# BaZzz01010101/ReflaxMan

Hardware: AMD Instinct MI355X
Metric: Mrays/sec at 3840×2160 depth-8; max per-channel |Δ| vs CPU reference (higher is better)
Workload: dtype f32; 1 GPU; C3 synth16: 16 spheres + 4 textured triangles + sun, 3840x2160, depth 8, 1 spp; scene=synth16, width=3840, height=2160, depth=8, spp=1, parallelism=single-gpu

## Files before the change

include/rfx.h:

```cpp
#ifndef RFX_H
#define RFX_H
#include <stddef.h>
#include <stdint.h>

#ifdef __cplusplus
extern "C" {
#endif

#define RFX_ABI_VERSION 4

typedef enum {
  RFX_OK = 0,
  RFX_ERR_ARG = -1,
  RFX_ERR_HIP = -2,
  RFX_ERR_STATE = -3,
  RFX_ERR_IO = -4,
  RFX_ERR_RNG = -5,
  RFX_ERR_NODEV = -6
} rfx_status;

enum { RFX_METAL = 0, RFX_DIELECTRIC = 1 };

typedef struct rfx_scene rfx_scene;
typedef struct rfx_renderer rfx_renderer;

int rfx_abi_version(void);
const char *rfx_last_error(void);
enum { RFX_BUILD_PRIM_LARGE = 1, RFX_BUILD_PRIM_SSAA = 2, RFX_BUILD_PRIM_LANES = 4, RFX_BUILD_ONE_LIGHT = 8 };
int rfx_build_options(void);

rfx_scene *rfx_scene_create(float diff_r, float diff_g, float diff_b, float diff_power);
void rfx_scene_destroy(rfx_scene *scene);
int rfx_scene_add_sphere(rfx_scene *scene, const float center[3], float radius, int material_type,
                         const float rgb[3], float reflectivity, float transparency);
int rfx_scene_add_triangle(rfx_scene *scene, const float v1[3], const float v2[3], const float v3[3],
                           int material_type, const float rgb[3], float reflectivity, float transparency);
int rfx_scene_add_mesh(rfx_scene *scene, const float *vertices, uint32_t n_vertices, const uint32_t *indices,
                       uint32_t n_triangles, int material_type, const float rgb[3], float reflectivity,
                       float transparency);
int rfx_scene_add_plane(rfx_scene *scene, const float pos[3], const float norm[3], int material_type,
                        const float rgb[3], float reflectivity, float transparency);
int rfx_scene_plane_count(const rfx_scene *scene);
int rfx_triangle_set_texture(rfx_scene *scene, int object_index, int texture_index, const float uv[6]);
int rfx_scene_add_light(rfx_scene *scene, const float origin[3], float radius, const float rgb[3], float power);
int rfx_scene_add_texture_argb(rfx_scene *scene, uint32_t width, uint32_t height, const uint32_t *argb);
int rfx_scene_add_texture_file(rfx_scene *scene, const char *path, int *loaded);
int rfx_scene_set_skybox_file(rfx_scene *scene, const char *path);
int rfx_scene_set_skybox_argb(rfx_scene *scene, uint32_t width, uint32_t height, const uint32_t *argb);
int rfx_scene_counts(const rfx_scene *scene, int *spheres, int *triangles, int *lights, int *textures);
int rfx_scene_tri_bvh_dump(const rfx_scene *scene, int32_t counts[5], float *boxes, int32_t *children,
                           int32_t *leaf_ids, int32_t *residual);

void rfx_camera_view(const float eye[3], const float at[3], float view[9]);
float rfx_camera_rz(uint32_t width, float fov);

int rfx_tga_load(const char *path, uint32_t *width, uint32_t *height, uint32_t *argb, size_t capacity);
int rfx_tga_save(const char *path, uint32_t width, uint32_t height, const uint32_t *argb);
int rfx_bmp_save(const char *path, uint32_t width, uint32_t height, const uint32_t *argb);
void rfx_argb_from_rgb(const float *rgb, size_t pixels, uint32_t *argb);

int rfx_renderer_create(rfx_renderer **out, int device);
void rfx_renderer_destroy(rfx_renderer *r);
int rfx_renderer_device(const rfx_renderer *r);
int rfx_renderer_set_stream(rfx_renderer *r, void *hip_stream);
int rfx_renderer_set_scene(rfx_renderer *r, const rfx_scene *scene);
int rfx_renderer_set_tile_order(rfx_renderer *r, int mode);
int rfx_renderer_set_regroup(rfx_renderer *r, int park_after);
int rfx_renderer_set_regroup_sort(rfx_renderer *r, int on);
int rfx_renderer_bounce_form(const rfx_renderer *r);
int rfx_renderer_set_tri_accel(rfx_renderer *r, int mode);
typedef struct {
  int32_t tri_nodes, tri_depth;
  int32_t tri_leaf_size;
  int32_t tri_in_leaves;
  int32_t tri_residual;
  int32_t sph_nodes, sph_depth;
  int32_t narrow_tri_bvh;
} rfx_accel_info;
int rfx_renderer_accel_info(const rfx_renderer *r, rfx_accel_info *out);
int rfx_renderer_set_prim_masks(rfx_renderer *r, int mode);
int rfx_renderer_set_rng(rfx_renderer *r, uint32_t sphere_seed, uint32_t jitter_seed);
int rfx_renderer_get_rng(rfx_renderer *r, uint32_t *sphere_seed, uint32_t *jitter_seed);

typedef struct {
  float eye[3];
  float view[9];
  float fov;
  uint32_t width, height;
  int32_t reflect_num;
  int32_t sample_num;
  int32_t additive;
  int32_t additive_counter;
  uint32_t row_block;
  uint32_t rank, nranks;
  uint64_t pixel_begin;
  uint64_t pixel_end;
  uint64_t span_begin;
  uint64_t span_end;
} rfx_frame;

uint32_t rfx_strip_rows(uint32_t height, uint32_t row_block, uint32_t rank, uint32_t nranks);
uint32_t rfx_strip_row_to_y(uint32_t r, uint32_t row_block, uint32_t rank, uint32_t nranks);

#define RFX_NCOUNTERS 40
int rfx_render_frame(rfx_renderer *r, const rfx_frame *frame, float *d_rgb, uint32_t *d_argb,
                     uint64_t *d_counters, void *stream);
int rfx_renderer_set_launch_traces(rfx_renderer *r, uint64_t max_traces);

int rfx_frame_rng_blocks(rfx_renderer *r, const rfx_frame *frame, uint32_t nslices, uint64_t *blocks_per_slice);
int rfx_frame_rng_count(rfx_renderer *r, const rfx_frame *frame, uint32_t slice, uint32_t nslices,
                        uint32_t *d_blk_counts, void *stream);
int rfx_render_frame_counted(rfx_renderer *r, const rfx_frame *frame, uint32_t nslices, const uint32_t *d_blk_counts,
                             float *d_rgb, uint32_t *d_argb, uint64_t *d_counters, void *stream);
int rfx_render_frame_counted_ev(rfx_renderer *r, const rfx_frame *frame, uint32_t nslices,
                                const uint32_t *d_blk_counts, float *d_rgb, uint32_t *d_argb, uint64_t *d_counters,
                                void *stream, void *emitted_event);

int rfx_frame_rng_emit(rfx_renderer *r, const rfx_frame *frame, uint32_t nslices, const uint32_t *d_blk_counts,
                       void *stream, void *emitted_event);
int rfx_render_frame_emitted(rfx_renderer *r, const rfx_frame *frame, float *d_rgb, uint32_t *d_argb,
                             uint64_t *d_counters, void *stream);
int rfx_frame_rng_discard(rfx_renderer *r);
int rfx_frame_rng_pending(rfx_renderer *r, uint32_t *frame_start);

int rfx_frame_rng_rewind(rfx_renderer *r);

typedef struct rfx_group rfx_group;
int rfx_group_create(rfx_group **out, const int *devices, int n);
void rfx_group_destroy(rfx_group *g);
int rfx_group_size(const rfx_group *g);
rfx_renderer *rfx_group_renderer(rfx_group *g, int member);
int rfx_group_set_scene(rfx_group *g, const rfx_scene *scene);
int rfx_group_set_bands(rfx_group *g, uint32_t height, const uint32_t *bounds);
int rfx_group_get_bands(const rfx_group *g, uint32_t *bounds);
int rfx_group_render_frame(rfx_group *g, const rfx_frame *frame, float *d_rgb, uint32_t *d_argb, void *stream);

int rfx_renderer_set_timing(rfx_renderer *r, int enable);
int rfx_renderer_get_timing(rfx_renderer *r, double *prepass_ms, double *trace_ms, uint64_t *frames);

int rfx_render_frame_host(rfx_renderer *r, const rfx_frame *frame, float *rgb, uint32_t *argb,
                          uint64_t *counters);

int rfx_device_alloc(rfx_renderer *r, size_t bytes, void **dptr);
int rfx_device_free(rfx_renderer *r, void *dptr);
int rfx_memcpy_d2h(rfx_renderer *r, void *dst, const void *src, size_t bytes);
int rfx_memcpy_h2d(rfx_renderer *r, void *dst, const void *src, size_t bytes);
int rfx_memcpy_d2d(rfx_renderer *r, void *dst, const void *src, size_t bytes);
int rfx_synchronize(rfx_renderer *r);

int rfx_rand_dirs(rfx_renderer *r, uint32_t seed, uint64_t n, float *out3, uint32_t *seed_out);

int rfx_kat_objects(rfx_renderer *r, const float *rays, const int32_t *objects, uint64_t n, float *out);
int rfx_kat_texels(rfx_renderer *r, int texture, const float *in, uint64_t n, float *out);
int rfx_kat_powf(rfx_renderer *r, const float *xy, uint64_t n, float *out);
int rfx_kat_argb(rfx_renderer *r, const float *rgb, uint64_t n, uint32_t *out);
int rfx_kat_powf_cube(rfx_renderer *r, uint64_t counts[2]);
int rfx_kat_div(rfx_renderer *r, uint64_t first, uint64_t n, uint64_t counts[3]);
int rfx_kat_kernarg(rfx_renderer *r, int swapped, uint32_t out[3]);

#ifdef __cplusplus
}
#endif
#endif
```

reflaxman_amd/_lib.py:

```python
from __future__ import annotations

import ctypes as C
import os

from . import _build

RFX_OK = 0
RFX_NCOUNTERS = 40
RFX_ABI_VERSION = 4
METAL, DIELECTRIC = 0, 1

_fp = C.POINTER(C.c_float)
_u32p = C.POINTER(C.c_uint32)
_u64p = C.POINTER(C.c_uint64)


class RfxError(RuntimeError):
    pass


class Frame(C.Structure):
    _fields_ = [
        ("eye", C.c_float * 3), ("view", C.c_float * 9), ("fov", C.c_float),
        ("width", C.c_uint32), ("height", C.c_uint32),
        ("reflect_num", C.c_int32), ("sample_num", C.c_int32),
        ("additive", C.c_int32), ("additive_counter", C.c_int32),
        ("row_block", C.c_uint32), ("rank", C.c_uint32), ("nranks", C.c_uint32),
        ("pixel_begin", C.c_uint64), ("pixel_end", C.c_uint64),
        ("span_begin", C.c_uint64), ("span_end", C.c_uint64),
    ]


class AccelInfo(C.Structure):
    _fields_ = [(n, C.c_int32) for n in ("tri_nodes", "tri_depth", "tri_leaf_size", "tri_in_leaves", "tri_residual",
                                         "sph_nodes", "sph_depth", "narrow_tri_bvh")]


_i32p = C.POINTER(C.c_int32)

SIGNATURES = [
    ("rfx_abi_version", C.c_int, []),
    ("rfx_last_error", C.c_char_p, []),
    ("rfx_build_options", C.c_int, []),
    ("rfx_scene_create", C.c_void_p, [C.c_float] * 4),
    ("rfx_scene_destroy", None, [C.c_void_p]),
    ("rfx_scene_add_sphere", C.c_int, [C.c_void_p, _fp, C.c_float, C.c_int, _fp, C.c_float, C.c_float]),
    ("rfx_scene_add_triangle", C.c_int, [C.c_void_p, _fp, _fp, _fp, C.c_int, _fp, C.c_float, C.c_float]),
    ("rfx_scene_add_mesh", C.c_int, [C.c_void_p, _fp, C.c_uint32, _u32p, C.c_uint32, C.c_int, _fp, C.c_float, C.c_float]),
    ("rfx_scene_tri_bvh_dump", C.c_int, [C.c_void_p, _i32p, _fp, _i32p, _i32p, _i32p]),
    ("rfx_scene_add_plane", C.c_int, [C.c_void_p, _fp, _fp, C.c_int, _fp, C.c_float, C.c_float]),
    ("rfx_scene_plane_count", C.c_int, [C.c_void_p]),
    ("rfx_triangle_set_texture", C.c_int, [C.c_void_p, C.c_int, C.c_int, _fp]),
    ("rfx_scene_add_light", C.c_int, [C.c_void_p, _fp, C.c_float, _fp, C.c_float]),
    ("rfx_scene_add_texture_argb", C.c_int, [C.c_void_p, C.c_uint32, C.c_uint32, _u32p]),
    ("rfx_scene_add_texture_file", C.c_int, [C.c_void_p, C.c_char_p, C.POINTER(C.c_int)]),
    ("rfx_scene_set_skybox_file", C.c_int, [C.c_void_p, C.c_char_p]),
    ("rfx_scene_set_skybox_argb", C.c_int, [C.c_void_p, C.c_uint32, C.c_uint32, _u32p]),
    ("rfx_scene_counts", C.c_int, [C.c_void_p] + [C.POINTER(C.c_int)] * 4),
    ("rfx_camera_view", None, [_fp, _fp, _fp]),
    ("rfx_camera_rz", C.c_float, [C.c_uint32, C.c_float]),
    ("rfx_tga_load", C.c_int, [C.c_char_p, _u32p, _u32p, _u32p, C.c_size_t]),
    ("rfx_tga_save", C.c_int, [C.c_char_p, C.c_uint32, C.c_uint32, _u32p]),
    ("rfx_bmp_save", C.c_int, [C.c_char_p, C.c_uint32, C.c_uint32, _u32p]),
    ("rfx_argb_from_rgb", None, [_fp, C.c_size_t, _u32p]),
    ("rfx_renderer_create", C.c_int, [C.POINTER(C.c_void_p), C.c_int]),
    ("rfx_renderer_destroy", None, [C.c_void_p]),
    ("rfx_renderer_device", C.c_int, [C.c_void_p]),
    ("rfx_renderer_set_stream", C.c_int, [C.c_void_p, C.c_void_p]),
    ("rfx_renderer_set_scene", C.c_int, [C.c_void_p, C.c_void_p]),
    ("rfx_renderer_set_rng", C.c_int, [C.c_void_p, C.c_uint32, C.c_uint32]),
    ("rfx_renderer_get_rng", C.c_int, [C.c_void_p, _u32p, _u32p]),
    ("rfx_strip_rows", C.c_uint32, [C.c_uint32] * 4),
    ("rfx_strip_row_to_y", C.c_uint32, [C.c_uint32] * 4),
    ("rfx_render_frame", C.c_int, [C.c_void_p, C.POINTER(Frame), C.c_void_p, C.c_void_p, C.c_void_p, C.c_void_p]),
    ("rfx_render_frame_host", C.c_int, [C.c_void_p, C.POINTER(Frame), _fp, _u32p, _u64p]),
    ("rfx_frame_rng_blocks", C.c_int, [C.c_void_p, C.POINTER(Frame), C.c_uint32, _u64p]),
    ("rfx_frame_rng_count", C.c_int, [C.c_void_p, C.POINTER(Frame), C.c_uint32, C.c_uint32, C.c_void_p, C.c_void_p]),
    ("rfx_render_frame_counted", C.c_int, [C.c_void_p, C.POINTER(Frame), C.c_uint32, C.c_void_p, C.c_void_p,
                                           C.c_void_p, C.c_void_p, C.c_void_p]),
    ("rfx_render_frame_counted_ev", C.c_int, [C.c_void_p, C.POINTER(Frame), C.c_uint32, C.c_void_p, C.c_void_p,
                                              C.c_void_p, C.c_void_p, C.c_void_p, C.c_void_p]),
    ("rfx_frame_rng_emit", C.c_int, [C.c_void_p, C.POINTER(Frame), C.c_uint32, C.c_void_p, C.c_void_p, C.c_void_p]),
    ("rfx_render_frame_emitted", C.c_int, [C.c_void_p, C.POINTER(Frame), C.c_void_p, C.c_void_p, C.c_void_p,
                                           C.c_void_p]),
    ("rfx_frame_rng_discard", C.c_int, [C.c_void_p]),
    ("rfx_frame_rng_pending", C.c_int, [C.c_void_p, _u32p]),
    ("rfx_frame_rng_rewind", C.c_int, [C.c_void_p]),
    ("rfx_group_create", C.c_int, [C.POINTER(C.c_void_p), C.POINTER(C.c_int), C.c_int]),
    ("rfx_group_destroy", None, [C.c_void_p]),
    ("rfx_group_size", C.c_int, [C.c_void_p]),
    ("rfx_group_renderer", C.c_void_p, [C.c_void_p, C.c_int]),
    ("rfx_group_set_scene", C.c_int, [C.c_void_p, C.c_void_p]),
    ("rfx_group_set_bands", C.c_int, [C.c_void_p, C.c_uint32, _u32p]),
    ("rfx_group_get_bands", C.c_int, [C.c_void_p, _u32p]),
    ("rfx_group_render_frame", C.c_int, [C.c_void_p, C.POINTER(Frame), C.c_void_p, C.c_void_p, C.c_void_p]),
    ("rfx_renderer_set_timing", C.c_int, [C.c_void_p, C.c_int]),
    ("rfx_renderer_set_tile_order", C.c_int, [C.c_void_p, C.c_int]),
    ("rfx_renderer_set_prim_masks", C.c_int, [C.c_void_p, C.c_int]),
    ("rfx_renderer_set_regroup", C.c_int, [C.c_void_p, C.c_int]),
    ("rfx_renderer_set_regroup_sort", C.c_int, [C.c_void_p, C.c_int]),
    ("rfx_renderer_set_launch_traces", C.c_int, [C.c_void_p, C.c_uint64]),
    ("rfx_renderer_bounce_form", C.c_int, [C.c_void_p]),
    ("rfx_renderer_set_tri_accel", C.c_int, [C.c_void_p, C.c_int]),
    ("rfx_renderer_accel_info", C.c_int, [C.c_void_p, C.POINTER(AccelInfo)]),
    ("rfx_renderer_get_timing", C.c_int, [C.c_void_p, C.POINTER(C.c_double), C.POINTER(C.c_double), _u64p]),
    ("rfx_device_alloc", C.c_int, [C.c_void_p, C.c_size_t, C.POINTER(C.c_void_p)]),
    ("rfx_device_free", C.c_int, [C.c_void_p, C.c_void_p]),
    ("rfx_memcpy_d2h", C.c_int, [C.c_void_p, C.c_void_p, C.c_void_p, C.c_size_t]),
    ("rfx_memcpy_h2d", C.c_int, [C.c_void_p, C.c_void_p, C.c_void_p, C.c_size_t]),
    ("rfx_memcpy_d2d", C.c_int, [C.c_void_p, C.c_void_p, C.c_void_p, C.c_size_t]),
    ("rfx_synchronize", C.c_int, [C.c_void_p]),
    ("rfx_rand_dirs", C.c_int, [C.c_void_p, C.c_uint32, C.c_uint64, _fp, _u32p]),
    ("rfx_kat_objects", C.c_int, [C.c_void_p, _fp, C.POINTER(C.c_int32), C.c_uint64, _fp]),
    ("rfx_kat_texels", C.c_int, [C.c_void_p, C.c_int, _fp, C.c_uint64, _fp]),
    ("rfx_kat_powf", C.c_int, [C.c_void_p, _fp, C.c_uint64, _fp]),
    ("rfx_kat_argb", C.c_int, [C.c_void_p, _fp, C.c_uint64, _u32p]),
    ("rfx_kat_powf_cube", C.c_int, [C.c_void_p, C.POINTER(C.c_uint64)]),
    ("rfx_kat_div", C.c_int, [C.c_void_p, C.c_uint64, C.c_uint64, C.POINTER(C.c_uint64)]),
    ("rfx_kat_kernarg", C.c_int, [C.c_void_p, C.c_int, C.POINTER(C.c_uint32)]),
]

_lib = None


def lib_path() -> str:
    return _build.LIB


def bind(path: str, partial: bool = False):
    L = C.CDLL(os.path.abspath(path))
    for name, res, args in SIGNATURES:
        if partial and not hasattr(L, name):
            continue
        fn = getattr(L, name)
        fn.restype = res
        fn.argtypes = args
    return L


def load(build_if_missing: bool = True):
    global _lib
    if _lib is not None:
        return _lib
    path = _build.LIB
    if build_if_missing:
        try:
            _build.build()
        except Exception as e:
            if not os.path.exists(path):
                raise RfxError(f"librfx.so missing and cannot be built: {e}") from e
    if not os.path.exists(path):
        raise RfxError(f"librfx.so not found at {path}: the HIP renderer is required (no CPU fallback)")
    L = C.CDLL(path)
    for name, res, args in SIGNATURES:
        fn = getattr(L, name)
        fn.restype = res
        fn.argtypes = args
    if L.rfx_abi_version() != RFX_ABI_VERSION:
        raise RfxError("librfx.so ABI version mismatch")
    _lib = L
    return L


def lib_sha256(path: str = None) -> str:
    import hashlib
    with open(path or _build.LIB, "rb") as f:
        return hashlib.sha256(f.read()).hexdigest()


def device_sha256(path: str = None) -> str:
    import hashlib
    import struct
    with open(path or _build.LIB, "rb") as f:
        b = f.read()
    shoff = struct.unpack_from("<Q", b, 0x28)[0]
    shentsize, shnum, shstrndx = struct.unpack_from("<HHH", b, 0x3A)
    secs = [struct.unpack_from("<IIQQQQIIQQ", b, shoff + i * shentsize) for i in range(shnum)]
    names = secs[shstrndx][4]
    for name_off, _, _, _, off, size, *_ in secs:
        if b[names + name_off:b.index(b"\0", names + name_off)] == b".hip_fatbin":
            return hashlib.sha256(b[off:off + size]).hexdigest()
    return None


def check(rc: int, what: str = "") -> int:
    if rc < 0:
        msg = load().rfx_last_error().decode(errors="replace")
        raise RfxError(f"{what or 'rfx call'} failed ({rc}): {msg}")
    return rc


def fptr(a):
    return a.ctypes.data_as(_fp)


def u32ptr(a):
    return a.ctypes.data_as(_u32p)


def u64ptr(a):
    return a.ctypes.data_as(_u64p)


def farr(v, n=None):
    v = list(v)
    if n is not None and len(v) != n:
        raise ValueError(f"expected {n} floats, got {len(v)}")
    return (C.c_float * len(v))(*v)
```

reflaxman_amd/csrc/rfx_host.cpp:

```cpp
#include <hip/hip_runtime.h>

#include <math.h>
#include <stdarg.h>
#include <stdio.h>
#include <stdlib.h>
#include <string.h>

#include <algorithm>
#include <cmath>
#include <mutex>
#include <string>
#include <vector>

#include "../../include/rfx.h"
#include "rfx_math.h"
#include "rfx_types.h"

#pragma clang fp contract(off)

namespace rfx {
uint64_t rng_blocks_for(uint64_t traces);
void rng_jump_table(uint64_t nblk, uint32_t *out);
hipError_t launch_rng_count(const uint32_t *d_seed, const uint32_t *d_jump, uint32_t *d_blk_cnt, uint64_t blk0,
                            uint64_t nblk_slice, uint16_t *d_masks, hipStream_t st);
hipError_t launch_rng_finish(const uint32_t *d_seed, const uint32_t *d_jump, uint32_t *d_next_seed,
                             const uint32_t *d_blk_cnt, const uint16_t *d_masks, uint64_t nblk, uint64_t traces,
                             uint32_t *d_rd_state, int *d_err, uint64_t ss2, uint64_t W, uint32_t row_block,
                             uint32_t rank, uint32_t nranks, hipStream_t st);
hipError_t launch_rng_finish_band(const uint32_t *d_seed, const uint32_t *d_jump, uint32_t *d_next_seed,
                                  const uint32_t *d_blk_cnt, const uint16_t *d_masks, uint64_t nblk, uint64_t traces,
                                  uint32_t *d_rd_state, int *d_err, uint64_t lo, uint64_t hi, uint64_t *d_off,
                                  uint32_t *d_range, uint32_t *d_tile_sum, hipStream_t st);
hipError_t launch_rng_fused(const uint32_t *d_seed, const uint32_t *d_jump, uint32_t *d_next_seed, uint64_t nblk,
                            uint64_t traces, uint32_t *d_rd_state, int *d_err, unsigned long long *d_status,
                            unsigned long long *d_ticket, unsigned long long base, uint32_t epoch, hipStream_t st);
hipError_t launch_trace(const DevScene &S, const FrameParams &P, bool stats, hipStream_t st);
hipError_t launch_prim_cull(const DevScene &S, const FrameParams &P, uint64_t *masks, hipStream_t st);
hipError_t launch_queue_sort(const uint32_t *count, const uint32_t *key, uint32_t *hist, uint32_t *order, hipStream_t st);
uint32_t trace_tiles(const FrameParams &P);
bool trace_lanes(const FrameParams &P);
bool trace_chunks(const FrameParams &P);
size_t tile_order_scratch();
hipError_t launch_tile_order(const uint32_t *cost, uint32_t n, uint32_t *order, uint32_t *scratch, hipStream_t st);
void launch_bounce(int cfg, dim3 grid, const DevScene &S, const FrameParams &P, hipStream_t st);
hipError_t launch_bounce_lds(int cfg, uint32_t groups, const DevScene &S, const FrameParams &P, hipStream_t st);
hipError_t launch_kat(int what, const DevScene &S, int tex, const void *in, const int32_t *objs, uint32_t n, void *out,
                      hipStream_t st);
hipError_t launch_kat_powf_cube(uint32_t first, uint32_t n, unsigned long long *counts, hipStream_t st);
hipError_t launch_kat_div(uint64_t first, uint32_t n, unsigned long long *counts, hipStream_t st);
hipError_t launch_kat_kernarg(const DevScene &S, const FrameParams &P, int swapped, uint32_t *out, hipStream_t st);
}

using namespace rfx;

static thread_local std::string g_last_error;

static int fail(int code, const char *fmt, ...)
{
  char buf[512];
  va_list ap;
  va_start(ap, fmt);
  vsnprintf(buf, sizeof(buf), fmt, ap);
  va_end(ap);
  g_last_error = buf;
  return code;
}

#define HIP_CHECK(expr)                                                                  \
  do {                                                                                   \
    hipError_t e_ = (expr);                                                              \
    if (e_ != hipSuccess) return fail(RFX_ERR_HIP, "%s: %s", #expr, hipGetErrorString(e_)); \
  } while (0)

extern "C" int rfx_abi_version(void) { return RFX_ABI_VERSION; }
extern "C" const char *rfx_last_error(void) { return g_last_error.c_str(); }

struct HostTexture { uint32_t w = 0, h = 0; bool loaded = false; std::vector<uint32_t> texels; };
struct HostMat { int dielectric; float r, g, b, refl, transp; };
struct HostSphere { v3 center; float radius, sq_radius; HostMat mat; int obj; };
struct HostTri {
  v3 v0, v1, v2, norm;
  double cond = INFINITY;
  m33 ax, tuv;
  float tu0 = 0, tv0 = 0;
  int tex = -1;
  HostMat mat;
  int obj;
};
struct HostLight { v3 origin; float radius; float r, g, b, power; };
struct HostPlane { v3 pos, norm; HostMat mat; int obj; };

struct rfx_scene {
  col diff, env;
  float diff_power;
  float half_tile_w, half_tile_h;
  int skybox = -1;
  std::vector<HostSphere> spheres;
  std::vector<HostTri> tris;
  std::vector<HostPlane> planes;
  std::vector<int> obj_kind, obj_idx;
  std::vector<HostLight> lights;
  std::vector<HostTexture> textures;
};

static void default_half_tiles(rfx_scene *s)
{
  s->half_tile_w = 1.0f / 8.0f - kFltEpsilon;
  s->half_tile_h = 1.0f / 6.0f - kFltEpsilon;
}

extern "C" rfx_scene *rfx_scene_create(float dr, float dg, float db, float dp)
{
  rfx_scene *s = new rfx_scene();
  s->diff = mkc(dr, dg, db);
  s->diff_power = dp;
  s->env = cscale(s->diff, dp);
  default_half_tiles(s);
  return s;
}

extern "C" void rfx_scene_destroy(rfx_scene *s) { delete s; }

static HostMat make_mat(int type, const float rgb[3], float refl, float transp)
{
  HostMat m;
  m.dielectric = type == RFX_DIELECTRIC;
  m.r = rgb[0]; m.g = rgb[1]; m.b = rgb[2];
  m.refl = clampf(refl, 0.0f, 1.0f);
  m.transp = clampf(transp, 0.0f, 1.0f);
  return m;
}

extern "C" int rfx_scene_add_sphere(rfx_scene *s, const float c[3], float radius, int type, const float rgb[3],
                                    float refl, float transp)
{
  if (!s || !c || !rgb || (type != RFX_METAL && type != RFX_DIELECTRIC)) return fail(RFX_ERR_ARG, "add_sphere: bad args");
  if (radius <= kVerySmall) radius = kVerySmall;
  HostSphere sp;
  sp.center = mk(c[0], c[1], c[2]);
  sp.radius = radius;
  sp.sq_radius = radius * radius;
  sp.mat = make_mat(type, rgb, refl, transp);
  sp.obj = (int)s->obj_kind.size();
  s->obj_kind.push_back(0);
  s->obj_idx.push_back((int)s->spheres.size());
  s->spheres.push_back(sp);
  return sp.obj;
}

extern "C" int rfx_scene_add_triangle(rfx_scene *s, const float a[3], const float b[3], const float c[3], int type,
                                      const float rgb[3], float refl, float transp)
{
  if (!s || !a || !b || !c || !rgb || (type != RFX_METAL && type != RFX_DIELECTRIC))
    return fail(RFX_ERR_ARG, "add_triangle: bad args");
  HostTri t;
  const v3 v0 = mk(a[0], a[1], a[2]), v1 = mk(b[0], b[1], b[2]), v2 = mk(c[0], c[1], c[2]);
  t.v0 = v0;
  t.mat = make_mat(type, rgb, refl, transp);
  t.norm = normalized(cross(sub(v1, v0), sub(v2, v0)));
  const m33 basis = from_cols(sub(v2, v0), sub(v1, v0), neg(t.norm));
  t.ax = inverted(basis);
  t.v1 = v1;
  t.v2 = v2;
  {
    const float *a = &basis.m11, *b = &t.ax.m11;
    double na = 0.0, nb = 0.0;
    for (int k = 0; k < 9; ++k) { na += (double)a[k] * a[k]; nb += (double)b[k] * b[k]; }
    const float det = basis.m11 * (basis.m22 * basis.m33 - basis.m32 * basis.m23) +
                      basis.m21 * (basis.m32 * basis.m13 - basis.m12 * basis.m33) +
                      basis.m31 * (basis.m12 * basis.m23 - basis.m13 * basis.m22);
    t.cond = fabsf(det) > kVerySmall ? sqrt(na * nb) : INFINITY;
  }
  memset(&t.tuv, 0, sizeof(t.tuv));
  t.obj = (int)s->obj_kind.size();
  s->obj_kind.push_back(1);
  s->obj_idx.push_back((int)s->tris.size());
  s->tris.push_back(t);
  return t.obj;
}

extern "C" int rfx_scene_add_mesh(rfx_scene *s, const float *vertices, uint32_t n_vertices, const uint32_t *indices,
                                  uint32_t n_triangles, int type, const float rgb[3], float refl, float transp)
{
  if (!s || !rgb || (type != RFX_METAL && type != RFX_DIELECTRIC) || (n_triangles && (!vertices || !indices)))
    return fail(RFX_ERR_ARG, "add_mesh: bad args");
  for (size_t i = 0; i < 3 * (size_t)n_triangles; ++i)
    if (indices[i] >= n_vertices)
      return fail(RFX_ERR_ARG, "add_mesh: index %u of triangle %zu is not below %u vertices", indices[i], i / 3, n_vertices);
// ... 156 lines not shown
  ih.biSize = sizeof(ih); ih.biWidth = (int32_t)w; ih.biHeight = (int32_t)h; ih.biPlanes = 1; ih.biBitCount = 32;
  bool ok = fwrite(&fh, sizeof(fh), 1, f) == 1 && fwrite(&ih, sizeof(ih), 1, f) == 1 &&
            fwrite(argb, (size_t)w * h * 4, 1, f) == 1;
  fclose(f);
  return ok ? RFX_OK : fail(RFX_ERR_IO, "bmp_save: short write");
}

extern "C" int rfx_scene_add_texture_file(rfx_scene *s, const char *path, int *loaded)
{
  if (!s || !path) return fail(RFX_ERR_ARG, "add_texture_file: bad args");
  HostTexture t;
  const bool ok = has_ext(path, ".tga") && tga_read(path, t.w, t.h, t.texels);
  t.loaded = ok;
  if (loaded) *loaded = ok ? 1 : 0;
  s->textures.push_back(std::move(t));
  return (int)s->textures.size() - 1;
}

static void set_skybox_index(rfx_scene *s, int idx)
{
  s->skybox = idx;
  const HostTexture &t = s->textures[idx];
  if (t.loaded)
  {
    s->half_tile_w = 1.0f / 8.0f - 1.0f / (float)t.w - kFltEpsilon;
    s->half_tile_h = 1.0f / 6.0f - 1.0f / (float)t.h - kFltEpsilon;
  }
  else
    default_half_tiles(s);
}

extern "C" int rfx_scene_set_skybox_file(rfx_scene *s, const char *path)
{
  if (!s || !path) return fail(RFX_ERR_ARG, "set_skybox_file: bad args");
  int loaded = 0;
  const int idx = rfx_scene_add_texture_file(s, path, &loaded);
  set_skybox_index(s, idx);
  return loaded;
}

extern "C" int rfx_scene_set_skybox_argb(rfx_scene *s, uint32_t w, uint32_t h, const uint32_t *argb)
{
  if (!s) return fail(RFX_ERR_ARG, "set_skybox_argb: null scene");
  const int idx = rfx_scene_add_texture_argb(s, w, h, argb);
  set_skybox_index(s, idx);
  return s->textures[idx].loaded ? 1 : 0;
}

extern "C" int rfx_scene_plane_count(const rfx_scene *s)
{
  if (!s) return fail(RFX_ERR_ARG, "plane_count: null scene");
  return (int)s->planes.size();
}

extern "C" int rfx_scene_counts(const rfx_scene *s, int *ns, int *nt, int *nl, int *nx)
{
  if (!s) return fail(RFX_ERR_ARG, "counts: null scene");
  if (ns) *ns = (int)s->spheres.size();
  if (nt) *nt = (int)s->tris.size();
  if (nl) *nl = (int)s->lights.size();
  if (nx) *nx = (int)s->textures.size();
  return RFX_OK;
}

extern "C" void rfx_camera_view(const float e[3], const float a[3], float view[9])
{
  const v3 eye = mk(e[0], e[1], e[2]), at = mk(a[0], a[1], a[2]);
  const v3 up = mk(0.0f, 1.0f, 0.0f);
  const v3 oz = normalized(sub(at, eye));
  const v3 ox = normalized(cross(up, oz));
  const v3 oy = normalized(cross(oz, ox));
  const m33 m = from_cols(ox, oy, oz);
  memcpy(view, &m, sizeof(m));
}

extern "C" float rfx_camera_rz(uint32_t width, float fov)
{
  return (float)width / 2.0f / tanf(fov / 2.0f);
}

extern "C" void rfx_argb_from_rgb(const float *rgb, size_t n, uint32_t *out)
{
  for (size_t i = 0; i < n; ++i) out[i] = argb(mkc(rgb[i * 3], rgb[i * 3 + 1], rgb[i * 3 + 2]));
}

extern "C" uint32_t rfx_strip_rows(uint32_t H, uint32_t rb, uint32_t rank, uint32_t nranks)
{
  if (nranks <= 1) return H;
  if (!rb || rank >= nranks) return 0;
  const uint32_t full = H / rb, rem = H % rb;
  uint32_t rows = (full / nranks) * rb;
  const uint32_t extra = full % nranks;
  if (rank < extra) rows += rb;
  if (rem && full % nranks == rank) rows += rem;
  return rows;
}

extern "C" uint32_t rfx_strip_row_to_y(uint32_t r, uint32_t rb, uint32_t rank, uint32_t nranks)
{
  if (nranks <= 1) return r;
  return (r / rb * nranks + rank) * rb + r % rb;
}

#ifndef RFX_TILE_ORDER_DEFAULT
#define RFX_TILE_ORDER_DEFAULT 1
#endif
#ifndef RFX_TILE_ORDER_MIN_TILES
#define RFX_TILE_ORDER_MIN_TILES 49152
#endif
constexpr size_t kPrimWords = 5;
constexpr size_t kPrimLargeWords = 12;
#ifndef RFX_PRIM_SSAA
#define RFX_PRIM_SSAA 0
#endif
#ifndef RFX_PRIM_LANES
#define RFX_PRIM_LANES 1
#endif
#ifndef RFX_PRIM_CHUNKS
#define RFX_PRIM_CHUNKS 1
#endif
#ifndef RFX_PRIM_LARGE
#define RFX_PRIM_LARGE 0
#endif
#ifndef RFX_ONE_LIGHT
#define RFX_ONE_LIGHT 1
#endif
#ifndef RFX_BOUNCE_GROUPS_PER_CU
#define RFX_BOUNCE_GROUPS_PER_CU 14
#endif

#ifndef RFX_QUEUE_SORT
#define RFX_QUEUE_SORT 0
#endif
#ifndef RFX_TRI_BVH_AUTO_MIN
#define RFX_TRI_BVH_AUTO_MIN 128
#endif
#ifndef RFX_TRI_BVH_NARROW_MIN
#define RFX_TRI_BVH_NARROW_MIN (1 << 30)
#endif
#ifndef RFX_PARK_AFTER
#define RFX_PARK_AFTER 2
#endif
#ifndef RFX_TILE_SORT_MAIN
#define RFX_TILE_SORT_MAIN 1
#endif
#ifndef RFX_TILE_SORT_EVERY
#define RFX_TILE_SORT_EVERY 16
#endif
#ifndef RFX_LAUNCH_TRACES
#define RFX_LAUNCH_TRACES (1ull << 30)
#endif
#ifndef RFX_SPLIT_STREAMS
#define RFX_SPLIT_STREAMS 2
#endif
constexpr uint64_t kMaxLaunchTraces = 1ull << 31;
#ifndef RFX_SCAN_EMIT_BLOCKS
#define RFX_SCAN_EMIT_BLOCKS 16384
#endif
struct rfx_renderer {
  int device = 0;
  int cus = 256;
  hipStream_t own_stream = nullptr;
  hipStream_t stream = nullptr;
  DevScene dev{};
  std::vector<void *> scene_allocs;
  bool has_scene = false;
  uint32_t *d_seed = nullptr;
  uint32_t seed_idx = 0;
  int *d_err = nullptr;
  uint32_t jitter_seed = 0;
  uint32_t *d_rd = nullptr; uint64_t rd_cap = 0;
  uint32_t *d_rd_alt = nullptr; uint64_t rd_alt_cap = 0;
  int emit_pending = -1;
  int trace_buf = 0;
  bool split_alt_busy = false;
  uint64_t emit_key[10] = {};
  bool rewind_ok = false, rewind_flip = false, rewind_saved = false;
  uint32_t rewind_jitter = 0;
  hipStream_t rewind_stream = nullptr;
  uint64_t launch_traces = RFX_LAUNCH_TRACES;
  uint64_t state_seq = 0;
  hipStream_t split_stream = nullptr;
  hipEvent_t split_ev[3] = {nullptr, nullptr, nullptr};
  uint32_t *d_blk_cnt = nullptr; uint64_t blk_cap = 0;
  uint64_t *d_blk_off = nullptr;
  uint32_t *d_rng_range = nullptr;
  uint32_t *d_tile_sum = nullptr;
  unsigned long long *d_rng_status = nullptr, *d_rng_ticket = nullptr;
  unsigned long long rng_tickets = 0;
  uint32_t rng_epoch = 0;
  uint16_t *d_rng_masks = nullptr;
  uint32_t *d_jump = nullptr;
  float *d_img = nullptr; uint32_t *d_argb = nullptr; uint64_t *d_cnt = nullptr; size_t img_cap = 0;
  int tile_mode = RFX_TILE_ORDER_DEFAULT;
  uint32_t *d_tile_cost = nullptr, *d_tile_order = nullptr, *d_tile_scratch = nullptr;
  uint32_t tile_cap = 0, tile_n = 0;
  uint64_t tile_key = 0;
  hipStream_t tile_stream = nullptr;
  hipEvent_t tile_fork = nullptr, tile_join = nullptr;
  bool tile_pending = false;
  hipStream_t tile_waited = nullptr;
  uint64_t tile_count = 0;
  int park_after = -1;
  uint64_t *d_prim_mask = nullptr;
  size_t prim_cap = 0;
  uint64_t *d_split_mask[2] = {nullptr, nullptr};
  size_t split_mask_cap[2] = {0, 0};
  std::vector<uint8_t> prim_key;
  std::vector<uint8_t> prim_seen;
  uint64_t scene_gen = 0;
  int prim_mode = 1;
  int tri_accel = -1;
  rfx_accel_info accel{};
  int bounce_form = 0;
  QRay *d_queue = nullptr;
  uint64_t queue_cap = 0;
  uint32_t *d_qctr = nullptr;
  uint32_t *d_qkey = nullptr, *d_qorder = nullptr;
  int queue_sort = RFX_QUEUE_SORT;
  bool timing = false, timing_this = false;
  uint32_t timing_every = 1;
  uint64_t timing_seq = 0;
  std::vector<hipEvent_t> events;
  size_t events_used = 0;
};

static uint32_t *seed_cur(rfx_renderer *r) { return r->d_seed + r->seed_idx; }
static uint32_t *seed_next(rfx_renderer *r) { return r->d_seed + (r->seed_idx ^ 1u); }

static int timing_event(rfx_renderer *r, hipStream_t st)
{
  if (!r->timing_this) return RFX_OK;
  if (r->events_used == r->events.size())
  {
    hipEvent_t e;
    HIP_CHECK(hipEventCreate(&e));
    r->events.push_back(e);
  }
  HIP_CHECK(hipEventRecord(r->events[r->events_used++], st));
  return RFX_OK;
}

static int timing_start(rfx_renderer *r, hipStream_t st)
{
  r->timing_this = r->timing && r->timing_seq++ % r->timing_every == 0;
  return timing_event(r, st);
}

extern "C" int rfx_renderer_set_timing(rfx_renderer *r, int enable)
{
  if (!r || enable < 0) return fail(RFX_ERR_ARG, "set_timing: null renderer or negative period");
  r->timing = enable != 0;
  r->timing_every = enable > 1 ? (uint32_t)enable : 1u;
  r->timing_seq = 0;
  r->timing_this = false;
  r->events_used = 0;
  return RFX_OK;
}

extern "C" int rfx_renderer_get_timing(rfx_renderer *r, double *prepass_ms, double *trace_ms, uint64_t *frames)
{
  if (!r) return fail(RFX_ERR_ARG, "get_timing: null renderer");
  double pre = 0.0, tr = 0.0;
  const size_t n = r->events_used / 3;
  if (n) HIP_CHECK(hipEventSynchronize(r->events[3 * n - 1]));
  for (size_t i = 0; i < n; ++i)
  {
    float a = 0.0f, b = 0.0f;
    HIP_CHECK(hipEventElapsedTime(&a, r->events[3 * i], r->events[3 * i + 1]));
    HIP_CHECK(hipEventElapsedTime(&b, r->events[3 * i + 1], r->events[3 * i + 2]));
    pre += a;
    tr += b;
  }
  r->events_used = 0;
  if (prepass_ms) *prepass_ms = pre;
  if (trace_ms) *trace_ms = tr;
  if (frames) *frames = n;
  return RFX_OK;
}

static int set_dev(rfx_renderer *r)
{
  HIP_CHECK(hipSetDevice(r->device));
  return RFX_OK;
}

extern "C" int rfx_renderer_create(rfx_renderer **out, int device)
{
  if (!out) return fail(RFX_ERR_ARG, "renderer_create: null out");
  *out = nullptr;
  int n = 0;
  if (hipGetDeviceCount(&n) != hipSuccess || n <= 0) return fail(RFX_ERR_NODEV, "no HIP device");
  if (device < 0 || device >= n) return fail(RFX_ERR_ARG, "device %d out of range (%d devices)", device, n);
  rfx_renderer *r = new rfx_renderer();
  r->device = device;
  int rc;
  if ((rc = set_dev(r)) != RFX_OK) { delete r; return rc; }
  if (hipStreamCreateWithFlags(&r->own_stream, hipStreamNonBlocking) != hipSuccess ||
      hipMalloc(&r->d_seed, 3 * sizeof(uint32_t)) != hipSuccess || hipMalloc(&r->d_err, sizeof(int)) != hipSuccess)
  {
    delete r;
    return fail(RFX_ERR_HIP, "renderer_create: HIP allocation failed");
  }
  r->stream = r->own_stream;
  if (hipDeviceGetAttribute(&r->cus, hipDeviceAttributeMultiprocessorCount, device) != hipSuccess || r->cus <= 0)
    r->cus = 256;
  const uint32_t seeds[2] = {1350490027u, 1350490027u};
  if (hipMemcpy(r->d_seed, seeds, sizeof(seeds), hipMemcpyHostToDevice) != hipSuccess ||
      hipMemset(r->d_err, 0, sizeof(int)) != hipSuccess)
  {
    delete r;
    return fail(RFX_ERR_HIP, "renderer_create: HIP init copy failed");
  }
  *out = r;
  return RFX_OK;
}

static void free_scene(rfx_renderer *r)
{
  for (void *p : r->scene_allocs) (void)hipFree(p);
  r->scene_allocs.clear();
  r->has_scene = false;
}

extern "C" void rfx_renderer_destroy(rfx_renderer *r)
{
  if (!r) return;
  (void)hipSetDevice(r->device);
  (void)hipStreamSynchronize(r->stream);
  free_scene(r);
  (void)hipFree(r->d_seed); (void)hipFree(r->d_err); (void)hipFree(r->d_rd); (void)hipFree(r->d_rd_alt);
  (void)hipFree(r->d_blk_cnt); (void)hipFree(r->d_jump); (void)hipFree(r->d_rng_masks); (void)hipFree(r->d_blk_off);
  (void)hipFree(r->d_tile_sum);
  (void)hipFree(r->d_rng_range);
  (void)hipFree(r->d_rng_status); (void)hipFree(r->d_rng_ticket);
  (void)hipFree(r->d_img); (void)hipFree(r->d_argb); (void)hipFree(r->d_cnt);
  (void)hipFree(r->d_queue); (void)hipFree(r->d_qctr); (void)hipFree(r->d_prim_mask);
  (void)hipFree(r->d_split_mask[0]); (void)hipFree(r->d_split_mask[1]);
  (void)hipFree(r->d_qkey); (void)hipFree(r->d_qorder);
  for (hipEvent_t e : r->events) (void)hipEventDestroy(e);
  if (r->tile_stream) (void)hipStreamSynchronize(r->tile_stream);
  (void)hipFree(r->d_tile_cost); (void)hipFree(r->d_tile_order); (void)hipFree(r->d_tile_scratch);
  if (r->tile_fork) (void)hipEventDestroy(r->tile_fork);
  if (r->tile_join) (void)hipEventDestroy(r->tile_join);
  if (r->tile_stream) (void)hipStreamDestroy(r->tile_stream);
  if (r->split_stream)
  {
    (void)hipStreamSynchronize(r->split_stream);
    (void)hipStreamDestroy(r->split_stream);
  }
  for (hipEvent_t e : r->split_ev)
    if (e) (void)hipEventDestroy(e);
  if (r->own_stream) (void)hipStreamDestroy(r->own_stream);
  delete r;
}

extern "C" int rfx_build_options(void)
{
  return (RFX_PRIM_LARGE ? RFX_BUILD_PRIM_LARGE : 0) | (RFX_PRIM_SSAA ? RFX_BUILD_PRIM_SSAA : 0) |
         (RFX_PRIM_LANES ? RFX_BUILD_PRIM_LANES : 0) | (RFX_ONE_LIGHT ? RFX_BUILD_ONE_LIGHT : 0) |
         (RFX_BVH_LEAF_PAIRS << 8);
}

extern "C" int rfx_renderer_set_launch_traces(rfx_renderer *r, uint64_t max_traces)
{
  if (!r) return fail(RFX_ERR_ARG, "renderer_set_launch_traces: null renderer");
  r->launch_traces = max_traces ? std::min(max_traces, kMaxLaunchTraces) : (uint64_t)RFX_LAUNCH_TRACES;
  return RFX_OK;
}

extern "C" int rfx_renderer_device(const rfx_renderer *r) { return r ? r->device : -1; }

extern "C" int rfx_renderer_set_tile_order(rfx_renderer *r, int mode)
{
  if (!r || mode < 0 || mode > 3) return fail(RFX_ERR_ARG, "renderer_set_tile_order: mode 0, 1, 2 or 3");
  r->tile_mode = mode;
  return RFX_OK;
}

extern "C" int rfx_renderer_set_prim_masks(rfx_renderer *r, int mode)
{
  if (!r || mode < 0 || mode > 2) return fail(RFX_ERR_ARG, "renderer_set_prim_masks: mode 0, 1 or 2");
  r->prim_mode = mode;
  r->prim_key.clear();
  r->prim_seen.clear();
  return RFX_OK;
}

extern "C" int rfx_renderer_bounce_form(const rfx_renderer *r)
{
  if (!r) return fail(RFX_ERR_ARG, "renderer_bounce_form: null renderer");
  return r->bounce_form;
}

extern "C" int rfx_renderer_set_regroup(rfx_renderer *r, int park_after)
{
  if (!r || park_after < -1) return fail(RFX_ERR_ARG, "renderer_set_regroup: -1 (default), 0 (off) or segments >= 1");
  r->park_after = park_after;
  return RFX_OK;
}

extern "C" int rfx_renderer_set_regroup_sort(rfx_renderer *r, int on)
{
  if (!r || on < 0 || on > 1) return fail(RFX_ERR_ARG, "renderer_set_regroup_sort: 0 or 1");
  r->queue_sort = on;
  return RFX_OK;
}

extern "C" int rfx_renderer_set_stream(rfx_renderer *r, void *s)
{
  if (!r) return fail(RFX_ERR_ARG, "set_stream: null renderer");
  r->stream = s ? (hipStream_t)s : r->own_stream;
  return RFX_OK;
}

template <class T>
static int upload(rfx_renderer *r, const std::vector<T> &v, const T **dst)
{
  if (v.empty()) { *dst = nullptr; return RFX_OK; }
  void *p = nullptr;
  HIP_CHECK(hipMalloc(&p, v.size() * sizeof(T)));
  r->scene_allocs.push_back(p);
  HIP_CHECK(hipMemcpy(p, v.data(), v.size() * sizeof(T), hipMemcpyHostToDevice));
  *dst = (const T *)p;
  return RFX_OK;
}

static void spatial_order(std::vector<uint32_t> &idx, size_t a, size_t b, const std::vector<HostSphere> &sp)
{
  if (b - a <= 2) return;
  double lo[3] = {INFINITY, INFINITY, INFINITY}, hi[3] = {-INFINITY, -INFINITY, -INFINITY};
  for (size_t i = a; i < b; ++i)
  {
    const double c[3] = {sp[idx[i]].center.x, sp[idx[i]].center.y, sp[idx[i]].center.z};
    for (int k = 0; k < 3; ++k) { lo[k] = fmin(lo[k], c[k]); hi[k] = fmax(hi[k], c[k]); }
  }
  int axis = 0;
  for (int k = 1; k < 3; ++k)
    if (hi[k] - lo[k] > hi[axis] - lo[axis]) axis = k;
  const size_t mid = a + 2 * ((b - a + 2) / 4);
  auto key = [&](uint32_t i) { return axis == 0 ? sp[i].center.x : axis == 1 ? sp[i].center.y : sp[i].center.z; };
  std::nth_element(idx.begin() + a, idx.begin() + mid, idx.begin() + b,
                   [&](uint32_t x, uint32_t y) { return key(x) < key(y) || (key(x) == key(y) && x < y); });
  spatial_order(idx, a, mid, sp);
  spatial_order(idx, mid, b, sp);
}

#ifndef RFX_BVH_STACK
#define RFX_BVH_STACK 16
#endif
namespace {
struct PairBox { double lo[3], hi[3], c[3]; };

int build_pair_bvh(std::vector<BvhNode> &nodes, std::vector<uint32_t> &pairs, size_t a, size_t b,
                   const std::vector<PairBox> &box, const double *ref, int level, int &depth, bool widen = true)
{
  if (b - a == 1) return ~(int)pairs[a];
  depth = std::max(depth, level + 1);
  const int id = (int)nodes.size();
  nodes.push_back(BvhNode{});
  double lo[3] = {INFINITY, INFINITY, INFINITY}, hi[3] = {-INFINITY, -INFINITY, -INFINITY};
  for (size_t i = a; i < b; ++i)
    for (int k = 0; k < 3; ++k) { lo[k] = fmin(lo[k], box[pairs[i]].c[k]); hi[k] = fmax(hi[k], box[pairs[i]].c[k]); }
  int axis = 0;
  for (int k = 1; k < 3; ++k)
    if (hi[k] - lo[k] > hi[axis] - lo[axis]) axis = k;
  size_t mid = a + (b - a) / 2;
  const size_t cnt = b - a;
  int need = 0;
  while (((size_t)1 << need) < cnt) ++need;
  if (level + need + 2 <= RFX_BVH_STACK && cnt > 2)
  {
    double best = INFINITY;
    int best_axis = axis;
    size_t best_mid = mid;
    std::vector<uint32_t> tmp(pairs.begin() + a, pairs.begin() + b);
    std::vector<double> right(cnt + 1);
    auto area = [](const double *l, const double *h) {
      const double dx = h[0] - l[0], dy = h[1] - l[1], dz = h[2] - l[2];
      return dx * dy + dy * dz + dz * dx;
    };
    for (int ax = 0; ax < 3; ++ax)
    {
      std::sort(tmp.begin(), tmp.end(), [&](uint32_t x, uint32_t y) {
        return box[x].c[ax] < box[y].c[ax] || (box[x].c[ax] == box[y].c[ax] && x < y);
      });
      double l[3] = {INFINITY, INFINITY, INFINITY}, h[3] = {-INFINITY, -INFINITY, -INFINITY};
      for (size_t i = cnt; i-- > 0;)
      {
        for (int k = 0; k < 3; ++k) { l[k] = fmin(l[k], box[tmp[i]].lo[k]); h[k] = fmax(h[k], box[tmp[i]].hi[k]); }
        right[i] = area(l, h) * (double)(cnt - i);
      }
      for (int k = 0; k < 3; ++k) { l[k] = INFINITY; h[k] = -INFINITY; }
      const size_t cap = (size_t)1 << std::min(30, RFX_BVH_STACK - level - 2);
      for (size_t i = 1; i < cnt; ++i)
      {
        for (int k = 0; k < 3; ++k) { l[k] = fmin(l[k], box[tmp[i - 1]].lo[k]); h[k] = fmax(h[k], box[tmp[i - 1]].hi[k]); }
        if (i > cap || cnt - i > cap) continue;
        const double cost = area(l, h) * (double)i + right[i];
        if (cost < best) { best = cost; best_axis = ax; best_mid = a + i; }
      }
    }
    axis = best_axis;
    mid = best_mid;
  }
  std::nth_element(pairs.begin() + a, pairs.begin() + mid, pairs.begin() + b, [&](uint32_t x, uint32_t y) {
    return box[x].c[axis] < box[y].c[axis] || (box[x].c[axis] == box[y].c[axis] && x < y);
  });
  const int kids[2] = {build_pair_bvh(nodes, pairs, a, mid, box, ref, level + 1, depth, widen),
                       build_pair_bvh(nodes, pairs, mid, b, box, ref, level + 1, depth, widen)};
  const size_t range[2][2] = {{a, mid}, {mid, b}};
  BvhNode &n = nodes[id];
  for (int c = 0; c < 2; ++c)
  {
    double l[3] = {INFINITY, INFINITY, INFINITY}, h[3] = {-INFINITY, -INFINITY, -INFINITY};
    for (size_t i = range[c][0]; i < range[c][1]; ++i)
      for (int k = 0; k < 3; ++k) { l[k] = fmin(l[k], box[pairs[i]].lo[k]); h[k] = fmax(h[k], box[pairs[i]].hi[k]); }
#if RFX_BVH_PREWIDE
    if (widen)
    {
      double cd = 0.0, hd = 0.0;
      for (int k = 0; k < 3; ++k)
      {
        const double dc = ref[k] - 0.5 * (l[k] + h[k]), dh = 0.5 * (h[k] - l[k]);
        cd += dc * dc;
        hd += dh * dh;
      }
      const double w = 2e-3 * (double)nextafterf((float)((sqrt(cd) + sqrt(hd)) * 1.0001), INFINITY) * (1.0 + 1e-6);
      for (int k = 0; k < 3; ++k) { l[k] -= w; h[k] += w; }
    }
#endif
    n.lx[c] = nextafterf((float)l[0], -INFINITY); n.ly[c] = nextafterf((float)l[1], -INFINITY);
    n.lz[c] = nextafterf((float)l[2], -INFINITY);
    n.hx[c] = nextafterf((float)h[0], INFINITY); n.hy[c] = nextafterf((float)h[1], INFINITY);
    n.hz[c] = nextafterf((float)h[2], INFINITY);
    n.child[c] = kids[c];
    double mt = 0.0;
    {
      double cd = 0.0, hd = 0.0;
      for (int k = 0; k < 3; ++k)
// ... 311 lines not shown
    {
      PairBox &b = box[j];
      for (int k = 0; k < 3; ++k) { b.lo[k] = INFINITY; b.hi[k] = -INFINITY; }
      for (size_t q = kLeafSph * j; q < std::min(nsph, kLeafSph * j + kLeafSph); ++q)
      {
        const double c[3] = {bd[q].x, bd[q].y, bd[q].z}, rr = bd[q].r;
        for (int k = 0; k < 3; ++k) { b.lo[k] = fmin(b.lo[k], c[k] - rr); b.hi[k] = fmax(b.hi[k], c[k] + rr); }
      }
      for (int k = 0; k < 3; ++k) b.c[k] = 0.5 * (b.lo[k] + b.hi[k]);
    }
    std::vector<uint32_t> pairs(npairs);
    for (size_t j = 0; j < npairs; ++j) pairs[j] = (uint32_t)j;
    for (int k = 0; k < 3; ++k)
    {
      double lo = INFINITY, hi = -INFINITY;
      for (const PairBox &pb : box) { lo = fmin(lo, pb.lo[k]); hi = fmax(hi, pb.hi[k]); }
      bvh_ref[k] = (double)(float)(0.5 * (lo + hi));
    }
    build_pair_bvh(bvh, pairs, 0, npairs, box, bvh_ref, 0, bvh_depth);
    if (bvh_depth > RFX_BVH_STACK) { bvh.clear(); bvh_depth = 0; }
    if (bvh.size() > 32767 || npairs > 32768) { bvh.clear(); bvh_depth = 0; }
  }
  TriTree tt;
  std::vector<TriGeo> tleaf;
  const bool want_tri = RFX_TRI_BVH && !small &&
                        (r->tri_accel >= 1 || (r->tri_accel < 0 && s->tris.size() >= (size_t)RFX_TRI_BVH_AUTO_MIN));
  if (want_tri)
  {
    if (nsph <= 32) tri_ref_point(s->tris, bvh_ref);
    if (build_tri_tree(s->tris, bvh_ref, true, tt))
    {
      tleaf.assign(tt.order.size(), TriGeo{});
      for (size_t q = 0; q < tt.order.size(); ++q)
      {
        const int32_t i = tt.order[q];
        if (i < 0) continue;
        tleaf[q] = tg[i];
        const int32_t obj = s->tris[i].obj;
        memcpy(&tleaf[q].pad[0], &i, 4);
        memcpy(&tleaf[q].pad[1], &obj, 4);
      }
    }
  }
  std::vector<PlaneGeo> pg;
  std::vector<MatRec> pm;
  for (const HostPlane &p : s->planes)
  {
    pg.push_back({p.pos.x, p.pos.y, p.pos.z, p.norm.x, p.norm.y, p.norm.z, p.obj, p.mat.dielectric});
    pm.push_back({p.mat.r, p.mat.g, p.mat.b, p.mat.refl});
  }
  std::vector<int32_t> loc(s->obj_kind.size());
  {
    std::vector<int32_t> sph_dev(nsph);
    for (size_t di = 0; di < nsph; ++di) sph_dev[order[di]] = (int32_t)di;
    for (size_t o = 0; o < loc.size(); ++o)
    {
      const int kind = s->obj_kind[o], idx = s->obj_idx[o];
      loc[o] = kind << 28 | (kind == 0 ? sph_dev[idx] : idx);
    }
  }
  std::vector<LightRec> lr;
  for (const HostLight &l : s->lights) lr.push_back({l.origin.x, l.origin.y, l.origin.z, l.radius, l.r, l.g, l.b, l.power});
  std::vector<TexRec> tr;
  std::vector<uint32_t> pool;
  for (const HostTexture &t : s->textures)
  {
    const bool empty = t.texels.empty();
    tr.push_back({(uint32_t)pool.size(), empty ? 0u : t.w, empty ? 0u : t.h, 0});
    pool.insert(pool.end(), t.texels.begin(), t.texels.end());
  }
  DevScene d{};
  if ((rc = upload(r, sg, &d.sph_geo)) || (rc = upload(r, sp, &d.sph_pair)) || (rc = upload(r, sm, &d.sph_mat)) ||
      (rc = upload(r, si, &d.sph_info)) ||
      (rc = upload(r, tg, &d.tri_geo)) || (rc = upload(r, ts, &d.tri_shade)) || (rc = upload(r, tm, &d.tri_mat)) ||
      (rc = upload(r, lr, &d.lights)) || (rc = upload(r, tr, &d.texs)) || (rc = upload(r, pool, &d.texels)) ||
      (rc = upload(r, bd, &d.bound)) || (rc = upload(r, cs, &d.cull_small)) || (rc = upload(r, ct, &d.cull_tri)) || (rc = upload(r, cb, &d.chunk_bound)) ||
      (rc = upload(r, pg, &d.pln_geo)) || (rc = upload(r, pm, &d.pln_mat)) || (rc = upload(r, loc, &d.obj_loc)) ||
      (rc = upload(r, bvh, &d.bvh)) || (rc = upload(r, tt.nodes, &d.tri_bvh)) || (rc = upload(r, tleaf, &d.tri_leaf)) ||
      (rc = upload(r, tt.resid, &d.tri_resid)))
    return rc;
  d.n_tri_resid = (int32_t)tt.resid.size();
  d.n_tri_bvh = (int32_t)tt.nodes.size();
  d.tri_bvh_depth = tt.depth;
  r->accel = rfx_accel_info{};
  r->accel.tri_nodes = d.n_tri_bvh;
  r->accel.tri_depth = tt.depth;
  r->accel.tri_leaf_size = RFX_TRI_BVH_LEAF;
  r->accel.tri_in_leaves = tt.nodes.empty() ? 0 : (int32_t)(s->tris.size() - tt.resid.size());
  r->accel.tri_residual = d.n_tri_resid;
  r->accel.sph_nodes = (int32_t)bvh.size();
  r->accel.sph_depth = bvh_depth;
  d.tri_bvh_narrow = !tt.nodes.empty() && (r->tri_accel == 2 || s->tris.size() >= (size_t)RFX_TRI_BVH_NARROW_MIN);
  r->accel.narrow_tri_bvh = d.tri_bvh_narrow;
  {
    float mt_max = 0.0f;
    for (const BvhNode &n : bvh) mt_max = fmaxf(mt_max, fmaxf(n.mt[0], n.mt[1]));
    const float mstep = mt_max > 0.0f ? mt_max / 65000.0f : 1.0f;
    std::vector<uint32_t> aux(2 * bvh.size());
    for (size_t i = 0; i < bvh.size(); ++i)
    {
      const BvhNode &n = bvh[i];
      uint32_t q[2];
      for (int c = 0; c < 2; ++c) q[c] = (uint32_t)std::min(65535.0, ceil((double)n.mt[c] / mstep) + 1.0);
      aux[2 * i] = ((uint32_t)(uint16_t)(int16_t)n.child[0]) | ((uint32_t)(uint16_t)(int16_t)n.child[1] << 16);
      aux[2 * i + 1] = q[0] | q[1] << 16;
    }
    if ((rc = upload(r, aux, &d.bvh_aux))) return rc;
    d.bvh_mstep = mstep;
    d.n_bvh = (int32_t)bvh.size();
  }
  d.n_sph = (int32_t)sg.size();
  d.n_tri = (int32_t)tg.size();
  d.n_light = (int32_t)lr.size();
  d.n_chunk = (int32_t)cb.size();
  d.n_pln = (int32_t)pg.size();
  d.n_tex = (int32_t)tr.size();
  d.bvh_depth = bvh_depth;
  d.bvh_rx = (float)bvh_ref[0]; d.bvh_ry = (float)bvh_ref[1]; d.bvh_rz = (float)bvh_ref[2];
  if (!bvh.empty())
  {
    const BvhNode &root = bvh[0];
    const float lo[3] = {fminf(root.lx[0], root.lx[1]), fminf(root.ly[0], root.ly[1]), fminf(root.lz[0], root.lz[1])};
    const float hi[3] = {fmaxf(root.hx[0], root.hx[1]), fmaxf(root.hy[0], root.hy[1]), fmaxf(root.hz[0], root.hz[1])};
    float s[3];
    for (int k = 0; k < 3; ++k) s[k] = hi[k] > lo[k] ? 8.0f / (hi[k] - lo[k]) : 0.0f;
    d.key_lx = lo[0]; d.key_ly = lo[1]; d.key_lz = lo[2];
    d.key_sx = s[0]; d.key_sy = s[1]; d.key_sz = s[2];
  }
  d.n_obj = (int32_t)loc.size();
  d.cull_valid = cull_valid;
  d.skybox_tex = s->skybox;
  const col amb = cscale(s->diff, s->diff_power);
  d.amb_r = amb.r; d.amb_g = amb.g; d.amb_b = amb.b;
  d.env_r = s->env.r; d.env_g = s->env.g; d.env_b = s->env.b;
  d.half_tile_w = s->half_tile_w;
  d.half_tile_h = s->half_tile_h;
  r->dev = d;
  r->has_scene = true;
  ++r->scene_gen;
  r->prim_key.clear();
  r->prim_seen.clear();
  return RFX_OK;
}

extern "C" int rfx_renderer_set_rng(rfx_renderer *r, uint32_t sphere_seed, uint32_t jitter_seed)
{
  if (!r) return fail(RFX_ERR_ARG, "set_rng: null renderer");
  int rc;
  if ((rc = set_dev(r)) != RFX_OK) return rc;
  HIP_CHECK(hipMemcpyAsync(seed_cur(r), &sphere_seed, sizeof(uint32_t), hipMemcpyHostToDevice, r->stream));
  HIP_CHECK(hipStreamSynchronize(r->stream));
  r->jitter_seed = jitter_seed;
  r->rewind_ok = false;
  ++r->state_seq;
  return RFX_OK;
}

extern "C" int rfx_renderer_get_rng(rfx_renderer *r, uint32_t *sphere_seed, uint32_t *jitter_seed)
{
  if (!r) return fail(RFX_ERR_ARG, "get_rng: null renderer");
  int rc;
  if ((rc = set_dev(r)) != RFX_OK) return rc;
  uint32_t s = 0;
  int err = 0;
  HIP_CHECK(hipMemcpyAsync(&s, seed_cur(r), sizeof(uint32_t), hipMemcpyDeviceToHost, r->stream));
  HIP_CHECK(hipMemcpyAsync(&err, r->d_err, sizeof(int), hipMemcpyDeviceToHost, r->stream));
  HIP_CHECK(hipStreamSynchronize(r->stream));
  if (err & 1) return fail(RFX_ERR_RNG, "RNG pre-pass ran short of accepted triples");
  if (sphere_seed) *sphere_seed = s;
  if (jitter_seed) *jitter_seed = r->jitter_seed;
  return RFX_OK;
}

static uint64_t rng_layout(uint64_t traces, uint32_t nslices, uint64_t *per_slice)
{
  if (!nslices) nslices = 1;
  const uint64_t bps = (rng_blocks_for(traces) + nslices - 1) / nslices;
  if (per_slice) *per_slice = bps;
  return bps * nslices;
}

static int ensure_rd_alt(rfx_renderer *r, uint64_t traces)
{
  if (r->rd_alt_cap < traces)
  {
    (void)hipFree(r->d_rd_alt);
    r->d_rd_alt = nullptr;
    r->rd_alt_cap = 0;
    HIP_CHECK(hipMalloc(&r->d_rd_alt, traces * sizeof(uint32_t)));
    r->rd_alt_cap = traces;
  }
  return RFX_OK;
}

static int ensure_rng_workspace(rfx_renderer *r, uint64_t traces, uint64_t nblk)
{
  if (traces > r->rd_cap)
  {
    (void)hipFree(r->d_rd);
    r->d_rd = nullptr;
    r->rd_cap = 0;
    HIP_CHECK(hipMalloc(&r->d_rd, traces * sizeof(uint32_t)));
    r->rd_cap = traces;
  }
  if (nblk > r->blk_cap)
  {
    (void)hipFree(r->d_blk_cnt); (void)hipFree(r->d_jump); (void)hipFree(r->d_rng_masks); (void)hipFree(r->d_blk_off);
    (void)hipFree(r->d_rng_status);
    r->d_blk_cnt = nullptr; r->d_jump = nullptr; r->d_rng_masks = nullptr; r->d_blk_off = nullptr; r->blk_cap = 0;
    r->d_rng_status = nullptr;
    HIP_CHECK(hipMalloc(&r->d_blk_cnt, nblk * sizeof(uint32_t)));
    HIP_CHECK(hipMalloc(&r->d_rng_status, nblk * sizeof(unsigned long long)));
    HIP_CHECK(hipMemset(r->d_rng_status, 0, nblk * sizeof(unsigned long long)));
    r->rng_epoch = 0;
    if (!r->d_rng_ticket)
    {
      HIP_CHECK(hipMalloc(&r->d_rng_ticket, sizeof(unsigned long long)));
      HIP_CHECK(hipMemset(r->d_rng_ticket, 0, sizeof(unsigned long long)));
    }
    HIP_CHECK(hipMalloc(&r->d_blk_off, nblk * sizeof(uint64_t)));
    (void)hipFree(r->d_tile_sum);
    r->d_tile_sum = nullptr;
    HIP_CHECK(hipMalloc(&r->d_tile_sum, (nblk / 4096 + 1) * sizeof(uint32_t)));
    if (!r->d_rng_range) HIP_CHECK(hipMalloc(&r->d_rng_range, 4 * sizeof(uint32_t)));
    HIP_CHECK(hipMalloc(&r->d_rng_masks, nblk * 256 * sizeof(uint16_t)));
    std::vector<uint32_t> jump(2 * (256 + nblk));
    rng_jump_table(nblk, jump.data());
    HIP_CHECK(hipMalloc(&r->d_jump, jump.size() * sizeof(uint32_t)));
    HIP_CHECK(hipMemcpy(r->d_jump, jump.data(), jump.size() * sizeof(uint32_t), hipMemcpyHostToDevice));
    r->blk_cap = nblk;
  }
  return RFX_OK;
}

static int enqueue_rng(rfx_renderer *r, uint64_t traces, hipStream_t st)
{
  int rc;
  const uint64_t nblk = rng_layout(traces, 1, nullptr);
  if ((rc = ensure_rng_workspace(r, traces, nblk)) != RFX_OK) return rc;
  HIP_CHECK(launch_rng_count(seed_cur(r), r->d_jump, r->d_blk_cnt, 0, nblk, r->d_rng_masks, st));
  HIP_CHECK(launch_rng_finish(seed_cur(r), r->d_jump, seed_next(r), r->d_blk_cnt, r->d_rng_masks, nblk, traces,
                              r->d_rd, r->d_err, 1, 1, 1, 0, 1, st));
  r->seed_idx ^= 1u;
  ++r->state_seq;
  r->rewind_ok = false;
  return RFX_OK;
}

struct FramePlan {
  FrameParams P;
  uint64_t traces = 0;
  hipStream_t st = nullptr;
  bool band = false;
  uint64_t band_lo = 0, band_hi = UINT64_MAX;
  bool split = false;
  int split_side = 0;
  uint64_t rd_traces() const { return band ? band_hi - band_lo : traces; }
};

static int plan_frame(rfx_renderer *r, const rfx_frame *f, void *stream, FramePlan &plan);

extern "C" int rfx_frame_rng_blocks(rfx_renderer *r, const rfx_frame *f, uint32_t nslices, uint64_t *per_slice)
{
  FramePlan pl;
  int rc;
  if ((rc = plan_frame(r, f, nullptr, pl)) != RFX_OK) return rc;
  if (!nslices || !per_slice) return fail(RFX_ERR_ARG, "frame_rng_blocks: nslices > 0 and an output required");
  rng_layout(pl.traces, nslices, per_slice);
  return RFX_OK;
}

extern "C" int rfx_frame_rng_count(rfx_renderer *r, const rfx_frame *f, uint32_t slice, uint32_t nslices,
                                   uint32_t *d_blk_counts, void *stream)
{
  FramePlan pl;
  int rc;
  if ((rc = plan_frame(r, f, stream, pl)) != RFX_OK) return rc;
  if (!d_blk_counts || !nslices || slice >= nslices) return fail(RFX_ERR_ARG, "frame_rng_count: bad slice");
  uint64_t bps = 0;
  const uint64_t nblk = rng_layout(pl.traces, nslices, &bps);
  if ((rc = ensure_rng_workspace(r, pl.rd_traces(), nblk)) != RFX_OK) return rc;
  HIP_CHECK(launch_rng_count(seed_cur(r), r->d_jump, d_blk_counts, (uint64_t)slice * bps, bps, nullptr, pl.st));
  return RFX_OK;
}

static int tile_schedule(rfx_renderer *r, FrameParams &P, hipStream_t st, uint64_t &key, bool &record)
{
  const uint32_t n = trace_tiles(P);
  key = ((uint64_t)P.W << 40) ^ ((uint64_t)P.grid_rows << 16) ^ ((uint64_t)(uint32_t)P.ss << 4) ^
        (uint64_t)(P.additive * 2 + P.accumulate);
  if (!r->tile_stream)
  {
    HIP_CHECK(hipStreamCreateWithFlags(&r->tile_stream, hipStreamNonBlocking));
    HIP_CHECK(hipEventCreateWithFlags(&r->tile_fork, hipEventDisableTiming));
    HIP_CHECK(hipEventCreateWithFlags(&r->tile_join, hipEventDisableTiming));
    HIP_CHECK(hipMalloc(&r->d_tile_scratch, tile_order_scratch()));
  }
  if (n > r->tile_cap)
  {
    HIP_CHECK(hipStreamSynchronize(r->tile_stream));
    if (r->tile_pending) HIP_CHECK(hipEventSynchronize(r->tile_join));
    HIP_CHECK(hipStreamSynchronize(st));
    (void)hipFree(r->d_tile_cost); (void)hipFree(r->d_tile_order);
    r->d_tile_cost = r->d_tile_order = nullptr;
    r->tile_cap = 0;
    r->tile_n = 0;
    r->tile_pending = false;
    HIP_CHECK(hipMalloc(&r->d_tile_cost, (size_t)n * sizeof(uint32_t)));
    HIP_CHECK(hipMalloc(&r->d_tile_order, (size_t)n * sizeof(uint32_t)));
    r->tile_cap = n;
  }
  if (r->tile_pending && r->tile_waited != st)
  {
    HIP_CHECK(hipStreamWaitEvent(st, r->tile_join, 0));
    r->tile_waited = st;
  }
  const bool same = r->tile_pending && r->tile_n == n && r->tile_key == key;
  P.tile_order = (same && r->tile_mode != 2) ? r->d_tile_order : nullptr;
  record = !same || r->tile_count % RFX_TILE_SORT_EVERY == 0;
  P.tile_cost = record ? r->d_tile_cost : nullptr;
  ++r->tile_count;
  return RFX_OK;
}

static int emit_frame(rfx_renderer *r, FramePlan &pl, const uint32_t *d_counts, const uint16_t *d_masks, uint64_t nblk,
                      uint32_t *rd, hipEvent_t emitted)
{
  const FrameParams &P = pl.P;
  const hipStream_t st = pl.st;
  const uint64_t ss2 = P.ss > 0 ? (uint64_t)(P.ss * P.ss) : 1;
  if (pl.band)
    HIP_CHECK(launch_rng_finish_band(seed_cur(r), r->d_jump, seed_next(r), d_counts, nullptr, nblk, pl.traces,
                                     rd - pl.band_lo, r->d_err, pl.band_lo, pl.band_hi, r->d_blk_off, r->d_rng_range,
                                     r->d_tile_sum, st));
  else if (P.nranks <= 1 && nblk > RFX_SCAN_EMIT_BLOCKS)
    HIP_CHECK(launch_rng_finish_band(seed_cur(r), r->d_jump, seed_next(r), d_counts, d_masks, nblk, pl.traces, rd,
                                     r->d_err, 0, pl.traces, r->d_blk_off, r->d_rng_range, r->d_tile_sum, st));
  else
    HIP_CHECK(launch_rng_finish(seed_cur(r), r->d_jump, seed_next(r), d_counts, d_masks, nblk, pl.traces, rd,
                                r->d_err, ss2, P.W, P.row_block, P.rank, P.nranks, st));
  r->seed_idx ^= 1u;
  ++r->state_seq;
  if (emitted) HIP_CHECK(hipEventRecord(emitted, st));
  return RFX_OK;
}

#ifndef RFX_RNG_FUSED
#define RFX_RNG_FUSED 1
#endif
#ifndef RFX_RNG_FUSED_MAX_BLOCKS
#define RFX_RNG_FUSED_MAX_BLOCKS 256
#endif
static bool fused_prepass(const FramePlan &pl, uint64_t nblk)
{
  return RFX_RNG_FUSED && !pl.band && pl.P.nranks <= 1 && nblk <= (uint64_t)RFX_RNG_FUSED_MAX_BLOCKS;
}

static int prepass_fused(rfx_renderer *r, FramePlan &pl, uint64_t nblk, uint32_t *rd, hipEvent_t emitted)
{
  if (r->rng_epoch == (1u << 28) - 1)
  {
    HIP_CHECK(hipMemsetAsync(r->d_rng_status, 0, r->blk_cap * sizeof(unsigned long long), pl.st));
    r->rng_epoch = 0;
  }
  ++r->rng_epoch;
  HIP_CHECK(launch_rng_fused(seed_cur(r), r->d_jump, seed_next(r), nblk, pl.traces, rd, r->d_err, r->d_rng_status,
                             r->d_rng_ticket, r->rng_tickets, r->rng_epoch, pl.st));
  r->rng_tickets += nblk;
  r->seed_idx ^= 1u;
  ++r->state_seq;
  if (emitted) HIP_CHECK(hipEventRecord(emitted, pl.st));
  return RFX_OK;
}

static int trace_frame(rfx_renderer *r, FramePlan &pl, const uint32_t *rd, float *d_rgb, uint32_t *d_argb,
                       uint64_t *d_counters);

static int finish_frame(rfx_renderer *r, FramePlan &pl, const uint32_t *d_counts, const uint16_t *d_masks,
                        uint64_t nblk, float *d_rgb, uint32_t *d_argb, uint64_t *d_counters,
                        hipEvent_t emitted = nullptr)
{
  int rc;
  if (r->emit_pending >= 0)
    return fail(RFX_ERR_STATE, "render_frame: an emitted frame awaits rfx_render_frame_emitted (or rfx_frame_rng_discard)");
  if ((rc = emit_frame(r, pl, d_counts, d_masks, nblk, r->d_rd, emitted)) != RFX_OK) return rc;
  r->trace_buf = 0;
  if ((rc = timing_event(r, pl.st)) != RFX_OK) return rc;
  return trace_frame(r, pl, r->d_rd, d_rgb, d_argb, d_counters);
}

static int trace_frame(rfx_renderer *r, FramePlan &pl, const uint32_t *rd, float *d_rgb, uint32_t *d_argb,
                       uint64_t *d_counters)
{
  int rc;
  FrameParams &P = pl.P;
  const hipStream_t st = pl.st;
  P.img = d_rgb;
  P.argb = d_argb;
  const bool small = r->dev.n_sph <= 32 && r->dev.n_tri <= 32;
  const bool plain = P.ss == 1 && !P.additive && !P.accumulate;
  const int park_after = r->park_after < 0 ? (small ? 0 : RFX_PARK_AFTER) : r->park_after;
  const bool park = park_after > 0 && plain && !d_counters && P.depth > park_after && P.grid_rows && !pl.split;
  const bool sort_queue = park && r->queue_sort;
  if (park)
  {
    if (pl.traces > r->queue_cap)
    {
      (void)hipFree(r->d_queue); (void)hipFree(r->d_qkey); (void)hipFree(r->d_qorder);
      r->d_queue = nullptr;
      r->d_qkey = r->d_qorder = nullptr;
      r->queue_cap = 0;
      HIP_CHECK(hipMalloc(&r->d_queue, pl.traces * sizeof(QRay)));
      HIP_CHECK(hipMalloc(&r->d_qkey, pl.traces * sizeof(uint32_t)));
      HIP_CHECK(hipMalloc(&r->d_qorder, pl.traces * sizeof(uint32_t)));
      r->queue_cap = pl.traces;
    }
    const size_t qwords = 2 + kQueueBuckets;
    if (!r->d_qctr) HIP_CHECK(hipMalloc(&r->d_qctr, qwords * sizeof(uint32_t)));
    HIP_CHECK(hipMemsetAsync(r->d_qctr, 0, (sort_queue ? qwords : 2) * sizeof(uint32_t), st));
    P.queue = r->d_queue;
    P.queue_count = r->d_qctr;
    P.queue_next = r->d_qctr + 1;
    P.park_after = park_after;
    if (sort_queue)
    {
      P.queue_key = r->d_qkey;
      P.queue_order = r->d_qorder;
    }
  }
  P.rd_state = pl.band ? rd - pl.band_lo : rd;
  P.counters = (unsigned long long *)d_counters;
  const bool sched = P.grid_rows && r->tile_mode && !d_counters && P.ss >= 0 && !pl.split &&
                     (r->tile_mode != 1 || trace_tiles(P) >= RFX_TILE_ORDER_MIN_TILES);
  uint64_t key = 0;
  bool record = false;
  if (sched && (rc = tile_schedule(r, P, st, key, record)) != RFX_OK) return rc;
  const bool chunks = RFX_PRIM_CHUNKS && RFX_PRIM_LANES && small && trace_chunks(P);
  if (chunks && pl.split && !d_counters && P.grid_rows && r->prim_mode)
  {
    const int sd = pl.split_side;
    const size_t nwords = (size_t)trace_tiles(P) * kPrimWords;
    if (nwords > r->split_mask_cap[sd])
    {
      (void)hipFree(r->d_split_mask[sd]);
      r->d_split_mask[sd] = nullptr;
      r->split_mask_cap[sd] = 0;
      HIP_CHECK(hipMalloc(&r->d_split_mask[sd], nwords * sizeof(uint64_t)));
      r->split_mask_cap[sd] = nwords;
    }
    HIP_CHECK(launch_prim_cull(r->dev, P, r->d_split_mask[sd], st));
    P.prim_mask = r->d_split_mask[sd];
    P.prim_shadow = 0;
  }
  else if (((small && (plain || (RFX_PRIM_LANES && (trace_lanes(P) || chunks)) || (RFX_PRIM_SSAA && P.ss >= 1)) &&
             !park) ||
            (RFX_PRIM_LARGE && !small && plain)) &&
           !d_counters && P.grid_rows && r->prim_mode && !pl.split)
  {
    struct Key { float cam[15]; uint32_t W, H, grid_rows, row0, row_block, rank, nranks; int32_t depth, ss, additive;
                 uint64_t p_begin, p_end, gen; } k;
    memset(&k, 0, sizeof(k));
    const float cam[15] = {P.eye_x, P.eye_y, P.eye_z, P.v11, P.v12, P.v13, P.v21, P.v22, P.v23,
                           P.v31, P.v32, P.v33, P.rz, P.wh, P.hh};
    memcpy(k.cam, cam, sizeof(cam));
    k.W = P.W; k.H = P.H; k.grid_rows = P.grid_rows; k.row0 = P.row0; k.row_block = P.row_block; k.rank = P.rank;
    k.nranks = P.nranks; k.depth = P.depth > 0 ? 1 : 0; k.p_begin = P.p_begin; k.p_end = P.p_end; k.gen = r->scene_gen;
    k.ss = P.ss; k.additive = P.additive ? 1 : 0;
    const size_t nwords = trace_tiles(P) * (small ? kPrimWords : kPrimLargeWords);
    std::vector<uint8_t> kb((const uint8_t *)&k, (const uint8_t *)&k + sizeof(k));
    if (nwords > r->prim_cap)
    {
      (void)hipFree(r->d_prim_mask);
      r->d_prim_mask = nullptr;
      r->prim_cap = 0;
      HIP_CHECK(hipMalloc(&r->d_prim_mask, nwords * sizeof(uint64_t)));
      r->prim_cap = nwords;
      r->prim_key.clear();
      r->prim_seen.clear();
    }
    if (r->prim_mode == 2 || kb != r->prim_key)
    {
      const bool repeat = kb == r->prim_seen;
      r->prim_seen = kb;
      r->prim_key.clear();
      if (repeat || r->prim_mode == 2 || chunks)
      {
        HIP_CHECK(launch_prim_cull(r->dev, P, r->d_prim_mask, st));
        r->prim_key = kb;
      }
    }
    if (!r->prim_key.empty())
    {
      P.prim_mask = r->d_prim_mask;
      P.prim_shadow = P.additive || chunks ? 0 : 1;
    }
  }
  if (P.grid_rows) HIP_CHECK(launch_trace(r->dev, P, d_counters != nullptr, st));
  r->bounce_form = 0;
  if (park)
  {
    const uint64_t waves = (pl.traces + 63) / 64;
    const uint32_t groups = (uint32_t)std::min<uint64_t>((waves + 1) / 2, (uint64_t)r->cus * RFX_BOUNCE_GROUPS_PER_CU);
    const int cfg = 1 | (r->dev.n_light > 32 ? 2 : 0) | (small ? 4 : 0) | (r->dev.n_pln ? 8 : 0) |
                    (RFX_ONE_LIGHT && r->dev.n_light == 1 ? 32 : 0) |
                    (RFX_TRI_BVH && r->dev.tri_bvh ? 64 : 0);
    if (sort_queue) HIP_CHECK(launch_queue_sort(r->d_qctr, r->d_qkey, r->d_qctr + 2, r->d_qorder, st));
    const uint32_t lgroups = (uint32_t)std::min<uint64_t>((waves + kLdsBvhWaves - 1) / kLdsBvhWaves, (uint64_t)r->cus);
    r->bounce_form = 2;
    if (small || !lds_bvh_fits(r->dev.n_bvh) || launch_bounce_lds(cfg, lgroups, r->dev, P, st) != hipSuccess)
    {
      (void)hipGetLastError();
      launch_bounce(cfg, dim3(groups), r->dev, P, st);
      r->bounce_form = 1;
    }
    HIP_CHECK(hipGetLastError());
  }
  if (record)
  {
#if RFX_TILE_SORT_MAIN
    HIP_CHECK(launch_tile_order(r->d_tile_cost, trace_tiles(P), r->d_tile_order, r->d_tile_scratch, st));
    HIP_CHECK(hipEventRecord(r->tile_join, st));
    r->tile_waited = st;
#else
    HIP_CHECK(hipEventRecord(r->tile_fork, st));
    HIP_CHECK(hipStreamWaitEvent(r->tile_stream, r->tile_fork, 0));
    HIP_CHECK(launch_tile_order(r->d_tile_cost, trace_tiles(P), r->d_tile_order, r->d_tile_scratch, r->tile_stream));
    HIP_CHECK(hipEventRecord(r->tile_join, r->tile_stream));
    r->tile_waited = nullptr;
#endif
    r->tile_pending = true;
    r->tile_n = trace_tiles(P);
    r->tile_key = key;
  }
  if ((rc = timing_event(r, st)) != RFX_OK) return rc;
  if (P.additive)
    r->jitter_seed = lcg_jump(r->jitter_seed, 2ull * (P.p_end - P.p_begin));
  return RFX_OK;
}

extern "C" int rfx_render_frame_counted(rfx_renderer *r, const rfx_frame *f, uint32_t nslices,
                                        const uint32_t *d_blk_counts, float *d_rgb, uint32_t *d_argb,
                                        uint64_t *d_counters, void *stream)
{
  return rfx_render_frame_counted_ev(r, f, nslices, d_blk_counts, d_rgb, d_argb, d_counters, stream, nullptr);
}

extern "C" int rfx_render_frame_counted_ev(rfx_renderer *r, const rfx_frame *f, uint32_t nslices,
                                           const uint32_t *d_blk_counts, float *d_rgb, uint32_t *d_argb,
                                           uint64_t *d_counters, void *stream, void *emitted_event)
{
  FramePlan pl;
  int rc;
  if ((rc = plan_frame(r, f, stream, pl)) != RFX_OK) return rc;
  if (!d_rgb || !d_blk_counts || !nslices) return fail(RFX_ERR_ARG, "render_frame_counted: bad args");
  if (pl.traces == 0) return RFX_OK;
  const uint64_t nblk = rng_layout(pl.traces, nslices, nullptr);
  if ((rc = ensure_rng_workspace(r, pl.rd_traces(), nblk)) != RFX_OK) return rc;
  if ((rc = timing_start(r, pl.st)) != RFX_OK) return rc;
  return finish_frame(r, pl, d_blk_counts, nullptr, nblk, d_rgb, d_argb, d_counters, (hipEvent_t)emitted_event);
}

static void plan_key(const FramePlan &pl, uint64_t key[10])
{
  const FrameParams &P = pl.P;
  key[0] = pl.traces;
  key[1] = pl.band_lo;
  key[2] = pl.band_hi;
  key[3] = ((uint64_t)P.W << 32) | P.H;
  key[4] = ((uint64_t)(uint32_t)P.ss << 32) | P.row_block;
  key[5] = ((uint64_t)P.rank << 32) | P.nranks;
  key[6] = ((uint64_t)P.row0 << 32) | P.grid_rows;
  key[7] = P.p_begin;
  key[8] = P.p_end;
  key[9] = P.trace_base;
}

extern "C" int rfx_frame_rng_emit(rfx_renderer *r, const rfx_frame *f, uint32_t nslices, const uint32_t *d_blk_counts,
                                  void *stream, void *emitted_event)
{
  FramePlan pl;
  int rc;
  if ((rc = plan_frame(r, f, stream, pl)) != RFX_OK) return rc;
  if (!d_blk_counts || !nslices) return fail(RFX_ERR_ARG, "frame_rng_emit: bad args");
  if (r->emit_pending >= 0) return fail(RFX_ERR_STATE, "frame_rng_emit: the last emitted frame has not been traced");
  if (pl.traces == 0) return RFX_OK;
  const uint64_t nblk = rng_layout(pl.traces, nslices, nullptr);
  if ((rc = ensure_rng_workspace(r, pl.rd_traces(), nblk)) != RFX_OK) return rc;
  if ((rc = ensure_rd_alt(r, pl.rd_traces())) != RFX_OK) return rc;
  const int buf = r->trace_buf == 0 ? 1 : 0;
  if (buf == 1 && r->split_alt_busy) HIP_CHECK(hipStreamWaitEvent(pl.st, r->split_ev[2], 0));
  r->split_alt_busy = false;
  if ((rc = emit_frame(r, pl, d_blk_counts, nullptr, nblk, buf ? r->d_rd_alt : r->d_rd,
                       (hipEvent_t)emitted_event)) != RFX_OK)
    return rc;
  r->emit_pending = buf;
  plan_key(pl, r->emit_key);
  return RFX_OK;
}

extern "C" int rfx_render_frame_emitted(rfx_renderer *r, const rfx_frame *f, float *d_rgb, uint32_t *d_argb,
                                        uint64_t *d_counters, void *stream)
{
  FramePlan pl;
  int rc;
  if ((rc = plan_frame(r, f, stream, pl)) != RFX_OK) return rc;
  if (!d_rgb) return fail(RFX_ERR_ARG, "render_frame_emitted: null framebuffer");
  if (pl.traces == 0) return RFX_OK;
  if (r->emit_pending < 0) return fail(RFX_ERR_STATE, "render_frame_emitted: no emitted frame (rfx_frame_rng_emit)");
  uint64_t key[10];
  plan_key(pl, key);
  if (memcmp(key, r->emit_key, sizeof(key)) != 0)
    return fail(RFX_ERR_STATE, "render_frame_emitted: the frame differs from the emitted one (band, geometry or traces); "
                               "rfx_frame_rng_discard it first");
  const int buf = r->emit_pending;
  r->emit_pending = -1;
  r->trace_buf = buf;
  if ((rc = timing_start(r, pl.st)) != RFX_OK) return rc;
  if ((rc = timing_event(r, pl.st)) != RFX_OK) return rc;
  return trace_frame(r, pl, buf ? r->d_rd_alt : r->d_rd, d_rgb, d_argb, d_counters);
}

extern "C" int rfx_frame_rng_discard(rfx_renderer *r)
{
  if (!r) return fail(RFX_ERR_ARG, "frame_rng_discard: null renderer");
  r->rewind_ok = false;
  if (r->emit_pending >= 0)
  {
    r->seed_idx ^= 1u;
    ++r->state_seq;
    r->emit_pending = -1;
  }
  return RFX_OK;
}

extern "C" int rfx_frame_rng_pending(rfx_renderer *r, uint32_t *frame_start)
{
  if (!r || !frame_start) return fail(RFX_ERR_ARG, "frame_rng_pending: bad args");
  int rc;
  if ((rc = set_dev(r)) != RFX_OK) return rc;
  const uint32_t *w = r->emit_pending >= 0 ? r->d_seed + (r->seed_idx ^ 1u) : seed_cur(r);
  HIP_CHECK(hipMemcpyAsync(frame_start, w, sizeof(uint32_t), hipMemcpyDeviceToHost, r->stream));
  HIP_CHECK(hipStreamSynchronize(r->stream));
  return r->emit_pending >= 0 ? 1 : 0;
}

static int render_split(rfx_renderer *r, const rfx_frame *f, uint64_t p0, uint64_t p1, float *d_rgb, uint32_t *d_argb,
                        uint64_t *d_counters, void *stream);

extern "C" int rfx_render_frame(rfx_renderer *r, const rfx_frame *f, float *d_rgb, uint32_t *d_argb,
                                uint64_t *d_counters, void *stream)
{
  FramePlan pl;
  int rc;
  if (!d_rgb) return fail(RFX_ERR_ARG, "render_frame: null framebuffer");
  if (r && f && f->sample_num > 0 && f->sample_num <= 256 && f->nranks <= 1 && f->width && f->height)
  {
    const uint64_t npx = (uint64_t)f->width * f->height;
    const uint64_t p0 = f->pixel_begin, p1 = (f->pixel_begin == 0 && f->pixel_end == 0) ? npx : f->pixel_end;
    if (p0 < p1 && p1 <= npx && (p1 - p0) * (uint64_t)(f->sample_num * f->sample_num) > r->launch_traces)
      return render_split(r, f, p0, p1, d_rgb, d_argb, d_counters, stream);
  }
  if ((rc = plan_frame(r, f, stream, pl)) != RFX_OK) return rc;
  const uint32_t jitter0 = r->jitter_seed;
  r->rewind_saved = false;
  if (pl.traces == 0)
  {
    r->rewind_ok = true;
    r->rewind_flip = false;
    r->rewind_jitter = jitter0;
    return RFX_OK;
  }
  const uint64_t nblk = rng_layout(pl.traces, 1, nullptr);
  if ((rc = ensure_rng_workspace(r, pl.traces, nblk)) != RFX_OK) return rc;
  if ((rc = timing_start(r, pl.st)) != RFX_OK) return rc;
  if (r->emit_pending >= 0)
    return fail(RFX_ERR_STATE, "render_frame: an emitted frame awaits rfx_render_frame_emitted (or rfx_frame_rng_discard)");
  if (fused_prepass(pl, nblk))
  {
    if ((rc = prepass_fused(r, pl, nblk, r->d_rd, nullptr)) != RFX_OK) return rc;
    r->trace_buf = 0;
    if ((rc = timing_event(r, pl.st)) != RFX_OK) return rc;
    if ((rc = trace_frame(r, pl, r->d_rd, d_rgb, d_argb, d_counters)) != RFX_OK) return rc;
  }
  else
  {
    HIP_CHECK(launch_rng_count(seed_cur(r), r->d_jump, r->d_blk_cnt, 0, nblk, r->d_rng_masks, pl.st));
    if ((rc = finish_frame(r, pl, r->d_blk_cnt, r->d_rng_masks, nblk, d_rgb, d_argb, d_counters)) != RFX_OK) return rc;
  }
  r->rewind_ok = true;
  r->rewind_flip = true;
  r->rewind_jitter = jitter0;
  return RFX_OK;
}

static int save_rewind_state(rfx_renderer *r, hipStream_t st)
{
  HIP_CHECK(hipMemcpyAsync(r->d_seed + 2, seed_cur(r), sizeof(uint32_t), hipMemcpyDeviceToDevice, st));
  return RFX_OK;
}

static int render_split(rfx_renderer *r, const rfx_frame *f, uint64_t p0, uint64_t p1, float *d_rgb, uint32_t *d_argb,
                        uint64_t *d_counters, void *stream)
{
  int rc;
  if ((rc = set_dev(r)) != RFX_OK) return rc;
  if (r->emit_pending >= 0)
    return fail(RFX_ERR_STATE, "render_frame: an emitted frame awaits rfx_render_frame_emitted (or rfx_frame_rng_discard)");
  const uint64_t W = f->width, spp = (uint64_t)(f->sample_num * f->sample_num);
  uint64_t per = std::max<uint64_t>(1, r->launch_traces / spp);
  const bool rows = per >= W;
  if (rows) per = per / W * W;
  const uint64_t cap = per * spp;
  const hipStream_t st[2] = {stream ? (hipStream_t)stream : r->stream, nullptr};
  if (!r->split_stream) HIP_CHECK(hipStreamCreateWithFlags(&r->split_stream, hipStreamNonBlocking));
  for (hipEvent_t &e : r->split_ev)
    if (!e) HIP_CHECK(hipEventCreateWithFlags(&e, hipEventDisableTiming));
  hipStream_t s2[2] = {st[0], r->split_stream};
  if ((rc = ensure_rng_workspace(r, cap, rng_layout(cap, 1, nullptr))) != RFX_OK) return rc;
  if ((rc = ensure_rd_alt(r, cap)) != RFX_OK) return rc;
  const uint32_t jitter0 = r->jitter_seed;
  if ((rc = save_rewind_state(r, s2[0])) != RFX_OK) return rc;
  HIP_CHECK(hipEventRecord(r->split_ev[2], s2[0]));
  HIP_CHECK(hipStreamWaitEvent(s2[1], r->split_ev[2], 0));
  uint64_t k = 0;
  for (uint64_t a = p0; a < p1; ++k)
  {
    const uint64_t b = std::min(p1, rows ? (a / W) * W + per : a + per);
    rfx_frame fk = *f;
    fk.pixel_begin = a;
    fk.pixel_end = b;
    const int side = RFX_SPLIT_STREAMS > 1 ? (int)(k & 1) : 0;
    FramePlan pl;
    if ((rc = plan_frame(r, &fk, s2[side], pl)) != RFX_OK) return rc;
    pl.split = true;
    pl.split_side = side;
    const uint64_t nblk = rng_layout(pl.traces, 1, nullptr);
    if (k > 0) HIP_CHECK(hipStreamWaitEvent(s2[side], r->split_ev[side ^ 1], 0));
    if ((rc = timing_start(r, pl.st)) != RFX_OK) return rc;
    uint32_t *rd = side ? r->d_rd_alt : r->d_rd;
    if (fused_prepass(pl, nblk))
    {
      if ((rc = prepass_fused(r, pl, nblk, rd, r->split_ev[side])) != RFX_OK) return rc;
    }
    else
    {
      HIP_CHECK(launch_rng_count(seed_cur(r), r->d_jump, r->d_blk_cnt, 0, nblk, r->d_rng_masks, pl.st));
      if ((rc = emit_frame(r, pl, r->d_blk_cnt, r->d_rng_masks, nblk, rd, r->split_ev[side])) != RFX_OK) return rc;
    }
    if ((rc = timing_event(r, pl.st)) != RFX_OK) return rc;
    if ((rc = trace_frame(r, pl, rd, d_rgb, d_argb, d_counters)) != RFX_OK) return rc;
    a = b;
  }
  if (k > 1)
  {
    HIP_CHECK(hipEventRecord(r->split_ev[2], s2[1]));
    HIP_CHECK(hipStreamWaitEvent(s2[0], r->split_ev[2], 0));
  }
  r->trace_buf = 0;
  r->split_alt_busy = k > 1;
  r->rewind_ok = true;
  r->rewind_flip = false;
  r->rewind_saved = true;
  r->rewind_stream = s2[0];
  r->rewind_jitter = jitter0;
  return RFX_OK;
}

extern "C" int rfx_frame_rng_rewind(rfx_renderer *r)
{
  if (!r) return fail(RFX_ERR_ARG, "frame_rng_rewind: null renderer");
  if (!r->rewind_ok) return fail(RFX_ERR_STATE, "frame_rng_rewind: the last call was not rfx_render_frame");
  if (r->rewind_flip) r->seed_idx ^= 1u;
  ++r->state_seq;
  if (r->rewind_saved)
  {
    int rc;
    if ((rc = set_dev(r)) != RFX_OK) return rc;
    HIP_CHECK(hipMemcpyAsync(seed_cur(r), r->d_seed + 2, sizeof(uint32_t), hipMemcpyDeviceToDevice, r->rewind_stream));
    ++r->state_seq;
  }
  r->jitter_seed = r->rewind_jitter;
  r->rewind_ok = false;
  r->rewind_saved = false;
  return RFX_OK;
}

static int plan_frame(rfx_renderer *r, const rfx_frame *f, void *stream, FramePlan &plan)
{
  if (!r || !f) return fail(RFX_ERR_ARG, "render_frame: bad args");
  if (!r->has_scene) return fail(RFX_ERR_STATE, "render_frame: no scene uploaded");
  r->rewind_ok = false;
  if (!f->width || !f->height || f->reflect_num <= 0 || f->sample_num == 0)
    return fail(RFX_ERR_ARG, "render_frame: W=%u H=%u reflect_num=%d sample_num=%d", f->width, f->height,
                f->reflect_num, f->sample_num);
  const uint32_t nranks = f->nranks ? f->nranks : 1;
  const bool band = nranks > 1 && !f->row_block;
  if (nranks > 1 && (f->sample_num < 0 || f->rank >= nranks))
    return fail(RFX_ERR_ARG, "render_frame: a partition needs sample_num > 0, rank < nranks");
  if (f->sample_num > 256 || f->sample_num < -4096) return fail(RFX_ERR_ARG, "render_frame: sample_num out of range");
  int rc;
  if ((rc = set_dev(r)) != RFX_OK) return rc;
  hipStream_t st = stream ? (hipStream_t)stream : r->stream;

  const uint32_t W = f->width, H = f->height;
  const uint64_t npx = (uint64_t)W * H;
  uint64_t p0 = f->pixel_begin, p1 = f->pixel_end;
  if (band)
  {
    const uint64_t s0 = f->span_begin, s1 = (f->span_begin == 0 && f->span_end == 0) ? npx : f->span_end;
    if (p0 >= p1 || p1 > npx || p0 % W || p1 % W)
      return fail(RFX_ERR_ARG, "render_frame: a band is whole rows [pixel_begin, pixel_end) / W of the frame");
    if (s0 >= s1 || s1 > npx || s0 % W || s1 % W || p0 < s0 || p1 > s1)
      return fail(RFX_ERR_ARG, "render_frame: a band's span is whole rows [span_begin, span_end) / W around the band");
    plan.band = true;
    plan.band_lo = (p0 - s0) * (uint64_t)(f->sample_num * f->sample_num);
    plan.band_hi = (p1 - s0) * (uint64_t)(f->sample_num * f->sample_num);
    p0 = s0;
    p1 = s1;
  }
  if (p0 == 0 && p1 == 0) p1 = npx;
  if (p0 >= p1 || p1 > npx) return fail(RFX_ERR_ARG, "render_frame: pixel span [%llu, %llu) outside frame",
                                        (unsigned long long)p0, (unsigned long long)p1);
  if (nranks > 1 && !band && (p0 != 0 || p1 != npx)) return fail(RFX_ERR_ARG, "render_frame: strips need the whole frame");
  const uint32_t y0 = (uint32_t)(p0 / W), y1 = (uint32_t)((p1 - 1) / W);
  uint64_t traces, trace_base = 0;
  uint32_t grid_rows, row0;
  if (f->sample_num < 0)
  {
    const uint64_t n = (uint64_t)(-f->sample_num);
    const uint64_t bw = (W + n - 1) / n;
    auto corners_before = [&](uint64_t p) -> uint64_t {
      const uint64_t y = p / W, x = p % W;
      return (y + n - 1) / n * bw + (y % n == 0 ? (x + n - 1) / n : 0);
    };
    trace_base = corners_before(p0);
    traces = corners_before(p1) - trace_base;
    row0 = (uint32_t)(y0 / n);
    grid_rows = (uint32_t)(y1 / n - y0 / n + 1);
  }
  else
  {
    traces = (p1 - p0) * (uint64_t)(f->sample_num * f->sample_num);
    row0 = nranks > 1 ? 0 : y0;
    grid_rows = nranks > 1 ? rfx_strip_rows(H, f->row_block, f->rank, nranks) : y1 - y0 + 1;
    if (band)
    {
      row0 = (uint32_t)(f->pixel_begin / W);
      grid_rows = (uint32_t)((f->pixel_end - f->pixel_begin) / W);
    }
  }
  if (traces > kMaxLaunchTraces)
    return fail(RFX_ERR_ARG, "render_frame: %llu traces in one launch exceed 2^31 (partitions: a smaller span)",
                (unsigned long long)traces);
  plan.traces = traces;
  plan.st = st;
  FrameParams &P = plan.P;
  P = FrameParams{};
  P.eye_x = f->eye[0]; P.eye_y = f->eye[1]; P.eye_z = f->eye[2];
  P.v11 = f->view[0]; P.v12 = f->view[1]; P.v13 = f->view[2];
  P.v21 = f->view[3]; P.v22 = f->view[4]; P.v23 = f->view[5];
  P.v31 = f->view[6]; P.v32 = f->view[7]; P.v33 = f->view[8];
  P.rz = rfx_camera_rz(W, f->fov);
  P.wh = W / 2.0f;
  P.hh = H / 2.0f;
  P.W = W; P.H = H;
  P.depth = f->reflect_num;
  P.ss = f->sample_num;
  P.accumulate = f->sample_num > 0 && f->additive_counter > 1;
  P.additive = f->sample_num > 0 && f->additive;
  P.jitter_seed = r->jitter_seed;
  P.row_block = f->row_block ? f->row_block : 1;
  P.rank = nranks > 1 && !band ? f->rank : 0;
  P.nranks = band ? 1 : nranks;
  P.grid_rows = grid_rows;
  P.row0 = row0;
  P.p_begin = p0;
  P.p_end = p1;
  P.trace_base = trace_base;
  return RFX_OK;
}

extern "C" int rfx_device_alloc(rfx_renderer *r, size_t bytes, void **p)
{
  if (!r || !p) return fail(RFX_ERR_ARG, "device_alloc: bad args");
  int rc;
  if ((rc = set_dev(r)) != RFX_OK) return rc;
  HIP_CHECK(hipMalloc(p, bytes ? bytes : 1));
  return RFX_OK;
}

extern "C" int rfx_device_free(rfx_renderer *r, void *p)
{
  if (!r) return fail(RFX_ERR_ARG, "device_free: null renderer");
  int rc;
  if ((rc = set_dev(r)) != RFX_OK) return rc;
  HIP_CHECK(hipFree(p));
  return RFX_OK;
}

extern "C" int rfx_memcpy_d2h(rfx_renderer *r, void *dst, const void *src, size_t n)
{
  if (!r) return fail(RFX_ERR_ARG, "memcpy: null renderer");
  HIP_CHECK(hipMemcpyAsync(dst, src, n, hipMemcpyDeviceToHost, r->stream));
  HIP_CHECK(hipStreamSynchronize(r->stream));
  return RFX_OK;
}

extern "C" int rfx_memcpy_d2d(rfx_renderer *r, void *dst, const void *src, size_t n)
{
  if (!r || (n && (!dst || !src))) return fail(RFX_ERR_ARG, "memcpy_d2d: bad args");
  int rc;
  if ((rc = set_dev(r)) != RFX_OK) return rc;
  if (n) HIP_CHECK(hipMemcpyAsync(dst, src, n, hipMemcpyDeviceToDevice, r->stream));
  return RFX_OK;
}

extern "C" int rfx_memcpy_h2d(rfx_renderer *r, void *dst, const void *src, size_t n)
{
  if (!r) return fail(RFX_ERR_ARG, "memcpy: null renderer");
  HIP_CHECK(hipMemcpyAsync(dst, src, n, hipMemcpyHostToDevice, r->stream));
  HIP_CHECK(hipStreamSynchronize(r->stream));
  return RFX_OK;
}

extern "C" int rfx_synchronize(rfx_renderer *r)
{
  if (!r) return fail(RFX_ERR_ARG, "synchronize: null renderer");
  HIP_CHECK(hipStreamSynchronize(r->stream));
  int err = 0;
  HIP_CHECK(hipMemcpy(&err, r->d_err, sizeof(int), hipMemcpyDeviceToHost));
  if (err & 1) return fail(RFX_ERR_RNG, "RNG pre-pass ran short of accepted triples");
  return RFX_OK;
}

extern "C" int rfx_render_frame_host(rfx_renderer *r, const rfx_frame *f, float *rgb, uint32_t *argb_out,
                                     uint64_t *counters)
{
  if (!r || !f || !rgb) return fail(RFX_ERR_ARG, "render_frame_host: bad args");
  if (f->nranks > 1) return fail(RFX_ERR_ARG, "render_frame_host: whole frames only");
  int rc;
  if ((rc = set_dev(r)) != RFX_OK) return rc;
  const size_t px = (size_t)f->width * f->height;
  if (px > r->img_cap)
  {
    (void)hipFree(r->d_img); (void)hipFree(r->d_argb);
    r->d_img = nullptr; r->d_argb = nullptr; r->img_cap = 0;
    HIP_CHECK(hipMalloc(&r->d_img, px * 3 * sizeof(float)));
    HIP_CHECK(hipMalloc(&r->d_argb, px * sizeof(uint32_t)));
    r->img_cap = px;
  }
  if (!r->d_cnt) HIP_CHECK(hipMalloc(&r->d_cnt, RFX_NCOUNTERS * sizeof(uint64_t)));
  HIP_CHECK(hipMemcpyAsync(r->d_img, rgb, px * 3 * sizeof(float), hipMemcpyHostToDevice, r->stream));
  if (counters) HIP_CHECK(hipMemsetAsync(r->d_cnt, 0, RFX_NCOUNTERS * sizeof(uint64_t), r->stream));
  if ((rc = rfx_render_frame(r, f, r->d_img, argb_out ? r->d_argb : nullptr, counters ? r->d_cnt : nullptr, nullptr)))
    return rc;
  HIP_CHECK(hipMemcpyAsync(rgb, r->d_img, px * 3 * sizeof(float), hipMemcpyDeviceToHost, r->stream));
  if (argb_out) HIP_CHECK(hipMemcpyAsync(argb_out, r->d_argb, px * sizeof(uint32_t), hipMemcpyDeviceToHost, r->stream));
  if (counters)
  {
    uint64_t c[RFX_NCOUNTERS];
    HIP_CHECK(hipMemcpyAsync(c, r->d_cnt, sizeof(c), hipMemcpyDeviceToHost, r->stream));
    HIP_CHECK(hipStreamSynchronize(r->stream));
    for (int k = 0; k < RFX_NCOUNTERS; ++k) counters[k] += c[k];
  }
  return rfx_synchronize(r);
}

extern "C" int rfx_rand_dirs(rfx_renderer *r, uint32_t seed, uint64_t n, float *out3, uint32_t *seed_out)
{
  if (!r || !out3 || !n) return fail(RFX_ERR_ARG, "rand_dirs: bad args");
  int rc;
  if ((rc = set_dev(r)) != RFX_OK) return rc;
  uint32_t saved = 0;
  HIP_CHECK(hipMemcpyAsync(&saved, seed_cur(r), sizeof(uint32_t), hipMemcpyDeviceToHost, r->stream));
  HIP_CHECK(hipStreamSynchronize(r->stream));
  HIP_CHECK(hipMemcpyAsync(seed_cur(r), &seed, sizeof(uint32_t), hipMemcpyHostToDevice, r->stream));
  if ((rc = enqueue_rng(r, n, r->stream)) != RFX_OK) return rc;
  std::vector<uint32_t> states(n);
  HIP_CHECK(hipMemcpyAsync(states.data(), r->d_rd, n * sizeof(uint32_t), hipMemcpyDeviceToHost, r->stream));
  uint32_t after = 0;
  HIP_CHECK(hipMemcpyAsync(&after, seed_cur(r), sizeof(uint32_t), hipMemcpyDeviceToHost, r->stream));
  HIP_CHECK(hipMemcpyAsync(seed_cur(r), &saved, sizeof(uint32_t), hipMemcpyHostToDevice, r->stream));
  if ((rc = rfx_synchronize(r)) != RFX_OK) return rc;
  for (uint64_t i = 0; i < n; ++i)
  {
    const uint32_t s1 = lcg_step(states[i]), s2 = lcg_step(s1), s3 = lcg_step(s2);
    out3[i * 3] = rand_component(lcg_out(s1));
    out3[i * 3 + 1] = rand_component(lcg_out(s2));
    out3[i * 3 + 2] = rand_component(lcg_out(s3));
  }
  if (seed_out) *seed_out = after;
  return RFX_OK;
}

template <class T>
static int kat_buffer(size_t n, const T *src, T **dev)
{
  *dev = nullptr;
  HIP_CHECK(hipMalloc((void **)dev, n ? n * sizeof(T) : sizeof(T)));
  if (src && n) HIP_CHECK(hipMemcpy(*dev, src, n * sizeof(T), hipMemcpyHostToDevice));
  return RFX_OK;
}

static int kat_run(rfx_renderer *r, int what, int tex, const void *in, size_t in_elems, const int32_t *objs,
                   uint64_t n, void *out, size_t out_elems)
{
  int rc;
  if ((rc = set_dev(r)) != RFX_OK) return rc;
  if (n >= (1ull << 31)) return fail(RFX_ERR_ARG, "kat: n too large");
  float *d_in = nullptr, *d_out = nullptr;
  int32_t *d_obj = nullptr;
  rc = kat_buffer(in_elems, (const float *)in, &d_in);
  if (rc == RFX_OK && objs) rc = kat_buffer((size_t)n, objs, &d_obj);
  if (rc == RFX_OK) rc = kat_buffer(out_elems, (const float *)nullptr, &d_out);
  if (rc == RFX_OK)
  {
    hipError_t e = launch_kat(what, r->dev, tex, d_in, d_obj, (uint32_t)n, d_out, r->stream);
    if (e == hipSuccess) e = hipStreamSynchronize(r->stream);
    if (e == hipSuccess) e = hipMemcpy(out, d_out, out_elems * 4, hipMemcpyDeviceToHost);
    if (e != hipSuccess) rc = fail(RFX_ERR_HIP, "kat: %s", hipGetErrorString(e));
  }
  (void)hipFree(d_in); (void)hipFree(d_obj); (void)hipFree(d_out);
  return rc;
}

extern "C" int rfx_kat_objects(rfx_renderer *r, const float *rays, const int32_t *objects, uint64_t n, float *out)
{
  if (!r || (n && (!rays || !objects || !out))) return fail(RFX_ERR_ARG, "kat_objects: bad args");
  if (!r->has_scene) return fail(RFX_ERR_STATE, "kat_objects: no scene uploaded");
  for (uint64_t i = 0; i < n; ++i)
    if (objects[i] < 0 || objects[i] >= r->dev.n_obj) return fail(RFX_ERR_ARG, "kat_objects: object %d", objects[i]);
  return kat_run(r, 0, 0, rays, (size_t)n * 6, objects, n, out, (size_t)n * 15);
}

extern "C" int rfx_kat_texels(rfx_renderer *r, int texture, const float *in, uint64_t n, float *out)
{
  if (!r || (n && (!in || !out))) return fail(RFX_ERR_ARG, "kat_texels: bad args");
  if (!r->has_scene) return fail(RFX_ERR_STATE, "kat_texels: no scene uploaded");
  if (texture >= r->dev.n_tex) return fail(RFX_ERR_ARG, "kat_texels: texture %d", texture);
  return kat_run(r, 1, texture, in, (size_t)n * (texture >= 0 ? 2 : 3), nullptr, n, out, (size_t)n * 3);
}

extern "C" int rfx_kat_powf(rfx_renderer *r, const float *xy, uint64_t n, float *out)
{
  if (!r || (n && (!xy || !out))) return fail(RFX_ERR_ARG, "kat_powf: bad args");
  return kat_run(r, 2, 0, xy, (size_t)n * 2, nullptr, n, out, (size_t)n);
}

extern "C" int rfx_kat_powf_cube(rfx_renderer *r, uint64_t counts[2])
{
  if (!r || !counts) return fail(RFX_ERR_ARG, "kat_powf_cube: bad args");
  unsigned long long *d = nullptr;
  hipError_t e = hipMalloc(&d, 2 * sizeof(unsigned long long));
  if (e == hipSuccess) e = hipMemsetAsync(d, 0, 2 * sizeof(unsigned long long), r->stream);
  for (uint64_t first = 0; e == hipSuccess && first <= 0x3f800000ull; first += 1ull << 28)
    e = launch_kat_powf_cube((uint32_t)first, (uint32_t)std::min<uint64_t>(1ull << 28, 0x3f800001ull - first), d, r->stream);
  unsigned long long h[2] = {0, 0};
  if (e == hipSuccess) e = hipStreamSynchronize(r->stream);
  if (e == hipSuccess) e = hipMemcpy(h, d, sizeof(h), hipMemcpyDeviceToHost);
  (void)hipFree(d);
  if (e != hipSuccess) return fail(RFX_ERR_HIP, "kat_powf_cube: %s", hipGetErrorString(e));
  counts[0] = h[0];
  counts[1] = h[1];
  return RFX_OK;
}

extern "C" int rfx_kat_div(rfx_renderer *r, uint64_t first, uint64_t n, uint64_t counts[3])
{
  if (!r || !counts) return fail(RFX_ERR_ARG, "kat_div: bad args");
  int rc;
  if ((rc = set_dev(r)) != RFX_OK) return rc;
  unsigned long long *d = nullptr;
  hipError_t e = hipMalloc(&d, 3 * sizeof(unsigned long long));
  if (e == hipSuccess) e = hipMemsetAsync(d, 0, 3 * sizeof(unsigned long long), r->stream);
  for (uint64_t k = 0; e == hipSuccess && k < n; k += 1ull << 28)
    e = launch_kat_div(first + k, (uint32_t)std::min<uint64_t>(1ull << 28, n - k), d, r->stream);
  unsigned long long h[3] = {0, 0, 0};
  if (e == hipSuccess) e = hipStreamSynchronize(r->stream);
  if (e == hipSuccess) e = hipMemcpy(h, d, sizeof(h), hipMemcpyDeviceToHost);
  (void)hipFree(d);
  if (e != hipSuccess) return fail(RFX_ERR_HIP, "kat_div: %s", hipGetErrorString(e));
  for (int i = 0; i < 3; ++i) counts[i] = h[i];
  return RFX_OK;
}

extern "C" int rfx_kat_argb(rfx_renderer *r, const float *rgb, uint64_t n, uint32_t *out)
{
  if (!r || (n && (!rgb || !out))) return fail(RFX_ERR_ARG, "kat_argb: bad args");
  return kat_run(r, 3, 0, rgb, (size_t)n * 3, nullptr, n, out, (size_t)n);
}

extern "C" int rfx_kat_kernarg(rfx_renderer *r, int swapped, uint32_t out[3])
{
  if (!r || !out) return fail(RFX_ERR_ARG, "kat_kernarg: bad args");
  if (!r->has_scene) return fail(RFX_ERR_STATE, "kat_kernarg: no scene uploaded");
  int rc;
  if ((rc = set_dev(r)) != RFX_OK) return rc;
  FrameParams P;
  uint32_t *w = (uint32_t *)&P;
  for (size_t i = 0; i < sizeof(P) / 4; ++i) w[i] = 0x9E3779B9u * (uint32_t)(i + 1);
  uint32_t *d = nullptr;
  hipError_t e = hipMalloc(&d, 3 * sizeof(uint32_t));
  if (e == hipSuccess) e = hipMemsetAsync(d, 0xFF, 3 * sizeof(uint32_t), r->stream);
  if (e == hipSuccess) e = launch_kat_kernarg(r->dev, P, swapped, d, r->stream);
  if (e == hipSuccess) e = hipStreamSynchronize(r->stream);
  if (e == hipSuccess) e = hipMemcpy(out, d, 3 * sizeof(uint32_t), hipMemcpyDeviceToHost);
  (void)hipFree(d);
  if (e != hipSuccess) return fail(RFX_ERR_HIP, "kat_kernarg: %s", hipGetErrorString(e));
  return RFX_OK;
}

int rfx_detail_fail(int code, const char *msg) { return fail(code, "%s", msg); }
uint32_t *rfx_detail_seed_word(rfx_renderer *r) { return seed_cur(r); }
uint32_t rfx_detail_jitter(const rfx_renderer *r) { return r->jitter_seed; }
void rfx_detail_set_jitter(rfx_renderer *r, uint32_t jitter) { r->jitter_seed = jitter; }
hipStream_t rfx_detail_stream(const rfx_renderer *r) { return r->stream; }
void rfx_detail_set_rewindable(rfx_renderer *r, uint32_t jitter0)
{
  r->rewind_ok = true;
  r->rewind_flip = true;
  r->rewind_saved = false;
  r->rewind_jitter = jitter0;
}
int rfx_detail_save_start(rfx_renderer *r, hipStream_t st)
{
  int rc;
  if ((rc = set_dev(r)) != RFX_OK) return rc;
  return save_rewind_state(r, st);
}
void rfx_detail_set_rewindable_saved(rfx_renderer *r, uint32_t jitter0, hipStream_t st)
{
  r->rewind_ok = true;
  r->rewind_flip = false;
  r->rewind_saved = true;
  r->rewind_stream = st;
  r->rewind_jitter = jitter0;
}
uint64_t rfx_detail_launch_traces(const rfx_renderer *r) { return r->launch_traces; }
uint64_t rfx_detail_state_seq(const rfx_renderer *r) { return r->state_seq; }
```

reflaxman_amd/csrc/rfx_kernels.hip:

```cpp
#include "rfx_trace.h"

#pragma clang fp contract(off)

namespace rfx {

constexpr int kLptThreads = 1024, kLptBuckets = 256, kLptGroups = 64;

__device__ __forceinline__ uint32_t lpt_key(const uint32_t *cost, uint32_t i)
{
  const uint32_t c = max(cost[i], 1u);
  const uint32_t e = 31u - (uint32_t)__clz(c);
  const uint32_t m = e >= 3u ? (c >> (e - 3u)) & 7u : (c << (3u - e)) & 7u;
  return (uint32_t)(kLptBuckets - 1) - min(e * 8u + m, (uint32_t)(kLptBuckets - 1));
}

__global__ __launch_bounds__(kLptThreads) void lpt_hist(const uint32_t *cost, uint32_t n, uint32_t chunk, uint32_t *hist)
{
  __shared__ uint32_t h[kLptBuckets];
  for (uint32_t b = threadIdx.x; b < kLptBuckets; b += kLptThreads) h[b] = 0;
  __syncthreads();
  const uint32_t i0 = blockIdx.x * chunk, i1 = min(n, i0 + chunk);
  for (uint32_t i = i0 + threadIdx.x; i < i1; i += kLptThreads) atomicAdd(&h[lpt_key(cost, i)], 1u);
  __syncthreads();
  for (uint32_t b = threadIdx.x; b < kLptBuckets; b += kLptThreads) hist[blockIdx.x * kLptBuckets + b] = h[b];
}

__global__ __launch_bounds__(kLptBuckets) void lpt_scan(uint32_t *hist)
{
  __shared__ uint32_t wtot[kLptBuckets / 64];
  const uint32_t b = threadIdx.x, lane = b & 63u;
  uint32_t v[kLptGroups];
#pragma unroll
  for (int g = 0; g < kLptGroups; ++g) v[g] = hist[g * kLptBuckets + b];
  uint32_t run = 0;
#pragma unroll
  for (int g = 0; g < kLptGroups; ++g) { const uint32_t c = v[g]; v[g] = run; run += c; }
  uint32_t inc = run;
#pragma unroll
  for (int o = 1; o < 64; o <<= 1)
  {
    const uint32_t t = __shfl_up(inc, o, 64);
    if (lane >= (uint32_t)o) inc += t;
  }
  if (lane == 63u) wtot[b >> 6] = inc;
  __syncthreads();
  uint32_t base = inc - run;
  for (uint32_t w = 0; w < (b >> 6); ++w) base += wtot[w];
#pragma unroll
  for (int g = 0; g < kLptGroups; ++g) hist[g * kLptBuckets + b] = v[g] + base;
}

__global__ __launch_bounds__(kLptThreads) void lpt_scatter(const uint32_t *cost, uint32_t n, uint32_t chunk,
                                                            const uint32_t *hist, uint32_t *order)
{
  __shared__ uint32_t off[kLptBuckets];
  for (uint32_t b = threadIdx.x; b < kLptBuckets; b += kLptThreads) off[b] = hist[blockIdx.x * kLptBuckets + b];
  __syncthreads();
  const uint32_t i0 = blockIdx.x * chunk, i1 = min(n, i0 + chunk);
  for (uint32_t i = i0 + threadIdx.x; i < i1; i += kLptThreads) order[atomicAdd(&off[lpt_key(cost, i)], 1u)] = i;
}

uint32_t trace_tiles(const FrameParams &P);

size_t tile_order_scratch() { return (size_t)kLptGroups * kLptBuckets * sizeof(uint32_t); }

hipError_t launch_tile_order(const uint32_t *cost, uint32_t n, uint32_t *order, uint32_t *scratch, hipStream_t st)
{
  const uint32_t chunk = (n + kLptGroups - 1) / kLptGroups;
  hipLaunchKernelGGL(lpt_hist, dim3(kLptGroups), dim3(kLptThreads), 0, st, cost, n, chunk, scratch);
  hipLaunchKernelGGL(lpt_scan, dim3(1), dim3(kLptBuckets), 0, st, scratch);
  hipLaunchKernelGGL(lpt_scatter, dim3(kLptGroups), dim3(kLptThreads), 0, st, cost, n, chunk, scratch, order);
  return hipGetLastError();
}

constexpr int kQsThreads = 1024, kQsGroups = 256;

__global__ __launch_bounds__(kQsThreads) void qs_hist(const uint32_t *count, const uint32_t *key, uint32_t *hist)
{
  __shared__ uint32_t h[kQueueBuckets];
  for (uint32_t b = threadIdx.x; b < kQueueBuckets; b += kQsThreads) h[b] = 0;
  __syncthreads();
  const uint32_t n = *count, chunk = (n + kQsGroups - 1) / kQsGroups;
  const uint32_t i0 = blockIdx.x * chunk, i1 = min(n, i0 + chunk);
  for (uint32_t i = i0 + threadIdx.x; i < i1; i += kQsThreads) atomicAdd(&h[key[i]], 1u);
  __syncthreads();
  for (uint32_t b = threadIdx.x; b < kQueueBuckets; b += kQsThreads)
    if (h[b]) atomicAdd(&hist[b], h[b]);
}

__global__ __launch_bounds__(kQsThreads) void qs_scan(uint32_t *hist)
{
  static_assert(kQueueBuckets == 4 * kQsThreads, "qs_scan: 4 buckets per thread");
  __shared__ uint32_t s[kQsThreads];
  const uint32_t t = threadIdx.x;
  const uint4 v = reinterpret_cast<const uint4 *>(hist)[t];
  const uint32_t sum = v.x + v.y + v.z + v.w;
  s[t] = sum;
  __syncthreads();
  for (uint32_t off = 1; off < kQsThreads; off <<= 1)
  {
    const uint32_t x = t >= off ? s[t - off] : 0u;
    __syncthreads();
    s[t] += x;
    __syncthreads();
  }
  const uint32_t e = s[t] - sum;
  reinterpret_cast<uint4 *>(hist)[t] = make_uint4(e, e + v.x, e + v.x + v.y, e + v.x + v.y + v.z);
}

__global__ __launch_bounds__(kQsThreads) void qs_scatter(const uint32_t *count, const uint32_t *key, uint32_t *cursor,
                                                         uint32_t *order)
{
  __shared__ uint32_t h[kQueueBuckets];
  for (uint32_t b = threadIdx.x; b < kQueueBuckets; b += kQsThreads) h[b] = 0;
  __syncthreads();
  const uint32_t n = *count, chunk = (n + kQsGroups - 1) / kQsGroups;
  const uint32_t i0 = blockIdx.x * chunk, i1 = min(n, i0 + chunk);
  for (uint32_t i = i0 + threadIdx.x; i < i1; i += kQsThreads) atomicAdd(&h[key[i]], 1u);
  __syncthreads();
  for (uint32_t b = threadIdx.x; b < kQueueBuckets; b += kQsThreads)
    if (h[b]) h[b] = atomicAdd(&cursor[b], h[b]);
  __syncthreads();
  for (uint32_t i = i0 + threadIdx.x; i < i1; i += kQsThreads) order[atomicAdd(&h[key[i]], 1u)] = i;
}

hipError_t launch_queue_sort(const uint32_t *count, const uint32_t *key, uint32_t *hist, uint32_t *order, hipStream_t st)
{
  hipLaunchKernelGGL(qs_hist, dim3(kQsGroups), dim3(kQsThreads), 0, st, count, key, hist);
  hipLaunchKernelGGL(qs_scan, dim3(1), dim3(kQsThreads), 0, st, hist);
  hipLaunchKernelGGL(qs_scatter, dim3(kQsGroups), dim3(kQsThreads), 0, st, count, key, hist, order);
  return hipGetLastError();
}

constexpr int kTriplesPerThread = 16;
constexpr int kRngBlock = 256;
constexpr uint64_t kTriplesPerBlock = (uint64_t)kTriplesPerThread * kRngBlock;

__device__ __forceinline__ uint32_t thread_state(uint32_t s, const uint32_t *jump, uint64_t b, uint32_t tid)
{
  const uint32_t *bj = jump + 2 * (kRngBlock + b), *tj = jump + 2 * tid;
  return tj[0] * (bj[0] * s + bj[1]) + tj[1];
}

constexpr int kHalfRun = kTriplesPerThread / 2;
struct LcgJump { uint32_t a, c; };
constexpr LcgJump lcg_jump_const(int draws)
{
  uint32_t a = 1u, c = 0u;
  for (int i = 0; i < draws; ++i) { a = 214013u * a; c = 214013u * c + 2531011u; }
  return LcgJump{a, c};
}
constexpr LcgJump kHalfJump = lcg_jump_const(3 * kHalfRun);
struct TripleJumps { LcgJump m[kTriplesPerThread]; };
constexpr TripleJumps triple_jumps()
{
  TripleJumps t{};
  for (int j = 0; j < kTriplesPerThread; ++j) t.m[j] = lcg_jump_const(3 * j);
  return t;
}
constexpr TripleJumps kTripleJump = triple_jumps();

__device__ __forceinline__ bool float_accept(uint32_t s1, uint32_t s2, uint32_t s3)
{
  const float x = rand_component_dev(lcg_out(s1)), y = rand_component_dev(lcg_out(s2)),
              z = rand_component_dev(lcg_out(s3));
  return !(x * x + y * y + z * z > 1.f);
}

#ifndef RFX_RNG_INT_ACCEPT
#define RFX_RNG_INT_ACCEPT 1
#endif
constexpr uint32_t kSphereN = 32767u * 32767u;
constexpr uint32_t kSphereShell = 1024u;

__device__ __forceinline__ uint32_t mad_u24(uint32_t a, uint32_t b, uint32_t c)
{
  uint32_t d;
  asm("v_mad_u32_u24 %0, %1, %2, %3" : "=v"(d) : "v"(a), "v"(b), "v"(c));
  return d;
}

__device__ __forceinline__ uint32_t sphere_n(uint32_t k1, uint32_t k2, uint32_t k3)
{
  const uint32_t q = mad_u24(k3, k3, mad_u24(k2, k2, mad_u24(k1, k1, 0u))), t = k1 + k2 + k3;
  return 4u * q - 131068u * t + 3u * kSphereN;
}

__device__ __forceinline__ void triple(uint32_t &s, int j, uint32_t &acc, uint32_t &und)
{
  const uint32_t s1 = lcg_step(s), s2 = lcg_step(s1), s3 = lcg_step(s2);
  s = s3;
#if RFX_RNG_INT_ACCEPT
  const uint32_t n = sphere_n(lcg_out(s1), lcg_out(s2), lcg_out(s3));
  acc |= (n < kSphereN ? 1u : 0u) << j;
  und |= (n - (kSphereN - kSphereShell) <= 2u * kSphereShell ? 1u : 0u) << j;
#else
  acc |= (float_accept(s1, s2, s3) ? 1u : 0u) << j;
#endif
}

template <bool kStates>
__device__ __forceinline__ uint32_t thread_flags(uint32_t s0, uint32_t *st)
{
  uint32_t s = s0, s2 = kHalfJump.a * s0 + kHalfJump.c, acc = 0, und = 0;
#pragma unroll
  for (int j = 0; j < kHalfRun; ++j)
  {
    if (kStates)
    {
      st[j] = s;
      st[j + kHalfRun] = s2;
    }
    triple(s, j, acc, und);
    triple(s2, j + kHalfRun, acc, und);
  }
  if (__builtin_expect(und != 0u, 0))
  {
    acc = 0u;
    s = s0;
#pragma nounroll
    for (int j = 0; j < kTriplesPerThread; ++j)
    {
      const uint32_t s1 = lcg_step(s), s2b = lcg_step(s1), s3 = lcg_step(s2b);
      s = s3;
      acc |= (float_accept(s1, s2b, s3) ? 1u : 0u) << j;
    }
  }
  return acc;
}

__global__ __launch_bounds__(kRngBlock) void rng_count(const uint32_t *seed, const uint32_t *jump, uint32_t *blk_cnt,
                                                       uint64_t blk0, uint16_t *masks)
{
  const uint64_t b = blk0 + blockIdx.x;
  const uint32_t acc = thread_flags<false>(thread_state(*seed, jump, b, threadIdx.x), nullptr);
  uint32_t c = (uint32_t)__popc(acc);
  if (masks) masks[b * kRngBlock + threadIdx.x] = (uint16_t)acc;
#pragma unroll
  for (int off = 32; off > 0; off >>= 1) c += __shfl_xor(c, off, 64);
  __shared__ uint32_t wsum[kRngBlock / 64];
  if ((threadIdx.x & 63) == 0) wsum[threadIdx.x >> 6] = c;
  __syncthreads();
  if (threadIdx.x == 0)
  {
    uint32_t tot = 0;
    for (int w = 0; w < kRngBlock / 64; ++w) tot += wsum[w];
    blk_cnt[b] = tot;
  }
}

struct EmitFilter {
  uint64_t ss2;
  uint64_t W;
  uint32_t row_block, rank, nranks;
  uint64_t lo, hi;
};

__device__ __forceinline__ bool owned(uint64_t idx, const EmitFilter &f)
{
  if (f.nranks <= 1) return idx >= f.lo && idx < f.hi;
  return ((idx / f.ss2 / f.W / f.row_block) % f.nranks) == f.rank;
}

constexpr int kScanThreads = 1024;

struct EmitIn {
  uint32_t cnt, s0, mask;
};
__device__ __forceinline__ EmitIn emit_in(uint32_t b, const uint32_t *seed, const uint32_t *jump, const uint32_t *blk_cnt,
                                          const uint16_t *masks)
{
  EmitIn e;
  e.cnt = blk_cnt[b];
  e.s0 = thread_state(*seed, jump, b, threadIdx.x);
  e.mask = masks ? (uint32_t)masks[(uint64_t)b * kRngBlock + threadIdx.x] : 0u;
  return e;
}

__device__ __forceinline__ void emit_block(uint64_t off, const EmitIn &in, bool have_masks, uint64_t need,
                                           uint32_t *rd_state, uint32_t *next_seed, const EmitFilter &flt,
                                           uint32_t *sst, uint32_t *wsum)
{
  if (off >= need) return;
  const uint32_t cnt = (uint32_t)min((uint64_t)in.cnt, need - off);
  const uint64_t last = off + cnt - 1;
  if (flt.nranks <= 1 && last != need - 1 && (last < flt.lo || off >= flt.hi)) return;
  if (flt.nranks > 1 && last != need - 1)
  {
    const uint64_t s_lo = off / flt.ss2 / flt.W / flt.row_block, s_hi = last / flt.ss2 / flt.W / flt.row_block;
    bool any = false;
    for (uint64_t st = s_lo; st <= s_hi && !any; ++st) any = (st % flt.nranks) == flt.rank;
    if (!any) return;
  }
  uint32_t st[kTriplesPerThread];
  uint32_t acc;
  if (have_masks)
  {
    acc = in.mask;
#pragma unroll
    for (int j = 0; j < kTriplesPerThread; ++j) st[j] = kTripleJump.m[j].a * in.s0 + kTripleJump.m[j].c;
  }
  else
    acc = thread_flags<true>(in.s0, st);
  const uint32_t c = (uint32_t)__popc(acc);
  const uint32_t lane = threadIdx.x & 63;
  uint32_t inc = c;
#pragma unroll
  for (int o = 1; o < 64; o <<= 1)
  {
    const uint32_t v = __shfl_up(inc, o, 64);
    if (lane >= (uint32_t)o) inc += v;
  }
  if (lane == 63) wsum[threadIdx.x >> 6] = inc;
  __syncthreads();
  uint32_t wbase = 0;
  for (uint32_t w = 0; w < (threadIdx.x >> 6); ++w) wbase += wsum[w];
  uint32_t li = wbase + (inc - c);
  const uint32_t fin = last == need - 1 ? cnt - 1 : ~0u;
#pragma unroll
  for (int j = 0; j < kTriplesPerThread; ++j)
    if ((acc >> j) & 1u)
    {
      if (li == fin) *next_seed = lcg_step(lcg_step(lcg_step(st[j])));
      if (li < cnt) sst[li] = st[j];
      ++li;
    }
  __syncthreads();
  for (uint32_t i = threadIdx.x; i < cnt; i += kRngBlock)
  {
    const uint64_t idx = off + i;
    if (owned(idx, flt)) rd_state[idx] = sst[i];
  }
}

__global__ __launch_bounds__(kRngBlock) void rng_emit(const uint32_t *seed, const uint32_t *jump, const uint32_t *blk_cnt,
                                                      const uint16_t *masks, uint64_t need, uint32_t *rd_state,
                                                      uint32_t *next_seed, int *err, EmitFilter flt)
{
  __shared__ uint32_t sst[kTriplesPerBlock];
  __shared__ uint32_t wsum[kRngBlock / 64];
  __shared__ uint32_t wpart[kRngBlock / 64];
  const EmitIn in = emit_in(blockIdx.x, seed, jump, blk_cnt, masks);
  uint32_t part = 0;
  if (((uintptr_t)blk_cnt & 15u) == 0)
  {
    const uint4 *v4 = reinterpret_cast<const uint4 *>(blk_cnt);
    const uint32_t nvec = blockIdx.x >> 2;
    for (uint32_t k0 = 0; k0 < nvec; k0 += 4 * kRngBlock)
    {
      uint4 a[4];
#pragma unroll
      for (int u = 0; u < 4; ++u)
      {
        const uint32_t k = k0 + (uint32_t)u * kRngBlock + threadIdx.x;
        a[u] = k < nvec ? v4[k] : make_uint4(0u, 0u, 0u, 0u);
      }
#pragma unroll
      for (int u = 0; u < 4; ++u) part += a[u].x + a[u].y + a[u].z + a[u].w;
    }
    if (threadIdx.x < (blockIdx.x & 3u)) part += blk_cnt[(nvec << 2) + threadIdx.x];
  }
  else
    for (uint32_t k = threadIdx.x; k < blockIdx.x; k += kRngBlock) part += blk_cnt[k];
#pragma unroll
  for (int o = 32; o > 0; o >>= 1) part += __shfl_xor(part, o, 64);
  if ((threadIdx.x & 63) == 0) wpart[threadIdx.x >> 6] = part;
  __syncthreads();
  uint64_t off = 0;
#pragma unroll
  for (int w = 0; w < kRngBlock / 64; ++w) off += wpart[w];
  if (blockIdx.x == gridDim.x - 1 && threadIdx.x == 0 && off + in.cnt < need) *err = 1;
  emit_block(off, in, masks != nullptr, need, rd_state, next_seed, flt, sst, wsum);
}

constexpr uint32_t kScanTile = 16 * kScanThreads;
__global__ __launch_bounds__(kScanThreads) void rng_band_range(const uint32_t *blk_cnt, uint64_t nblk, uint64_t need,
                                                               uint64_t lo, uint64_t hi, uint64_t *off, uint32_t *range,
                                                               int *err)
{
  __shared__ uint32_t t[kScanTile];
  __shared__ uint32_t wsum[kScanThreads / 64];
  const uint32_t tid = threadIdx.x, lane = tid & 63u, wv = tid >> 6;
  if (tid == 0) { range[0] = 0; range[1] = 0; range[2] = 0; }
  uint64_t carry = 0;
  for (uint64_t base = 0; base < nblk; base += kScanTile)
  {
    const uint32_t n = (uint32_t)min((uint64_t)kScanTile, nblk - base);
#pragma unroll
    for (uint32_t k = 0; k < 16; ++k)
    {
      const uint32_t i = k * kScanThreads + tid;
      t[i] = i < n ? blk_cnt[base + i] : 0u;
    }
    __syncthreads();
    uint32_t c[16], sum = 0;
#pragma unroll
    for (uint32_t k = 0; k < 16; ++k) { c[k] = t[16 * tid + k]; sum += c[k]; }
    uint32_t inc = sum;
#pragma unroll
    for (int o = 1; o < 64; o <<= 1)
    {
      const uint32_t v = __shfl_up(inc, o, 64);
      if (lane >= (uint32_t)o) inc += v;
    }
    if (lane == 63) wsum[wv] = inc;
    __syncthreads();
    uint32_t wb = 0, tot = 0;
    for (uint32_t w = 0; w < kScanThreads / 64; ++w)
    {
      wb += w < wv ? wsum[w] : 0u;
      tot += wsum[w];
    }
    uint64_t run = carry + wb + (inc - sum);
#pragma unroll
    for (uint32_t k = 0; k < 16; ++k)
    {
      const uint64_t b = base + 16 * tid + k, e = run + c[k];
      if (c[k] && run <= lo && lo < e) range[0] = (uint32_t)b;
      if (c[k] && run <= hi - 1 && hi - 1 < e) range[1] = (uint32_t)b;
      if (c[k] && run <= need - 1 && need - 1 < e) range[2] = (uint32_t)b;
      t[16 * tid + k] = (uint32_t)run;
      run = e;
    }
    __syncthreads();
#pragma unroll
    for (uint32_t k = 0; k < 16; ++k)
    {
      const uint32_t i = k * kScanThreads + tid;
      if (i < n) off[base + i] = t[i];
    }
    carry += tot;
    __syncthreads();
  }
  if (tid == 0 && carry < need) *err = 1;
}

constexpr uint32_t kScanTileCounts = 4096, kTileSumThreads = 256;
__global__ __launch_bounds__(kTileSumThreads) void rng_tile_sums(const uint32_t *blk_cnt, uint64_t nblk,
                                                                 uint32_t *tile_sum, uint32_t *range)
{
  __shared__ uint32_t wsum[kTileSumThreads / 64];
  const uint64_t base = (uint64_t)blockIdx.x * kScanTileCounts;
  const uint32_t n = (uint32_t)min((uint64_t)kScanTileCounts, nblk - base);
  uint32_t sum = 0;
  if (n == kScanTileCounts && ((uintptr_t)(blk_cnt + base) & 15u) == 0)
  {
    const uint4 *v = reinterpret_cast<const uint4 *>(blk_cnt + base);
#pragma unroll
    for (uint32_t k = 0; k < kScanTileCounts / 4 / kTileSumThreads; ++k)
    {
      const uint4 a = v[k * kTileSumThreads + threadIdx.x];
      sum += a.x + a.y + a.z + a.w;
    }
  }
  else
    for (uint32_t i = threadIdx.x; i < n; i += kTileSumThreads) sum += blk_cnt[base + i];
#pragma unroll
  for (int o = 32; o > 0; o >>= 1) sum += __shfl_xor(sum, o, 64);
  if ((threadIdx.x & 63u) == 0) wsum[threadIdx.x >> 6] = sum;
  __syncthreads();
  if (threadIdx.x == 0)
  {
    uint32_t t = 0;
    for (uint32_t w = 0; w < kTileSumThreads / 64; ++w) t += wsum[w];
    tile_sum[blockIdx.x] = t;
    if (blockIdx.x == 0) { range[0] = 0; range[1] = 0; range[2] = 0; }
  }
}

__global__ __launch_bounds__(kScanThreads) void rng_tile_scan(const uint32_t *blk_cnt, uint64_t nblk, uint64_t need,
                                                              uint64_t lo, uint64_t hi, const uint32_t *tile_sum,
                                                              uint64_t *off, uint32_t *range, int *err)
{
  __shared__ uint32_t wsum[kScanThreads / 64];
  __shared__ uint64_t s_pre;
  const uint32_t tid = threadIdx.x, lane = tid & 63u, wv = tid >> 6;
  unsigned long long pre = 0;
// ... 59 lines not shown
  const uint32_t first = range[0], last = range[1], fin = range[2];
  const uint32_t n = last - first + 1 + (fin > last || fin < first ? 1u : 0u);
  for (uint32_t j = blockIdx.x; j < n; j += gridDim.x)
  {
    const uint32_t b = j <= last - first ? first + j : fin;
    if (b >= nblk) break;
    emit_block(off[b], emit_in(b, seed, jump, blk_cnt, masks), masks != nullptr, need, rd_state, next_seed, flt, sst,
               wsum);
    __syncthreads();
  }
}

#ifndef RFX_RNG_TICKET
#define RFX_RNG_TICKET 1
#endif
#ifndef RFX_LOOKBACK_SLEEP
#define RFX_LOOKBACK_SLEEP 1
#endif
constexpr uint64_t kStatAgg = 1ull << 34, kStatPre = 2ull << 34, kStatVal = (1ull << 34) - 1;
#ifndef RFX_LOOKBACK_SPINS
#define RFX_LOOKBACK_SPINS (1u << 22)
#endif
constexpr uint32_t kLookbackSpins = RFX_LOOKBACK_SPINS;

__device__ __forceinline__ unsigned long long status_load(const unsigned long long *p)
{
  return __hip_atomic_load(p, __ATOMIC_RELAXED, __HIP_MEMORY_SCOPE_AGENT);
}

__device__ __forceinline__ void status_store(unsigned long long *p, unsigned long long v)
{
  __hip_atomic_store(p, v, __ATOMIC_RELAXED, __HIP_MEMORY_SCOPE_AGENT);
}

__global__ __launch_bounds__(kRngBlock) void rng_fused(const uint32_t *seed, const uint32_t *jump, uint32_t nblk,
                                                       uint64_t need, uint32_t *rd_state, uint32_t *next_seed, int *err,
                                                       unsigned long long *status, unsigned long long *ticket,
                                                       unsigned long long base, uint32_t epoch)
{
  __shared__ uint32_t sst[kTriplesPerBlock];
  __shared__ uint32_t wsum[kRngBlock / 64];
  __shared__ uint64_t s_off;
  uint32_t b = blockIdx.x;
#if RFX_RNG_TICKET
  __shared__ uint32_t s_b;
  if (threadIdx.x == 0) s_b = (uint32_t)(atomicAdd(ticket, 1ull) - base);
  __syncthreads();
  b = s_b;
#endif
  uint32_t st[kTriplesPerThread];
  const uint32_t acc = thread_flags<true>(thread_state(*seed, jump, b, threadIdx.x), st);
  const uint32_t c = (uint32_t)__popc(acc);
  const uint32_t lane = threadIdx.x & 63;
  uint32_t inc = c;
#pragma unroll
  for (int o = 1; o < 64; o <<= 1)
  {
    const uint32_t v = __shfl_up(inc, o, 64);
    if (lane >= (uint32_t)o) inc += v;
  }
  if (lane == 63) wsum[threadIdx.x >> 6] = inc;
  __shared__ uint32_t s_gaveup;
  if (threadIdx.x == 0) s_gaveup = 0;
  __syncthreads();
  uint32_t wbase = 0, tot = 0;
  for (uint32_t w = 0; w < kRngBlock / 64; ++w)
  {
    if (w < (threadIdx.x >> 6)) wbase += wsum[w];
    tot += wsum[w];
  }
  const unsigned long long tag = (unsigned long long)epoch << 36;
  if (threadIdx.x < 64)
  {
    uint64_t excl = 0;
    if (b == 0)
    {
      if (lane == 0) status_store(&status[0], tag | kStatPre | tot);
    }
    else
    {
      if (lane == 0) status_store(&status[b], tag | kStatAgg | tot);
      int64_t j = (int64_t)b - 1 - (int64_t)lane;
      uint32_t spins = 0;
      bool gaveup = false;
      for (;;)
      {
        const unsigned long long w = j >= 0 ? status_load(&status[j]) : (tag | kStatPre);
        const bool ready = (w >> 36) == (unsigned long long)epoch && (w & (3ull << 34)) != 0;
        const uint64_t pre = __ballot(ready && (w & (3ull << 34)) == kStatPre);
        const uint32_t first = pre ? (uint32_t)__builtin_ctzll(pre) : 64u;
        const uint64_t upto = first >= 63 ? ~0ull : (2ull << first) - 1ull;
        if (__ballot(!ready) & upto)
        {
          if (++spins > kLookbackSpins)
          {
            gaveup = true;
            break;
          }
          __builtin_amdgcn_s_sleep(RFX_LOOKBACK_SLEEP);
          continue;
        }
        uint64_t v = lane <= first ? (uint64_t)(w & kStatVal) : 0ull;
#pragma unroll
        for (int o = 32; o > 0; o >>= 1) v += __shfl_xor(v, o, 64);
        excl += v;
        if (first < 64) break;
        j -= 64;
      }
      if (gaveup)
      {
        if (lane == 0) s_gaveup = 1;
      }
      else if (lane == 0)
        status_store(&status[b], tag | kStatPre | ((excl + tot) & kStatVal));
    }
    if (lane == 0) s_off = excl;
  }
  __syncthreads();
  if (s_gaveup)
  {
    uint32_t part = 0;
    for (uint32_t pb = 0; pb < b; ++pb)
    {
      part += (uint32_t)__popc(thread_flags<false>(thread_state(*seed, jump, pb, threadIdx.x), nullptr));
    }
#pragma unroll
    for (int o = 32; o > 0; o >>= 1) part += __shfl_xor(part, o, 64);
    if (threadIdx.x == 0) s_off = 0;
    __syncthreads();
    if (lane == 0) atomicAdd((unsigned long long *)&s_off, (unsigned long long)part);
    __syncthreads();
    if (threadIdx.x == 0)
    {
      status_store(&status[b], tag | kStatPre | ((s_off + tot) & kStatVal));
      atomicOr(err, 4);
    }
  }
  const uint64_t off = s_off;
  if (b == nblk - 1 && threadIdx.x == 0 && off + tot < need) *err = 1;
  if (off >= need) return;
  const uint32_t cnt = (uint32_t)min((uint64_t)tot, need - off);
  uint32_t li = wbase + (inc - c);
  const uint32_t fin = off + cnt == need ? cnt - 1 : ~0u;
#pragma unroll
  for (int j = 0; j < kTriplesPerThread; ++j)
    if ((acc >> j) & 1u)
    {
      if (li == fin) *next_seed = lcg_step(lcg_step(lcg_step(st[j])));
      if (li < cnt) sst[li] = st[j];
      ++li;
    }
  __syncthreads();
  for (uint32_t i = threadIdx.x; i < cnt; i += kRngBlock) rd_state[off + i] = sst[i];
}

constexpr uint32_t kKatThreads = 256;

__device__ __forceinline__ void stage_lut(float *lut)
{
  for (uint32_t i = threadIdx.x; i < 256; i += blockDim.x) lut[i] = (float)i / 255.0f;
}

__global__ __launch_bounds__(kKatThreads) void kat_objects(DevScene S, const float *rays, const int32_t *objs, uint32_t n,
                                                          float *out)
{
  __shared__ float lut[256];
  stage_lut(lut);
  __syncthreads();
  const uint32_t i = blockIdx.x * kKatThreads + threadIdx.x;
  if (i >= n) return;
  Cnt cnt;
  const float *q = rays + 6 * (size_t)i;
  const v3 o = mk(q[0], q[1], q[2]), ray = mk(q[3], q[4], q[5]);
  const int32_t loc = S.obj_loc[objs[i]];
  const int kind = loc >> 28, idx = loc & 0x0FFFFFFF;
  const RayConst k = ray_const(ray);
  bool hit = false, any = false, pre_bad = false;
  float t = 0.0f, sq = 0.0f, t2, sq2, u = 0.0f, v = 0.0f, u2, v2;
  v3 norm = mk(0.0f, 0.0f, 0.0f), drop = o;
  col c = mkc(0.0f, 0.0f, 0.0f);
  if (kind == 0)
  {
    const SphereGeo g = S.sph_geo[idx];
    SpherePair p;
    p.cx[0] = g.cx; p.cy[0] = g.cy; p.cz[0] = g.cz; p.r2[0] = g.sq_radius;
    p.cx[1] = 0.0f; p.cy[1] = 0.0f; p.cz[1] = 0.0f; p.r2[1] = -INFINITY;
    f2 b, d;
    pair_bd(p, o, k, b, d);
    hit = pair_may_hit(b, d) && sphere_tail<false, false>(b.x, d.x, ray, k, t, sq, cnt);
    any = pair_may_hit(b, d) && sphere_tail<false, true>(b.x, d.x, ray, k, t2, sq2, cnt);
    if (hit)
    {
      drop = add(o, mul(ray, t));
      norm = sub(drop, mk(g.cx, g.cy, g.cz));
      const MatRec m = S.sph_mat[idx];
      c = mkc(m.r, m.g, m.b);
    }
  }
  else if (kind == 1)
  {
    hit = tri_hit<false, false>(S.tri_geo[idx], o, ray, t, u, v, sq, cnt, k);
    any = tri_hit<false, true>(S.tri_geo[idx], o, ray, t2, u2, v2, sq2, cnt, k);
    if (tri_hit<false, true, true>(S.tri_geo[idx], o, ray, t2, u2, v2, sq2, cnt, k) != any) pre_bad = true;
    if (hit)
    {
      drop = add(o, mul(ray, t));
      const TriShade sh = S.tri_shade[idx];
      norm = mk(sh.nx, sh.ny, sh.nz);
      const MatRec m = S.tri_mat[idx];
      c = sh.tex >= 0 ? tri_texel<false>(S, sh, u, v, lut, cnt) : mkc(m.r, m.g, m.b);
    }
  }
  else
  {
    const PlaneGeo g = S.pln_geo[idx];
    hit = plane_hit<false, false>(g, o, ray, t, sq, cnt, k);
    any = plane_hit<false, true>(g, o, ray, t2, sq2, cnt, k);
    if (hit)
    {
      drop = add(o, mul(ray, t));
      norm = mk(g.nx, g.ny, g.nz);
      const MatRec m = S.pln_mat[idx];
      c = mkc(m.r, m.g, m.b);
    }
  }
  float *w = out + 15 * (size_t)i;
  for (int j = 0; j < 15; ++j) w[j] = 0.0f;
  w[0] = hit ? 1.0f : 0.0f;
  if (hit)
  {
    const v3 rf = reflect(mul(ray, t), norm);
    w[1] = drop.x; w[2] = drop.y; w[3] = drop.z;
    w[4] = norm.x; w[5] = norm.y; w[6] = norm.z;
    w[7] = rf.x; w[8] = rf.y; w[9] = rf.z;
    w[10] = sqrt_rn(sq);
    w[11] = c.r; w[12] = c.g; w[13] = c.b;
  }
  w[14] = pre_bad ? __builtin_nanf("") : any ? 1.0f : 0.0f;
}

__global__ __launch_bounds__(kKatThreads) void kat_texels(DevScene S, int tex, const float *in, uint32_t n, float *out)
{
  __shared__ float lut[256];
  stage_lut(lut);
  __syncthreads();
  const uint32_t i = blockIdx.x * kKatThreads + threadIdx.x;
  if (i >= n) return;
  Cnt cnt;
  const col c = tex >= 0 ? texel_uv<false>(S, tex, in[2 * (size_t)i], in[2 * (size_t)i + 1], lut, cnt)
                         : skybox_texel<false>(S, mk(in[3 * (size_t)i], in[3 * (size_t)i + 1], in[3 * (size_t)i + 2]), lut, cnt);
  out[3 * (size_t)i] = c.r; out[3 * (size_t)i + 1] = c.g; out[3 * (size_t)i + 2] = c.b;
}

__global__ __launch_bounds__(kKatThreads) void kat_powf(const float *xy, uint32_t n, float *out)
{
  stage_powf_tables();
  __syncthreads();
  const uint32_t i = blockIdx.x * kKatThreads + threadIdx.x;
  if (i < n)
  {
    const float x = xy[2 * (size_t)i], y = xy[2 * (size_t)i + 1];
    out[i] = y == 3.0f ? powf3_dev(x) : powf_dev(x, y);
  }
}

__global__ __launch_bounds__(kKatThreads) void kat_powf_cube(uint32_t first, uint32_t n, unsigned long long *counts)
{
  stage_powf_tables();
  __syncthreads();
  const uint32_t i = blockIdx.x * kKatThreads + threadIdx.x;
  bool bad = false, slow = false;
  if (i < n)
  {
    const float x = __uint_as_float(first + i);
    float p;
    slow = !powf_cube_fast(x, p);
    bad = __float_as_uint(powf3_dev(x)) != __float_as_uint(powf_dev(x, 3.0f));
  }
  const uint64_t mb = __ballot(bad), ms = __ballot(slow);
  if ((threadIdx.x & 63u) == 0 && (mb | ms))
  {
    atomicAdd(&counts[0], (unsigned long long)__popcll(mb));
    atomicAdd(&counts[1], (unsigned long long)__popcll(ms));
  }
}

__device__ __forceinline__ uint32_t kat_mix(uint64_t x)
{
  x ^= x >> 33; x *= 0xff51afd7ed558ccdull; x ^= x >> 33; x *= 0xc4ceb9fe1a85ec53ull; x ^= x >> 33;
  return (uint32_t)x;
}
__device__ __forceinline__ float kat_float(uint32_t sign, int32_t e, uint32_t mant)
{
  return __uint_as_float((sign & 1u) << 31 | (uint32_t)(e + 127) << 23 | (mant & 0x7FFFFFu));
}
__device__ __forceinline__ bool kat_same(float x, float y)
{
  return __float_as_uint(x) == __float_as_uint(y) || (x != x && y != y);
}
__global__ __launch_bounds__(kKatThreads) void kat_div(uint64_t first, uint32_t n, unsigned long long *counts)
{
  const uint32_t i = blockIdx.x * kKatThreads + threadIdx.x;
  uint32_t bad = 0, fast = 0, seen = 0;
  if (i < n)
  {
    const uint64_t k = first + i;
// ... 29 lines not shown
      default: b = kat_float(h1 >> 31, (int32_t)(h0 % 253u) - 126, 0u); a = kat_float(h2 >> 31, (int32_t)(h1 % 253u) - 126, h2 >> 1); break;
    }
    const float q = div_rn(a, b);
    bool ok;
    (void)div_fast(a, div_prep(b), ok);
    const float a2 = __uint_as_float(__float_as_uint(a) ^ (h2 & 0x807F0000u)), a3 = b * -0.5f;
    const v3 v = mk(a, a2, a3), nv = normalized(v);
    const float l = len(v);
    const bool sv = l > kVerySmall;
    const float rx = sv ? v.x / l : v.x, ry = sv ? v.y / l : v.y, rz = sv ? v.z / l : v.z;
    const float den = fabsf(b) + kVerySmall, p = fabsf(a) <= den ? a : copysignf(den, a) * 0.75f;
    bool okp;
    float pd = div_fast_unit(p, den, rcp_refined(den), okp);
    const bool unit_ok = den <= 0x1p64f;
    if (!okp) pd = p / den;
    bad = (kat_same(q, a / b) ? 0u : 1u) + (kat_same(nv.x, rx) ? 0u : 1u) + (kat_same(nv.y, ry) ? 0u : 1u) +
          (kat_same(nv.z, rz) ? 0u : 1u) + (!unit_ok || kat_same(pd, p / den) ? 0u : 1u);
    fast = ok ? 1u : 0u;
    seen = 5;
  }
#pragma unroll
  for (int o = 32; o > 0; o >>= 1)
  {
    bad += __shfl_xor(bad, o, 64);
    fast += __shfl_xor(fast, o, 64);
    seen += __shfl_xor(seen, o, 64);
  }
  if ((threadIdx.x & 63u) == 0 && seen)
  {
    if (bad) atomicAdd(&counts[0], (unsigned long long)bad);
    atomicAdd(&counts[1], (unsigned long long)fast);
    atomicAdd(&counts[2], (unsigned long long)seen);
  }
}

template <bool SWAPPED>
__device__ __forceinline__ void kernarg_compare(const DevScene &S, const FrameParams &P, uint32_t *out)
{
  const uint32_t *ps = (const uint32_t *)&P, *qs = (const uint32_t *)&kernarg_params();
  uint32_t bad_p = 0, bad_s = 0;
  for (size_t i = 0; i < sizeof(FrameParams) / 4; ++i) bad_p += ps[i] != qs[i] ? 1u : 0u;
#ifdef RFX_LAUNDER_SCENE
  const uint32_t *a = (const uint32_t *)&S, *b = (const uint32_t *)&launder_scene<true>(S);
  for (size_t i = 0; i < sizeof(DevScene) / 4; ++i) bad_s += a[i] != b[i] ? 1u : 0u;
  out[2] = 1;
#else
  out[2] = 0;
#endif
  out[0] = bad_s;
  out[1] = bad_p;
}
__global__ void kat_kernarg(DevScene S, FrameParams P, uint32_t *out)
{
  if (threadIdx.x == 0 && blockIdx.x == 0) kernarg_compare<false>(S, P, out);
}
__global__ void kat_kernarg_swapped(FrameParams P, DevScene S, uint32_t *out)
{
  if (threadIdx.x == 0 && blockIdx.x == 0) kernarg_compare<true>(S, P, out);
}

__global__ __launch_bounds__(kKatThreads) void kat_argb(const float *rgb, uint32_t n, uint32_t *out)
{
  const uint32_t i = blockIdx.x * kKatThreads + threadIdx.x;
  if (i < n) out[i] = argb(mkc(rgb[3 * (size_t)i], rgb[3 * (size_t)i + 1], rgb[3 * (size_t)i + 2]));
}

}



namespace rfx {

uint64_t rng_blocks_for(uint64_t traces)
{
  const uint64_t triples = 2 * traces + 65536;
  return (triples + kTriplesPerBlock - 1) / kTriplesPerBlock;
}

void rng_jump_table(uint64_t nblk, uint32_t *out)
{
  uint32_t a1 = 1u, c1 = 0u;
  for (int i = 0; i < 3 * kTriplesPerThread; ++i) { c1 = 214013u * c1 + 2531011u; a1 = 214013u * a1; }
  uint32_t A = 1u, C = 0u;
  for (int t = 0; t < kRngBlock; ++t)
  {
    out[2 * t] = A; out[2 * t + 1] = C;
    C = a1 * C + c1; A = a1 * A;
  }
  const uint32_t ab = A, cb = C;
  A = 1u; C = 0u;
  for (uint64_t b = 0; b < nblk; ++b)
  {
    out[2 * (kRngBlock + b)] = A; out[2 * (kRngBlock + b) + 1] = C;
    C = ab * C + cb; A = ab * A;
  }
}

hipError_t launch_rng_count(const uint32_t *d_seed, const uint32_t *d_jump, uint32_t *d_blk_cnt, uint64_t blk0,
                            uint64_t nblk_slice, uint16_t *d_masks, hipStream_t st)
{
  if (nblk_slice)
    hipLaunchKernelGGL(rng_count, dim3((uint32_t)nblk_slice), dim3(kRngBlock), 0, st, d_seed, d_jump, d_blk_cnt, blk0,
                       d_masks);
  return hipGetLastError();
}

hipError_t launch_rng_finish(const uint32_t *d_seed, const uint32_t *d_jump, uint32_t *d_next_seed,
                             const uint32_t *d_blk_cnt, const uint16_t *d_masks, uint64_t nblk, uint64_t traces,
                             uint32_t *d_rd_state, int *d_err, uint64_t ss2, uint64_t W, uint32_t row_block,
                             uint32_t rank, uint32_t nranks, hipStream_t st)
{
  const EmitFilter flt{ss2 ? ss2 : 1, W ? W : 1, row_block ? row_block : 1, rank, nranks ? nranks : 1, 0, UINT64_MAX};
  hipLaunchKernelGGL(rng_emit, dim3((uint32_t)nblk), dim3(kRngBlock), 0, st, d_seed, d_jump, d_blk_cnt, d_masks,
                     traces, d_rd_state, d_next_seed, d_err, flt);
  return hipGetLastError();
}

#ifndef RFX_SCAN_TILES
#define RFX_SCAN_TILES 2
#endif
hipError_t launch_rng_finish_band(const uint32_t *d_seed, const uint32_t *d_jump, uint32_t *d_next_seed,
                                  const uint32_t *d_blk_cnt, const uint16_t *d_masks, uint64_t nblk, uint64_t traces,
                                  uint32_t *d_rd_state, int *d_err, uint64_t lo, uint64_t hi, uint64_t *d_off,
                                  uint32_t *d_range, uint32_t *d_tile_sum, hipStream_t st)
{
  const EmitFilter flt{1, 1, 1, 0, 1, lo, hi};
  const uint64_t ntiles = (nblk + kScanTileCounts - 1) / kScanTileCounts;
  if (RFX_SCAN_TILES && ntiles >= RFX_SCAN_TILES && d_tile_sum)
  {
    hipLaunchKernelGGL(rng_tile_sums, dim3((uint32_t)ntiles), dim3(kTileSumThreads), 0, st, d_blk_cnt, nblk, d_tile_sum,
                       d_range);
    hipLaunchKernelGGL(rng_tile_scan, dim3((uint32_t)ntiles), dim3(kScanThreads), 0, st, d_blk_cnt, nblk, traces, lo, hi,
                       (const uint32_t *)d_tile_sum, d_off, d_range, d_err);
  }
  else
    hipLaunchKernelGGL(rng_band_range, dim3(1), dim3(kScanThreads), 0, st, d_blk_cnt, nblk, traces, lo, hi, d_off,
                       d_range, d_err);
  const uint64_t est = (hi - lo) / 2048 + 4;
  hipLaunchKernelGGL(rng_emit_band, dim3((uint32_t)std::min<uint64_t>(est, nblk)), dim3(kRngBlock), 0, st, d_seed, d_jump,
                     d_blk_cnt, d_masks, (const uint64_t *)d_off, (const uint32_t *)d_range, nblk, traces, d_rd_state,
                     d_next_seed, flt);
  return hipGetLastError();
}

hipError_t launch_rng_fused(const uint32_t *d_seed, const uint32_t *d_jump, uint32_t *d_next_seed, uint64_t nblk,
                            uint64_t traces, uint32_t *d_rd_state, int *d_err, unsigned long long *d_status,
                            unsigned long long *d_ticket, unsigned long long base, uint32_t epoch, hipStream_t st)
{
  hipLaunchKernelGGL(rng_fused, dim3((uint32_t)nblk), dim3(kRngBlock), 0, st, d_seed, d_jump, (uint32_t)nblk, traces,
                     d_rd_state, d_next_seed, d_err, d_status, d_ticket, base, epoch);
  return hipGetLastError();
}

static void launch_mode_cfg(bool stats, int mode, int cfg, dim3 grid, const DevScene &S, const FrameParams &P,
                            hipStream_t st)
{
  if (mode == kModeBlock) (stats ? launch_trace_block_stats : launch_trace_block_fast)(cfg, grid, S, P, st);
  else if (mode == kModePlain)
  {
    if (stats) launch_trace_plain_stats(cfg, grid, S, P, st);
    else if (P.park_after > 0) launch_trace_plain_park(cfg, grid, S, P, st);
    else launch_trace_plain_fast(cfg, grid, S, P, st);
  }
  else if (mode == kModeSsaaLanes) (stats ? launch_trace_lanes_stats : launch_trace_lanes_fast)(cfg, grid, S, P, st);
  else if (mode == kModeSsaaChunks) (stats ? launch_trace_chunks_stats : launch_trace_chunks_fast)(cfg, grid, S, P, st);
  else (stats ? launch_trace_ssaa_stats : launch_trace_ssaa_fast)(cfg, grid, S, P, st);
}

static dim3 kat_grid(uint32_t n) { return dim3((n + kKatThreads - 1) / kKatThreads); }

hipError_t launch_kat_kernarg(const DevScene &S, const FrameParams &P, int swapped, uint32_t *out, hipStream_t st)
{
  if (swapped) hipLaunchKernelGGL(kat_kernarg_swapped, dim3(1), dim3(64), 0, st, P, S, out);
  else hipLaunchKernelGGL(kat_kernarg, dim3(1), dim3(64), 0, st, S, P, out);
  return hipGetLastError();
}

hipError_t launch_kat(int what, const DevScene &S, int tex, const void *in, const int32_t *objs, uint32_t n, void *out,
                      hipStream_t st)
{
  if (!n) return hipSuccess;
  switch (what)
  {
    case 0: hipLaunchKernelGGL(kat_objects, kat_grid(n), dim3(kKatThreads), 0, st, S, (const float *)in, objs, n, (float *)out); break;
    case 1: hipLaunchKernelGGL(kat_texels, kat_grid(n), dim3(kKatThreads), 0, st, S, tex, (const float *)in, n, (float *)out); break;
    case 2: hipLaunchKernelGGL(kat_powf, kat_grid(n), dim3(kKatThreads), 0, st, (const float *)in, n, (float *)out); break;
    default: hipLaunchKernelGGL(kat_argb, kat_grid(n), dim3(kKatThreads), 0, st, (const float *)in, n, (uint32_t *)out); break;
  }
  return hipGetLastError();
}

hipError_t launch_kat_div(uint64_t first, uint32_t n, unsigned long long *counts, hipStream_t st)
{
  if (!n) return hipSuccess;
  hipLaunchKernelGGL(kat_div, kat_grid(n), dim3(kKatThreads), 0, st, first, n, counts);
  return hipGetLastError();
}

hipError_t launch_kat_powf_cube(uint32_t first, uint32_t n, unsigned long long *counts, hipStream_t st)
{
  if (!n) return hipSuccess;
  hipLaunchKernelGGL(kat_powf_cube, kat_grid(n), dim3(kKatThreads), 0, st, first, n, counts);
  return hipGetLastError();
}

#ifndef RFX_NOCULL_MAX_TILES
#define RFX_NOCULL_MAX_TILES 0
#endif

static int trace_mode(const FrameParams &P)
{
  if (P.ss < 0) return kModeBlock;
  if (P.ss == 1 && !P.additive && !P.accumulate) return kModePlain;
  if (!RFX_SSAA_LANES || !ss_lane_block(P.ss)) return kModeSsaa;
  return P.ss > 8 ? kModeSsaaChunks : kModeSsaaLanes;
}

static dim3 trace_grid(const FrameParams &P)
{
  const int mode = trace_mode(P);
  if (mode == kModeSsaaLanes || mode == kModeSsaaChunks)
  {
    const uint32_t bw = ss_lane_block(P.ss);
    return dim3((P.W + kTileWavesX * bw - 1) / (kTileWavesX * bw), (P.grid_rows + kTileWavesY * bw - 1) / (kTileWavesY * bw));
  }
  const uint32_t cols = P.ss < 0 ? (P.W + (uint32_t)(-P.ss) - 1) / (uint32_t)(-P.ss) : P.W;
  return dim3((cols + kTileW - 1) / kTileW, (P.grid_rows + kTileH - 1) / kTileH);
}

uint32_t trace_tiles(const FrameParams &P)
{
  const dim3 g = trace_grid(P);
  return kWgWaves * g.x * g.y;
}

bool trace_lanes(const FrameParams &P)
{
  return trace_mode(P) == kModeSsaaLanes;
}

bool trace_chunks(const FrameParams &P)
{
  return trace_mode(P) == kModeSsaaChunks;
}

hipError_t launch_prim_cull(const DevScene &S, const FrameParams &P, uint64_t *masks, hipStream_t st)
{
  const dim3 grid = trace_grid(P);
  if (!(S.n_sph <= 32 && S.n_tri <= 32))
    hipLaunchKernelGGL(prim_cull_large_kernel<0>, grid, dim3(kWgThreads), 0, st, S, P, masks);
  else if (trace_lanes(P) || trace_chunks(P))
  {
    if (S.n_pln > 0)
      hipLaunchKernelGGL((prim_cull_kernel<true, true>), grid, dim3(kWgThreads), 0, st, S, P, masks);
    else
      hipLaunchKernelGGL((prim_cull_kernel<false, true>), grid, dim3(kWgThreads), 0, st, S, P, masks);
  }
  else if (S.n_pln > 0)
    hipLaunchKernelGGL(prim_cull_kernel<true>, grid, dim3(kWgThreads), 0, st, S, P, masks);
  else
    hipLaunchKernelGGL(prim_cull_kernel<false>, grid, dim3(kWgThreads), 0, st, S, P, masks);
  return hipGetLastError();
}

hipError_t launch_trace(const DevScene &S, const FrameParams &P, bool stats, hipStream_t st)
{
  const dim3 grid = trace_grid(P);
  FrameParams Pt = P;
  Pt.tiles_x = kTileWavesX * grid.x;
  const int mode = trace_mode(P);
  const bool cull = !stats && !(RFX_NOCULL_MAX_TILES > 0 && S.n_sph <= 32 && S.n_tri <= 32 &&
                                trace_tiles(P) <= (uint32_t)RFX_NOCULL_MAX_TILES);
  const int cfg = (S.n_light > 32 ? kCfgManyLights : 0) | (cull ? kCfgCull : 0) |
                  (S.n_sph <= 32 && S.n_tri <= 32 ? kCfgSmall : 0) | (S.n_pln > 0 ? kCfgPlanes : 0) |
                  (S.n_light == 1 && !stats && RFX_ONE_LIGHT ? kCfgOneLight : 0) |
                  (RFX_TRI_BVH && S.tri_bvh != nullptr && !stats ? kCfgTriBvh : 0);
  launch_mode_cfg(stats, mode, cfg, grid, S, Pt, st);
  return hipGetLastError();
}

}
```

reflaxman_amd/render.py:

```python
from __future__ import annotations

import ctypes as C
import os
from typing import List, Optional, Sequence

import numpy as np

from . import _lib
from ._lib import DIELECTRIC, METAL, check, farr

DEFAULT_SPHERE_SEED = 1350490027
DEFAULT_JITTER_SEED = 424238335


class Vector3:
    __slots__ = ("x", "y", "z")

    def __init__(self, x=0.0, y=0.0, z=0.0):
        self.x, self.y, self.z = float(x), float(y), float(z)

    def __iter__(self):
        return iter((self.x, self.y, self.z))

    def __repr__(self):
# ... 130 lines not shown
        return {"nodes": nodes, "leaves": leaves, "leaf_size": leaf, "depth": depth, "boxes": boxes,
                "children": children, "leaf_ids": ids, "residual": res}

    def addPlane(self, pos: Vector3, norm: Vector3, material: Material) -> Plane:
        obj = check(_lib.load().rfx_scene_add_plane(self._h, farr(Vector3(*pos)), farr(Vector3(*norm)), material.type,
                                                    farr(material.color), material.reflectivity, material.transparency),
                    "Scene.addPlane")
        self._version += 1
        return Plane(self, obj)

    def addLight(self, origin: Vector3, radius: float, color: Color, power: float) -> OmniLight:
        idx = check(_lib.load().rfx_scene_add_light(self._h, farr(Vector3(*origin)), float(radius), farr(Color(*color)),
                                                    float(power)), "Scene.addLight")
        self._version += 1
        return OmniLight(self, idx)

    def addTexture(self, fileName: str) -> Texture:
        loaded = C.c_int(0)
        idx = check(_lib.load().rfx_scene_add_texture_file(self._h, os.fsencode(fileName), C.byref(loaded)),
                    "Scene.addTexture")
        self._version += 1
        return Texture(self, idx, bool(loaded.value))

    def addTextureArgb(self, argb: Optional[np.ndarray]) -> Texture:
        L = _lib.load()
        if argb is None:
            idx = check(L.rfx_scene_add_texture_argb(self._h, 0, 0, None), "Scene.addTextureArgb")
        else:
            a = np.ascontiguousarray(argb, dtype=np.uint32)
            idx = check(L.rfx_scene_add_texture_argb(self._h, a.shape[1], a.shape[0], _lib.u32ptr(a)), "Scene.addTextureArgb")
        self._version += 1
        return Texture(self, idx, argb is not None)

    def setSkyboxTexture(self, fileName: str) -> bool:
        ok = check(_lib.load().rfx_scene_set_skybox_file(self._h, os.fsencode(fileName)), "Scene.setSkyboxTexture")
        self._version += 1
        return bool(ok)

    def setSkyboxTextureArgb(self, argb: Optional[np.ndarray]) -> bool:
        L = _lib.load()
        if argb is None:
            ok = check(L.rfx_scene_set_skybox_argb(self._h, 0, 0, None), "Scene.setSkyboxTextureArgb")
        else:
            a = np.ascontiguousarray(argb, dtype=np.uint32)
            ok = check(L.rfx_scene_set_skybox_argb(self._h, a.shape[1], a.shape[0], _lib.u32ptr(a)), "Scene.setSkyboxTextureArgb")
        self._version += 1
        return bool(ok)

    def counts(self):
        v = [C.c_int() for _ in range(4)]
        check(_lib.load().rfx_scene_counts(self._h, *[C.byref(x) for x in v]), "Scene.counts")
        return tuple(x.value for x in v)


def build_scene(desc, texture_dir: Optional[str] = None) -> tuple:
    d = desc.diffuse
    s = Scene(Color(d[0], d[1], d[2]), d[3])
    files = {}
    if texture_dir is not None:
        path = desc.write(texture_dir)
        for line in open(path):
            parts = line.split()
            if parts and parts[0] in ("skybox", "texture"):
                files.setdefault(parts[0], []).append(
                    None if parts[1] == "-" else os.path.join(texture_dir, parts[1]))
    if desc.skybox is not None:
        if texture_dir is not None:
            s.setSkyboxTexture(files["skybox"][0] or "/nonexistent/absent.tga")
        else:
            s.setSkyboxTextureArgb(desc.skybox.argb)
    for (o, r, c, p) in desc.lights:
        s.addLight(Vector3(*o), r, Color(*c), p)
    if texture_dir is not None:
        texs = [s.addTexture(f or "/nonexistent/absent.tga") for f in files.get("texture", [])]
    else:
        texs = [s.addTextureArgb(t.argb) for t in desc.textures]
    handles = []
    for ob in desc.objects:
        mt, rgb, refl, tr = ob[-1]
        m = Material(mt, Color(*rgb), refl, tr)
        if ob[0] == "sphere":
            handles.append(s.addSphere(Vector3(*ob[1]), ob[2], m))
        elif ob[0] == "plane":
            handles.append(s.addPlane(Vector3(*ob[1]), Vector3(*ob[2]), m))
        else:
            handles.append(s.addTriangle(Vector3(*ob[1]), Vector3(*ob[2]), Vector3(*ob[3]), m))
    for (oi, ti, uv) in desc.settex:
        handles[oi].setTexture(texs[ti], *uv)
    eye, at, fov = desc.camera
    return s, Camera(Vector3(*eye), Vector3(*at), fov)


class Renderer:

    def __init__(self, device: int = 0, sphere_seed: int = DEFAULT_SPHERE_SEED, jitter_seed: int = DEFAULT_JITTER_SEED):
        L = _lib.load()
        h = C.c_void_p()
        check(L.rfx_renderer_create(C.byref(h), int(device)), "rfx_renderer_create")
        self._h = h
        self.device = device
        self._scene_key = None
        self.set_rng(sphere_seed, jitter_seed)

    def close(self):
        if getattr(self, "_h", None) and _lib._lib is not None:
            _lib._lib.rfx_renderer_destroy(self._h)
            self._h = None

    __del__ = close

    def set_scene(self, scene: Scene):
        key = (id(scene), scene._version)
        if key != self._scene_key:
            check(_lib.load().rfx_renderer_set_scene(self._h, scene._h), "rfx_renderer_set_scene")
            self._scene_key = key
            self._scene_ref = scene

    def set_rng(self, sphere_seed: int, jitter_seed: int):
        check(_lib.load().rfx_renderer_set_rng(self._h, sphere_seed & 0xFFFFFFFF, jitter_seed & 0xFFFFFFFF), "set_rng")

    def get_rng(self):
        s, j = C.c_uint32(), C.c_uint32()
        check(_lib.load().rfx_renderer_get_rng(self._h, C.byref(s), C.byref(j)), "get_rng")
        return s.value, j.value

    def set_stream(self, stream_ptr: int):
        check(_lib.load().rfx_renderer_set_stream(self._h, C.c_void_p(stream_ptr)), "set_stream")

    def render_frame(self, frame: _lib.Frame, d_rgb: int, d_argb: int = 0, d_counters: int = 0, stream: int = 0):
        check(_lib.load().rfx_render_frame(self._h, C.byref(frame), C.c_void_p(d_rgb), C.c_void_p(d_argb or None),
                                           C.c_void_p(d_counters or None), C.c_void_p(stream or None)), "rfx_render_frame")

    def synchronize(self):
        check(_lib.load().rfx_synchronize(self._h), "rfx_synchronize")

    def set_tile_order(self, mode: int):
        check(_lib.load().rfx_renderer_set_tile_order(self._h, int(mode)), "set_tile_order")

    def set_prim_masks(self, mode: int):
        check(_lib.load().rfx_renderer_set_prim_masks(self._h, int(mode)), "set_prim_masks")

    def set_regroup(self, park_after: int):
        check(_lib.load().rfx_renderer_set_regroup(self._h, int(park_after)), "set_regroup")

    def set_regroup_sort(self, on: bool):
        check(_lib.load().rfx_renderer_set_regroup_sort(self._h, int(bool(on))), "set_regroup_sort")

    def set_launch_traces(self, max_traces: int):
        check(_lib.load().rfx_renderer_set_launch_traces(self._h, int(max_traces)), "set_launch_traces")

    def bounce_form(self) -> int:
        return _lib.load().rfx_renderer_bounce_form(self._h)

    def set_tri_accel(self, mode: int):
        check(_lib.load().rfx_renderer_set_tri_accel(self._h, int(mode)), "set_tri_accel")
        self._scene_key = None

    def accel_info(self) -> "_lib.AccelInfo":
        a = _lib.AccelInfo()
        check(_lib.load().rfx_renderer_accel_info(self._h, C.byref(a)), "accel_info")
        return a

    def set_timing(self, enable):
        check(_lib.load().rfx_renderer_set_timing(self._h, int(enable)), "set_timing")

    def get_timing(self):
        a, b, n = C.c_double(), C.c_double(), C.c_uint64()
        check(_lib.load().rfx_renderer_get_timing(self._h, C.byref(a), C.byref(b), C.byref(n)), "get_timing")
        return a.value, b.value, n.value

    def kat_objects(self, rays: np.ndarray, objects: np.ndarray) -> np.ndarray:
        rays = np.ascontiguousarray(rays, np.float32).reshape(-1, 6)
        objs = np.ascontiguousarray(objects, np.int32)
        out = np.zeros((rays.shape[0], 15), np.float32)
        check(_lib.load().rfx_kat_objects(self._h, _lib.fptr(rays), objs.ctypes.data_as(C.POINTER(C.c_int32)),
                                          rays.shape[0], _lib.fptr(out)), "rfx_kat_objects")
        return out

    def kat_texels(self, texture: int, inp: np.ndarray) -> np.ndarray:
        inp = np.ascontiguousarray(inp, np.float32)
        out = np.zeros((inp.shape[0], 3), np.float32)
        check(_lib.load().rfx_kat_texels(self._h, int(texture), _lib.fptr(inp), inp.shape[0], _lib.fptr(out)),
              "rfx_kat_texels")
        return out

    def kat_powf(self, xy: np.ndarray) -> np.ndarray:
        xy = np.ascontiguousarray(xy, np.float32)
        out = np.zeros(xy.shape[0], np.float32)
        check(_lib.load().rfx_kat_powf(self._h, _lib.fptr(xy), xy.shape[0], _lib.fptr(out)), "rfx_kat_powf")
        return out

    def kat_powf_cube(self):
        counts = (C.c_uint64 * 2)()
        check(_lib.load().rfx_kat_powf_cube(self._h, counts), "rfx_kat_powf_cube")
        return int(counts[0]), int(counts[1])

    def kat_argb(self, rgb: np.ndarray) -> np.ndarray:
        rgb = np.ascontiguousarray(rgb, np.float32)
        out = np.zeros(rgb.shape[0], np.uint32)
        check(_lib.load().rfx_kat_argb(self._h, _lib.fptr(rgb), rgb.shape[0], _lib.u32ptr(out)), "rfx_kat_argb")
        return out

    def rand_dirs(self, seed: int, n: int):
        out = np.zeros((n, 3), np.float32)
        after = C.c_uint32()
        check(_lib.load().rfx_rand_dirs(self._h, seed, n, _lib.fptr(out), C.byref(after)), "rfx_rand_dirs")
        return out, after.value


def make_frame(camera: Camera, W: int, H: int, reflect_num: int, sample_num: int = 1, additive: bool = False,
               additive_counter: int = 0, row_block: int = 0, rank: int = 0, nranks: int = 1,
               pixel_begin: int = 0, pixel_end: int = 0) -> _lib.Frame:
    f = _lib.Frame()
    f.eye[:] = list(camera.eye)
    f.view[:] = list(camera.view)
    f.fov = camera.fov
    f.width, f.height = W, H
    f.reflect_num, f.sample_num = reflect_num, sample_num
    f.additive, f.additive_counter = int(bool(additive)), additive_counter
    f.row_block, f.rank, f.nranks = row_block, rank, nranks
    f.pixel_begin, f.pixel_end = pixel_begin, pixel_end
    return f


class Render:

    def __init__(self, exePath: str = "", device: int = 0, sphere_seed: int = DEFAULT_SPHERE_SEED,
                 jitter_seed: int = DEFAULT_JITTER_SEED, load_default_scene: bool = True):
        self._r = Renderer(device, sphere_seed, jitter_seed)
        self.imageWidth = 0
        self.imageHeight = 0
        self.additiveCounter = 0
        self.inProgress = False
        self._curx = 0
        self._cury = 0
        self._d_img = None
        self._cap = 0
        self._host = None
        self._host_valid = False
        self.camera = Camera()
        self.scene = Scene()
        self._refl = 0
        self._ss = 0
        self._additive = False
        if load_default_scene:
            self.loadScene(exePath)

    def loadScene(self, exePath: str):
        from . import scenes
        sky = os.path.join(exePath, "./textures/skybox.tga")
        plane = os.path.join(exePath, "./textures/himiya.tga")
        self.camera = Camera(Vector3(*scenes.DEFAULT_CAMERA[0]), Vector3(*scenes.DEFAULT_CAMERA[1]), scenes.DEFAULT_CAMERA[2])
        self.scene = Scene(Color(0.95, 0.95, 1.0), 0.15)
        self.scene.setSkyboxTexture(sky)
        self.scene.addLight(Vector3(11.8e9, 4.26e9, 3.08e9), 3.48e8, Color(1.0, 1.0, 0.95), 0.85)
        for (c, r, mt, rgb, refl) in [
            ((-1.25, 1.5, -0.25), 1.5, METAL, (1.0, 1.0, 1.0), 1.0), ((0.15, 1.0, 1.75), 1.0, METAL, (1.0, 1.0, 1.0), 0.95),
            ((-3.0, 0.6, -3.0), 0.6, DIELECTRIC, (1.0, 1.0, 1.0), 0.0), ((-0.5, 0.5, -2.5), 0.5, DIELECTRIC, (0.5, 1.0, 0.15), 0.75),
            ((1.0, 0.4, -1.5), 0.4, DIELECTRIC, (0.0, 0.5, 1.0), 1.0), ((1.8, 0.4, 0.1), 0.4, METAL, (1.0, 0.65, 0.45), 1.0),
            ((1.7, 0.5, 1.9), 0.5, METAL, (1.0, 0.90, 0.60), 0.75), ((0.6, 0.6, 4.2), 0.6, METAL, (0.9, 0.9, 0.9), 0.0)]:
            self.scene.addSphere(Vector3(*c), r, Material(mt, Color(*rgb), refl, 0.0))
        tex = self.scene.addTexture(plane)
        tr1 = self.scene.addTriangle(Vector3(-14.0, 0.0, -10.0), Vector3(-14.0, 0.0, 10.0), Vector3(14.0, 0.0, -10.0),
                                     Material(DIELECTRIC, Color(1.0, 1.0, 1.0), 0.95, 0.0))
        tr1.setTexture(tex, 0.0, 0.0, 0.0, 1.0, 1.0, 0.0)
        tr2 = self.scene.addTriangle(Vector3(-14.0, 0.0, 10.0), Vector3(14.0, 0.0, 10.0), Vector3(14.0, 0.0, -10.0),
                                     Material(DIELECTRIC, Color(1.0, 1.0, 1.0), 0.95, 0.0))
        tr2.setTexture(tex, 0.0, 1.0, 1.0, 1.0, 1.0, 0.0)

    def setImageSize(self, width: int, height: int):
        if width <= 0 or height <= 0:
            return
        L = _lib.load()
        n = width * height * 3 * 4
        if n > self._cap:
            if self._d_img:
                check(L.rfx_device_free(self._r._h, self._d_img), "device_free")
                self._d_img = None
            p = C.c_void_p()
            check(L.rfx_device_alloc(self._r._h, n, C.byref(p)), "device_alloc")
            self._d_img, self._cap = p, n
        zeros = np.zeros(width * height * 3, np.float32)
        check(L.rfx_memcpy_h2d(self._r._h, self._d_img, zeros.ctypes.data_as(C.c_void_p), n), "memcpy_h2d")
        self.imageWidth, self.imageHeight = width, height
        self.additiveCounter = 0
        self.inProgress = False
        self._curx = self._cury = 0
        self._host_valid = False

    def _image(self) -> np.ndarray:
        if not self._host_valid:
            n = self.imageWidth * self.imageHeight
            self._host = np.empty((self.imageHeight, self.imageWidth, 3), np.float32)
            check(_lib.load().rfx_memcpy_d2h(self._r._h, self._host.ctypes.data_as(C.c_void_p), self._d_img, n * 12), "memcpy_d2h")
            self._host_valid = True
        return self._host

    @property
    def image(self) -> np.ndarray:
        return self._image()

    def imagePixel(self, x: int, y: int) -> Color:
        if x < 0 or y < 0:
            return Color(0, 0, 0)
        c = self._image()[y, x]
        if self.additiveCounter > 1:
# ... 66 lines not shown
```

Before: 13070 Mrays/s.

## Precompute full LCG cycle prefix table to replace per-frame RNG count/scan prepass

Builds a one-time device table covering the whole 2^32-state LCG cycle: per-block accepted-triple counts and their exclusive prefix sums. Each frame then only locates the seed's position in the cycle (once, cached across frames) and emits the RNG states directly, without re-counting and re-scanning every block. This removes the count and scan kernels from the per-frame prepass. The cost is a large one-time table build, extra device memory, and more state invalidation paths to keep the cached position correct.

```diff
diff --git a/include/rfx.h b/include/rfx.h
--- a/include/rfx.h
+++ b/include/rfx.h
@@ -106,6 +106,10 @@
 int rfx_render_frame(rfx_renderer *r, const rfx_frame *frame, float *d_rgb, uint32_t *d_argb,
                      uint64_t *d_counters, void *stream);
 int rfx_renderer_set_launch_traces(rfx_renderer *r, uint64_t max_traces);
+int rfx_renderer_set_rng_prepass(rfx_renderer *r, int mode);
+int rfx_renderer_prepass_form(const rfx_renderer *r);
+uint32_t rfx_rng_triple_index(uint32_t state);
+uint32_t rfx_rng_seq_blocks(void);
 
 int rfx_frame_rng_blocks(rfx_renderer *r, const rfx_frame *frame, uint32_t nslices, uint64_t *blocks_per_slice);
 int rfx_frame_rng_count(rfx_renderer *r, const rfx_frame *frame, uint32_t slice, uint32_t nslices,
@@ -157,6 +161,8 @@
 int rfx_kat_powf_cube(rfx_renderer *r, uint64_t counts[2]);
 int rfx_kat_div(rfx_renderer *r, uint64_t first, uint64_t n, uint64_t counts[3]);
 int rfx_kat_kernarg(rfx_renderer *r, int swapped, uint32_t out[3]);
+int rfx_kat_rng_seq_prefix(rfx_renderer *r, uint32_t *prefix);
+int rfx_kat_rng_seq_legacy(rfx_renderer *r, uint32_t *counts);
 
 #ifdef __cplusplus
 }
diff --git a/reflaxman_amd/_lib.py b/reflaxman_amd/_lib.py
--- a/reflaxman_amd/_lib.py
+++ b/reflaxman_amd/_lib.py
@@ -101,6 +101,10 @@
     ("rfx_renderer_set_regroup_sort", C.c_int, [C.c_void_p, C.c_int]),
     ("rfx_renderer_set_launch_traces", C.c_int, [C.c_void_p, C.c_uint64]),
     ("rfx_renderer_bounce_form", C.c_int, [C.c_void_p]),
+    ("rfx_renderer_set_rng_prepass", C.c_int, [C.c_void_p, C.c_int]),
+    ("rfx_renderer_prepass_form", C.c_int, [C.c_void_p]),
+    ("rfx_rng_triple_index", C.c_uint32, [C.c_uint32]),
+    ("rfx_rng_seq_blocks", C.c_uint32, []),
     ("rfx_renderer_set_tri_accel", C.c_int, [C.c_void_p, C.c_int]),
     ("rfx_renderer_accel_info", C.c_int, [C.c_void_p, C.POINTER(AccelInfo)]),
     ("rfx_renderer_get_timing", C.c_int, [C.c_void_p, C.POINTER(C.c_double), C.POINTER(C.c_double), _u64p]),
@@ -118,6 +122,8 @@
     ("rfx_kat_powf_cube", C.c_int, [C.c_void_p, C.POINTER(C.c_uint64)]),
     ("rfx_kat_div", C.c_int, [C.c_void_p, C.c_uint64, C.c_uint64, C.POINTER(C.c_uint64)]),
     ("rfx_kat_kernarg", C.c_int, [C.c_void_p, C.c_int, C.POINTER(C.c_uint32)]),
+    ("rfx_kat_rng_seq_prefix", C.c_int, [C.c_void_p, _u32p]),
+    ("rfx_kat_rng_seq_legacy", C.c_int, [C.c_void_p, _u32p]),
 ]
 
 _lib = None
diff --git a/reflaxman_amd/csrc/rfx_host.cpp b/reflaxman_amd/csrc/rfx_host.cpp
--- a/reflaxman_amd/csrc/rfx_host.cpp
+++ b/reflaxman_amd/csrc/rfx_host.cpp
@@ -34,6 +34,17 @@
 hipError_t launch_rng_fused(const uint32_t *d_seed, const uint32_t *d_jump, uint32_t *d_next_seed, uint64_t nblk,
                             uint64_t traces, uint32_t *d_rd_state, int *d_err, unsigned long long *d_status,
                             unsigned long long *d_ticket, unsigned long long base, uint32_t epoch, hipStream_t st);
+uint32_t rng_seq_blocks();
+uint32_t rng_seq_header_words();
+void rng_seq_tables(uint32_t *hdr, uint32_t *state);
+uint32_t rng_seq_index_of(uint32_t s);
+hipError_t launch_rng_seq_build(const uint32_t *d_hdr, const uint32_t *d_state, uint32_t *d_p, uint32_t *d_tiles,
+                                hipStream_t st);
+hipError_t launch_rng_locate(const uint32_t *d_seed, const uint32_t *d_hdr, const uint32_t *d_state, const uint32_t *d_p,
+                             uint32_t *d_pos, hipStream_t st);
+hipError_t launch_rng_emit_seq(const uint32_t *d_pos, const uint32_t *d_hdr, const uint32_t *d_state, const uint32_t *d_p,
+                               uint64_t nblk, uint64_t traces, uint32_t *d_rd_state, uint32_t *d_next_seed,
+                               uint32_t *d_next_pos, int *d_err, hipStream_t st);
 hipError_t launch_trace(const DevScene &S, const FrameParams &P, bool stats, hipStream_t st);
 hipError_t launch_prim_cull(const DevScene &S, const FrameParams &P, uint64_t *masks, hipStream_t st);
 hipError_t launch_queue_sort(const uint32_t *count, const uint32_t *key, uint32_t *hist, uint32_t *order, hipStream_t st);
@@ -496,6 +507,15 @@
 #endif
 #ifndef RFX_SPLIT_STREAMS
 #define RFX_SPLIT_STREAMS 2
+#endif
+#ifndef RFX_RNG_SEQ
+#define RFX_RNG_SEQ 1
+#endif
+#ifndef RFX_RNG_SEQ_SPLIT
+#define RFX_RNG_SEQ_SPLIT 1
+#endif
+#ifndef RFX_RNG_SEQ_MIN_BLOCKS
+#define RFX_RNG_SEQ_MIN_BLOCKS 0
 #endif
 constexpr uint64_t kMaxLaunchTraces = 1ull << 31;
 #ifndef RFX_SCAN_EMIT_BLOCKS
@@ -535,6 +555,10 @@
   uint32_t rng_epoch = 0;
   uint16_t *d_rng_masks = nullptr;
   uint32_t *d_jump = nullptr;
+  uint32_t *d_seq_hdr = nullptr, *d_seq_state = nullptr, *d_seq_p = nullptr, *d_seq_tiles = nullptr, *d_seq_pos = nullptr;
+  bool seq_valid = false;
+  int rng_prepass = RFX_RNG_SEQ;
+  int prepass_form = 0;
   float *d_img = nullptr; uint32_t *d_argb = nullptr; uint64_t *d_cnt = nullptr; size_t img_cap = 0;
   int tile_mode = RFX_TILE_ORDER_DEFAULT;
   uint32_t *d_tile_cost = nullptr, *d_tile_order = nullptr, *d_tile_scratch = nullptr;
@@ -678,6 +702,8 @@
   (void)hipFree(r->d_tile_sum);
   (void)hipFree(r->d_rng_range);
   (void)hipFree(r->d_rng_status); (void)hipFree(r->d_rng_ticket);
+  (void)hipFree(r->d_seq_hdr); (void)hipFree(r->d_seq_state); (void)hipFree(r->d_seq_p); (void)hipFree(r->d_seq_tiles);
+  (void)hipFree(r->d_seq_pos);
   (void)hipFree(r->d_img); (void)hipFree(r->d_argb); (void)hipFree(r->d_cnt);
   (void)hipFree(r->d_queue); (void)hipFree(r->d_qctr); (void)hipFree(r->d_prim_mask);
   (void)hipFree(r->d_split_mask[0]); (void)hipFree(r->d_split_mask[1]);
@@ -730,6 +756,21 @@
   r->prim_seen.clear();
   return RFX_OK;
 }
+
+extern "C" int rfx_renderer_set_rng_prepass(rfx_renderer *r, int mode)
+{
+  if (!r || mode < 0 || mode > 1) return fail(RFX_ERR_ARG, "renderer_set_rng_prepass: mode 0 or 1");
+  r->rng_prepass = mode;
+  return RFX_OK;
+}
+
+extern "C" int rfx_renderer_prepass_form(const rfx_renderer *r)
+{
+  if (!r) return fail(RFX_ERR_ARG, "renderer_prepass_form: null renderer");
+  return r->prepass_form;
+}
+
+extern "C" uint32_t rfx_rng_triple_index(uint32_t state) { return rng_seq_index_of(state); }
 
 extern "C" int rfx_renderer_bounce_form(const rfx_renderer *r)
 {
@@ -1347,6 +1388,7 @@
   HIP_CHECK(hipStreamSynchronize(r->stream));
   r->jitter_seed = jitter_seed;
   r->rewind_ok = false;
+  r->seq_valid = false;
   ++r->state_seq;
   return RFX_OK;
 }
@@ -1437,6 +1479,8 @@
   HIP_CHECK(launch_rng_finish(seed_cur(r), r->d_jump, seed_next(r), r->d_blk_cnt, r->d_rng_masks, nblk, traces,
                               r->d_rd, r->d_err, 1, 1, 1, 0, 1, st));
   r->seed_idx ^= 1u;
+  r->seq_valid = false;
+  r->prepass_form = 0;
   ++r->state_seq;
   r->rewind_ok = false;
   return RFX_OK;
@@ -1535,6 +1579,8 @@
     HIP_CHECK(launch_rng_finish(seed_cur(r), r->d_jump, seed_next(r), d_counts, d_masks, nblk, pl.traces, rd,
                                 r->d_err, ss2, P.W, P.row_block, P.rank, P.nranks, st));
   r->seed_idx ^= 1u;
+  r->seq_valid = false;
+  r->prepass_form = 0;
   ++r->state_seq;
   if (emitted) HIP_CHECK(hipEventRecord(emitted, st));
   return RFX_OK;
@@ -1563,6 +1609,57 @@
                              r->d_rng_ticket, r->rng_tickets, r->rng_epoch, pl.st));
   r->rng_tickets += nblk;
   r->seed_idx ^= 1u;
+  r->seq_valid = false;
+  r->prepass_form = 2;
+  ++r->state_seq;
+  if (emitted) HIP_CHECK(hipEventRecord(emitted, pl.st));
+  return RFX_OK;
+}
+
+static bool seq_prepass(const rfx_renderer *r, const FramePlan &pl, uint64_t nblk)
+{
+  return RFX_RNG_SEQ && r->rng_prepass == 1 && !pl.band && (RFX_RNG_SEQ_SPLIT || !pl.split) && pl.P.nranks <= 1 &&
+         nblk >= (uint64_t)RFX_RNG_SEQ_MIN_BLOCKS && nblk + 1 <= (uint64_t)rng_seq_blocks() / 16 * 15;
+}
+
+static int ensure_seq_table(rfx_renderer *r, hipStream_t st)
+{
+  if (r->d_seq_p) return RFX_OK;
+  const uint32_t nb = rng_seq_blocks(), nh = rng_seq_header_words();
+  std::vector<uint32_t> hdr(nh), state(nb);
+  rng_seq_tables(hdr.data(), state.data());
+  uint32_t *d_p = nullptr;
+  if (!r->d_seq_hdr) HIP_CHECK(hipMalloc(&r->d_seq_hdr, nh * sizeof(uint32_t)));
+  if (!r->d_seq_state) HIP_CHECK(hipMalloc(&r->d_seq_state, (size_t)nb * sizeof(uint32_t)));
+  if (!r->d_seq_tiles) HIP_CHECK(hipMalloc(&r->d_seq_tiles, ((size_t)nb / 4096 + 4) * sizeof(uint32_t)));
+  if (!r->d_seq_pos) HIP_CHECK(hipMalloc(&r->d_seq_pos, 4 * sizeof(uint32_t)));
+  HIP_CHECK(hipMalloc(&d_p, ((size_t)nb + 4) * sizeof(uint32_t)));
+  hipError_t e = hipMemcpy(r->d_seq_hdr, hdr.data(), nh * sizeof(uint32_t), hipMemcpyHostToDevice);
+  if (e == hipSuccess) e = hipMemcpy(r->d_seq_state, state.data(), (size_t)nb * sizeof(uint32_t), hipMemcpyHostToDevice);
+  if (e == hipSuccess) e = launch_rng_seq_build(r->d_seq_hdr, r->d_seq_state, d_p, r->d_seq_tiles, st);
+  if (e == hipSuccess) e = hipStreamSynchronize(st);
+  if (e != hipSuccess)
+  {
+    (void)hipFree(d_p);
+    return fail(RFX_ERR_HIP, "cycle table: %s", hipGetErrorString(e));
+  }
+  r->d_seq_p = d_p;
+  r->seq_valid = false;
+  return RFX_OK;
+}
+
+static int prepass_seq(rfx_renderer *r, FramePlan &pl, uint64_t nblk, uint32_t *rd, hipEvent_t emitted)
+{
+  int rc;
+  if ((rc = ensure_seq_table(r, pl.st)) != RFX_OK) return rc;
+  uint32_t *pos = r->d_seq_pos + 2 * r->seed_idx, *next_pos = r->d_seq_pos + 2 * (r->seed_idx ^ 1u);
+  if (!r->seq_valid)
+    HIP_CHECK(launch_rng_locate(seed_cur(r), r->d_seq_hdr, r->d_seq_state, r->d_seq_p, pos, pl.st));
+  HIP_CHECK(launch_rng_emit_seq(pos, r->d_seq_hdr, r->d_seq_state, r->d_seq_p, nblk + 1, pl.traces, rd, seed_next(r),
+                                next_pos, r->d_err, pl.st));
+  r->seed_idx ^= 1u;
+  r->seq_valid = true;
+  r->prepass_form = 1;
   ++r->state_seq;
   if (emitted) HIP_CHECK(hipEventRecord(emitted, pl.st));
   return RFX_OK;
@@ -1819,6 +1916,7 @@
 {
   if (!r) return fail(RFX_ERR_ARG, "frame_rng_discard: null renderer");
   r->rewind_ok = false;
+  r->seq_valid = false;
   if (r->emit_pending >= 0)
   {
     r->seed_idx ^= 1u;
@@ -1870,9 +1968,11 @@
   if ((rc = timing_start(r, pl.st)) != RFX_OK) return rc;
   if (r->emit_pending >= 0)
     return fail(RFX_ERR_STATE, "render_frame: an emitted frame awaits rfx_render_frame_emitted (or rfx_frame_rng_discard)");
-  if (fused_prepass(pl, nblk))
-  {
-    if ((rc = prepass_fused(r, pl, nblk, r->d_rd, nullptr)) != RFX_OK) return rc;
+  if (seq_prepass(r, pl, nblk) || fused_prepass(pl, nblk))
+  {
+    if ((rc = seq_prepass(r, pl, nblk) ? prepass_seq(r, pl, nblk, r->d_rd, nullptr)
+                                       : prepass_fused(r, pl, nblk, r->d_rd, nullptr)) != RFX_OK)
+      return rc;
     r->trace_buf = 0;
     if ((rc = timing_event(r, pl.st)) != RFX_OK) return rc;
     if ((rc = trace_frame(r, pl, r->d_rd, d_rgb, d_argb, d_counters)) != RFX_OK) return rc;
@@ -1933,7 +2033,11 @@
     if (k > 0) HIP_CHECK(hipStreamWaitEvent(s2[side], r->split_ev[side ^ 1], 0));
     if ((rc = timing_start(r, pl.st)) != RFX_OK) return rc;
     uint32_t *rd = side ? r->d_rd_alt : r->d_rd;
-    if (fused_prepass(pl, nblk))
+    if (seq_prepass(r, pl, nblk))
+    {
+      if ((rc = prepass_seq(r, pl, nblk, rd, r->split_ev[side])) != RFX_OK) return rc;
+    }
+    else if (fused_prepass(pl, nblk))
     {
       if ((rc = prepass_fused(r, pl, nblk, rd, r->split_ev[side])) != RFX_OK) return rc;
     }
@@ -1966,6 +2070,7 @@
   if (!r) return fail(RFX_ERR_ARG, "frame_rng_rewind: null renderer");
   if (!r->rewind_ok) return fail(RFX_ERR_STATE, "frame_rng_rewind: the last call was not rfx_render_frame");
   if (r->rewind_flip) r->seed_idx ^= 1u;
+  r->seq_valid = false;
   ++r->state_seq;
   if (r->rewind_saved)
   {
@@ -2176,6 +2281,7 @@
   uint32_t after = 0;
   HIP_CHECK(hipMemcpyAsync(&after, seed_cur(r), sizeof(uint32_t), hipMemcpyDeviceToHost, r->stream));
   HIP_CHECK(hipMemcpyAsync(seed_cur(r), &saved, sizeof(uint32_t), hipMemcpyHostToDevice, r->stream));
+  r->seq_valid = false;
   if ((rc = rfx_synchronize(r)) != RFX_OK) return rc;
   for (uint64_t i = 0; i < n; ++i)
   {
@@ -2279,6 +2385,41 @@
   return RFX_OK;
 }
 
+extern "C" uint32_t rfx_rng_seq_blocks(void) { return rng_seq_blocks(); }
+
+extern "C" int rfx_kat_rng_seq_prefix(rfx_renderer *r, uint32_t *prefix)
+{
+  if (!r || !prefix) return fail(RFX_ERR_ARG, "kat_rng_seq_prefix: bad args");
+  int rc;
+  if ((rc = set_dev(r)) != RFX_OK) return rc;
+  if ((rc = ensure_seq_table(r, r->stream)) != RFX_OK) return rc;
+  HIP_CHECK(hipStreamSynchronize(r->stream));
+  HIP_CHECK(hipMemcpy(prefix, r->d_seq_p, ((size_t)rng_seq_blocks() + 1) * sizeof(uint32_t), hipMemcpyDeviceToHost));
+  return RFX_OK;
+}
+
+extern "C" int rfx_kat_rng_seq_legacy(rfx_renderer *r, uint32_t *counts)
+{
+  if (!r || !counts) return fail(RFX_ERR_ARG, "kat_rng_seq_legacy: bad args");
+  int rc;
+  if ((rc = set_dev(r)) != RFX_OK) return rc;
+  const uint64_t nb = rng_seq_blocks();
+  std::vector<uint32_t> jump(2 * (256 + nb));
+  rng_jump_table(nb, jump.data());
+  uint32_t *d_jump = nullptr, *d_cnt = nullptr, *d_origin = nullptr;
+  hipError_t e = hipMalloc(&d_jump, jump.size() * sizeof(uint32_t));
+  if (e == hipSuccess) e = hipMalloc(&d_cnt, nb * sizeof(uint32_t));
+  if (e == hipSuccess) e = hipMalloc(&d_origin, sizeof(uint32_t));
+  if (e == hipSuccess) e = hipMemcpy(d_jump, jump.data(), jump.size() * sizeof(uint32_t), hipMemcpyHostToDevice);
+  if (e == hipSuccess) e = hipMemset(d_origin, 0, sizeof(uint32_t));
+  if (e == hipSuccess) e = launch_rng_count(d_origin, d_jump, d_cnt, 0, nb, nullptr, r->stream);
+  if (e == hipSuccess) e = hipStreamSynchronize(r->stream);
+  if (e == hipSuccess) e = hipMemcpy(counts, d_cnt, nb * sizeof(uint32_t), hipMemcpyDeviceToHost);
+  (void)hipFree(d_jump); (void)hipFree(d_cnt); (void)hipFree(d_origin);
+  if (e != hipSuccess) return fail(RFX_ERR_HIP, "kat_rng_seq_legacy: %s", hipGetErrorString(e));
+  return RFX_OK;
+}
+
 extern "C" int rfx_kat_argb(rfx_renderer *r, const float *rgb, uint64_t n, uint32_t *out)
 {
   if (!r || (n && (!rgb || !out))) return fail(RFX_ERR_ARG, "kat_argb: bad args");
@@ -2306,7 +2447,11 @@
 }
 
 int rfx_detail_fail(int code, const char *msg) { return fail(code, "%s", msg); }
-uint32_t *rfx_detail_seed_word(rfx_renderer *r) { return seed_cur(r); }
+uint32_t *rfx_detail_seed_word(rfx_renderer *r)
+{
+  r->seq_valid = false;
+  return seed_cur(r);
+}
 uint32_t rfx_detail_jitter(const rfx_renderer *r) { return r->jitter_seed; }
 void rfx_detail_set_jitter(rfx_renderer *r, uint32_t jitter) { r->jitter_seed = jitter; }
 hipStream_t rfx_detail_stream(const rfx_renderer *r) { return r->stream; }
diff --git a/reflaxman_amd/csrc/rfx_kernels.hip b/reflaxman_amd/csrc/rfx_kernels.hip
--- a/reflaxman_amd/csrc/rfx_kernels.hip
+++ b/reflaxman_amd/csrc/rfx_kernels.hip
@@ -1,4 +1,6 @@
 #include "rfx_trace.h"
+
+#include <vector>
 
 #pragma clang fp contract(off)
 
@@ -277,12 +279,17 @@
   return e;
 }
 
+struct EmitSeq {
+  uint32_t base, before;
+  uint32_t *next_pos;
+};
 __device__ __forceinline__ void emit_block(uint64_t off, const EmitIn &in, bool have_masks, uint64_t need,
                                            uint32_t *rd_state, uint32_t *next_seed, const EmitFilter &flt,
-                                           uint32_t *sst, uint32_t *wsum)
+                                           uint32_t *sst, uint32_t *wsum, uint32_t skip = 0u,
+                                           const EmitSeq *seq = nullptr)
 {
   if (off >= need) return;
-  const uint32_t cnt = (uint32_t)min((uint64_t)in.cnt, need - off);
+  const uint32_t cnt = (uint32_t)min((uint64_t)(in.cnt - skip), need - off);
   const uint64_t last = off + cnt - 1;
   if (flt.nranks <= 1 && last != need - 1 && (last < flt.lo || off >= flt.hi)) return;
   if (flt.nranks > 1 && last != need - 1)
@@ -321,8 +328,21 @@
   for (int j = 0; j < kTriplesPerThread; ++j)
     if ((acc >> j) & 1u)
     {
-      if (li == fin) *next_seed = lcg_step(lcg_step(lcg_step(st[j])));
-      if (li < cnt) sst[li] = st[j];
+      const uint32_t ti = li - skip;
+      if (ti < cnt)
+      {
+        if (ti == fin)
+        {
+          *next_seed = lcg_step(lcg_step(lcg_step(st[j])));
+          if (seq)
+          {
+            const uint32_t k = seq->base + (uint32_t)kTriplesPerThread * threadIdx.x + (uint32_t)j + 1u;
+            seq->next_pos[0] = k;
+            seq->next_pos[1] = k ? seq->before + li + 1u : 0u;
+          }
+        }
+        sst[ti] = st[j];
+      }
       ++li;
     }
   __syncthreads();
@@ -688,6 +708,128 @@
     }
   __syncthreads();
   for (uint32_t i = threadIdx.x; i < cnt; i += kRngBlock) rd_state[off + i] = sst[i];
+}
+
+constexpr uint32_t kSeqBlocks = (uint32_t)((1ull << 32) / kTriplesPerBlock);
+static_assert((uint64_t)kSeqBlocks * kTriplesPerBlock == (1ull << 32), "the cycle is a whole number of blocks");
+static_assert(kSeqBlocks % kScanTileCounts == 0, "rng_seq_scan: whole tiles");
+
+__device__ __forceinline__ uint32_t seq_thread_state(uint32_t s, const uint32_t *tj, uint32_t tid)
+{
+  return tj[2 * tid] * s + tj[2 * tid + 1];
+}
+
+__global__ __launch_bounds__(kRngBlock) void rng_seq_count(const uint32_t *state, const uint32_t *tj, uint32_t *cnt)
+{
+  const uint32_t B = blockIdx.x;
+  uint32_t c = (uint32_t)__popc(thread_flags<false>(seq_thread_state(state[B], tj, threadIdx.x), nullptr));
+#pragma unroll
+  for (int off = 32; off > 0; off >>= 1) c += __shfl_xor(c, off, 64);
+  __shared__ uint32_t wsum[kRngBlock / 64];
+  if ((threadIdx.x & 63) == 0) wsum[threadIdx.x >> 6] = c;
+  __syncthreads();
+  if (threadIdx.x == 0)
+  {
+    uint32_t tot = 0;
+    for (int w = 0; w < kRngBlock / 64; ++w) tot += wsum[w];
+    cnt[B] = tot;
+  }
+}
+
+__global__ __launch_bounds__(kScanThreads) void rng_seq_scan(uint32_t *p, const uint32_t *tile_sum)
+{
+  static_assert(kScanTileCounts == 4 * kScanThreads, "rng_seq_scan: four counts per thread");
+  __shared__ uint32_t wsum[kScanThreads / 64];
+  __shared__ uint32_t s_pre;
+  const uint32_t tid = threadIdx.x, lane = tid & 63u, wv = tid >> 6;
+  uint32_t pre = 0;
+  for (uint32_t t = tid; t < blockIdx.x; t += kScanThreads) pre += tile_sum[t];
+#pragma unroll
+  for (int o = 32; o > 0; o >>= 1) pre += __shfl_xor(pre, o, 64);
+  if (tid == 0) s_pre = 0;
+  __syncthreads();
+  if (lane == 0 && pre) atomicAdd(&s_pre, pre);
+  __syncthreads();
+  uint4 *v = reinterpret_cast<uint4 *>(p + (size_t)blockIdx.x * kScanTileCounts) + tid;
+  const uint4 a = *v;
+  const uint32_t sum = a.x + a.y + a.z + a.w;
+  uint32_t inc = sum;
+#pragma unroll
+  for (int o = 1; o < 64; o <<= 1)
+  {
+    const uint32_t t = __shfl_up(inc, o, 64);
+    if (lane >= (uint32_t)o) inc += t;
+  }
+  if (lane == 63) wsum[wv] = inc;
+  __syncthreads();
+  uint32_t wb = 0, tot = 0;
+  for (uint32_t w = 0; w < kScanThreads / 64; ++w)
+  {
+    wb += w < wv ? wsum[w] : 0u;
+    tot += wsum[w];
+  }
+  const uint32_t e = s_pre + wb + (inc - sum);
+  *v = make_uint4(e, e + a.x, e + a.x + a.y, e + a.x + a.y + a.z);
+  if (blockIdx.x == gridDim.x - 1 && tid == 0) p[kSeqBlocks] = s_pre + tot;
+}
+
+__host__ __device__ inline uint32_t seq_index_of(uint32_t s, const uint32_t *pow2)
+{
+  uint32_t k = 0, x = 0;
+  for (int j = 0; j < 32; ++j)
+    if ((x ^ s) >> j & 1u)
+    {
+      k |= 1u << j;
+      x = pow2[2 * j] * x + pow2[2 * j + 1];
+    }
+  return k;
+}
+
+__global__ __launch_bounds__(kRngBlock) void rng_locate(const uint32_t *seed, const uint32_t *pow2, const uint32_t *state,
+                                                        const uint32_t *tj, const uint32_t *p, uint32_t *pos)
+{
+  __shared__ uint32_t wsum[kRngBlock / 64];
+  const uint32_t k = seq_index_of(*seed, pow2);
+  const uint32_t B = k / (uint32_t)kTriplesPerBlock, r = k % (uint32_t)kTriplesPerBlock;
+  const uint32_t acc = thread_flags<false>(seq_thread_state(state[B], tj, threadIdx.x), nullptr);
+  const uint32_t first = (uint32_t)kTriplesPerThread * threadIdx.x;
+  const uint32_t n = r > first ? min(r - first, (uint32_t)kTriplesPerThread) : 0u;
+  uint32_t c = (uint32_t)__popc(acc & ((1u << n) - 1u));
+#pragma unroll
+  for (int off = 32; off > 0; off >>= 1) c += __shfl_xor(c, off, 64);
+  if ((threadIdx.x & 63) == 0) wsum[threadIdx.x >> 6] = c;
+  __syncthreads();
+  if (threadIdx.x == 0)
+  {
+    uint32_t tot = 0;
+    for (int w = 0; w < kRngBlock / 64; ++w) tot += wsum[w];
+    pos[0] = k;
+    pos[1] = p[B] + tot;
+  }
+}
+
+__global__ __launch_bounds__(kRngBlock) void rng_emit_seq(const uint32_t *pos, const uint32_t *state, const uint32_t *tj,
+                                                          const uint32_t *p, uint64_t need, uint32_t *rd_state,
+                                                          uint32_t *next_seed, uint32_t *next_pos, int *err)
+{
+  __shared__ uint32_t sst[kTriplesPerBlock];
+  __shared__ uint32_t wsum[kRngBlock / 64];
+  const uint32_t k = pos[0], A = pos[1];
+  const uint32_t T = p[kSeqBlocks];
+  const uint32_t Bu = k / (uint32_t)kTriplesPerBlock + blockIdx.x, B = Bu % kSeqBlocks;
+  const uint32_t before = p[B];
+  EmitIn in;
+  in.cnt = p[B + 1] - before;
+  in.s0 = seq_thread_state(state[B], tj, threadIdx.x);
+  in.mask = 0u;
+  uint64_t off = 0;
+  uint32_t skip = 0;
+  if (blockIdx.x == 0) skip = min(A - before, in.cnt);
+  else off = (uint64_t)before + (Bu >= kSeqBlocks ? (uint64_t)T : 0ull) - (uint64_t)A;
+  if (blockIdx.x == gridDim.x - 1 && threadIdx.x == 0 && off + (in.cnt - skip) < need) *err = 1;
+  const EmitFilter flt{1, 1, 1, 0, 1, 0, UINT64_MAX};
+  const EmitSeq seq{B * (uint32_t)kTriplesPerBlock, before, next_pos};
+  emit_block(off, in, false, need, rd_state, next_seed, flt, sst, wsum, skip, &seq);
 }
 
 constexpr uint32_t kKatThreads = 256;
@@ -1023,6 +1165,67 @@
   return hipGetLastError();
 }
 
+uint32_t rng_seq_blocks() { return kSeqBlocks; }
+constexpr uint32_t kSeqPow2 = 2 * kRngBlock, kSeqHeader = kSeqPow2 + 64;
+uint32_t rng_seq_header_words() { return kSeqHeader; }
+
+void rng_seq_tables(uint32_t *hdr, uint32_t *state)
+{
+  std::vector<uint32_t> jump(2 * (kRngBlock + 2));
+  rng_jump_table(2, jump.data());
+  for (uint32_t i = 0; i < kSeqPow2; ++i) hdr[i] = jump[i];
+  const uint32_t ab = jump[2 * (kRngBlock + 1)], cb = jump[2 * (kRngBlock + 1) + 1];
+  uint32_t a = kTripleJump.m[1].a, c = kTripleJump.m[1].c;
+  for (int j = 0; j < 32; ++j)
+  {
+    hdr[kSeqPow2 + 2 * j] = a;
+    hdr[kSeqPow2 + 2 * j + 1] = c;
+    c = a * c + c;
+    a = a * a;
+  }
+  if (!state) return;
+  uint32_t s = 0;
+  for (uint32_t b = 0; b < kSeqBlocks; ++b)
+  {
+    state[b] = s;
+    s = ab * s + cb;
+  }
+}
+
+uint32_t rng_seq_index_of(uint32_t s)
+{
+  uint32_t hdr[kSeqHeader];
+  rng_seq_tables(hdr, nullptr);
+  return seq_index_of(s, hdr + kSeqPow2);
+}
+
+hipError_t launch_rng_seq_build(const uint32_t *d_hdr, const uint32_t *d_state, uint32_t *d_p, uint32_t *d_tiles,
+                                hipStream_t st)
+{
+  const uint32_t ntiles = kSeqBlocks / kScanTileCounts;
+  hipLaunchKernelGGL(rng_seq_count, dim3(kSeqBlocks), dim3(kRngBlock), 0, st, d_state, d_hdr, d_p);
+  hipLaunchKernelGGL(rng_tile_sums, dim3(ntiles), dim3(kTileSumThreads), 0, st, (const uint32_t *)d_p,
+                     (uint64_t)kSeqBlocks, d_tiles, d_tiles + ntiles);
+  hipLaunchKernelGGL(rng_seq_scan, dim3(ntiles), dim3(kScanThreads), 0, st, d_p, (const uint32_t *)d_tiles);
+  return hipGetLastError();
+}
+
+hipError_t launch_rng_locate(const uint32_t *d_seed, const uint32_t *d_hdr, const uint32_t *d_state, const uint32_t *d_p,
+                             uint32_t *d_pos, hipStream_t st)
+{
+  hipLaunchKernelGGL(rng_locate, dim3(1), dim3(kRngBlock), 0, st, d_seed, d_hdr + kSeqPow2, d_state, d_hdr, d_p, d_pos);
+  return hipGetLastError();
+}
+
+hipError_t launch_rng_emit_seq(const uint32_t *d_pos, const uint32_t *d_hdr, const uint32_t *d_state, const uint32_t *d_p,
+                               uint64_t nblk, uint64_t traces, uint32_t *d_rd_state, uint32_t *d_next_seed,
+                               uint32_t *d_next_pos, int *d_err, hipStream_t st)
+{
+  hipLaunchKernelGGL(rng_emit_seq, dim3((uint32_t)nblk), dim3(kRngBlock), 0, st, d_pos, d_state, d_hdr, d_p, traces,
+                     d_rd_state, d_next_seed, d_next_pos, d_err);
+  return hipGetLastError();
+}
+
 static void launch_mode_cfg(bool stats, int mode, int cfg, dim3 grid, const DevScene &S, const FrameParams &P,
                             hipStream_t st)
 {
diff --git a/reflaxman_amd/render.py b/reflaxman_amd/render.py
--- a/reflaxman_amd/render.py
+++ b/reflaxman_amd/render.py
@@ -306,6 +306,22 @@
     def bounce_form(self) -> int:
         return _lib.load().rfx_renderer_bounce_form(self._h)
 
+    def set_rng_prepass(self, mode: int):
+        check(_lib.load().rfx_renderer_set_rng_prepass(self._h, int(mode)), "set_rng_prepass")
+
+    def prepass_form(self) -> int:
+        return _lib.load().rfx_renderer_prepass_form(self._h)
+
+    def kat_rng_seq_prefix(self) -> np.ndarray:
+        out = np.zeros(_lib.load().rfx_rng_seq_blocks() + 1, np.uint32)
+        check(_lib.load().rfx_kat_rng_seq_prefix(self._h, _lib.u32ptr(out)), "rfx_kat_rng_seq_prefix")
+        return out
+
+    def kat_rng_seq_legacy(self) -> np.ndarray:
+        out = np.zeros(_lib.load().rfx_rng_seq_blocks(), np.uint32)
+        check(_lib.load().rfx_kat_rng_seq_legacy(self._h, _lib.u32ptr(out)), "rfx_kat_rng_seq_legacy")
+        return out
+
     def set_tri_accel(self, mode: int):
         check(_lib.load().rfx_renderer_set_tri_accel(self._h, int(mode)), "set_tri_accel")
         self._scene_key = None
```

Result: faster. 13250 Mrays/s (median of 6 runs) (+1.4%).
